# mrjoshuak/go-jpeg2000

Hardware: AMD Instinct MI355X
Metric: Mpixels/s encode+decode (4K sRGB, 5-3 lossless) (higher is better)
Workload: dtype int32

## Files before the change

go-jpeg2000_amd/csrc/ht.hip:

```cpp
#include <cstdlib>

#include "ht_tables.h"
#include "j2k_internal.h"

namespace j2k {

__device__ __constant__ uint16_t c_vlc_tbl0[1024] = J2K_HT_VLC_TBL0_INIT;
__device__ __constant__ uint16_t c_vlc_tbl1[1024] = J2K_HT_VLC_TBL1_INIT;
__device__ uint16_t g_vlc_enc[2 * 4 * 16];

__global__ void ht_build_enc_table() {
    const int t = threadIdx.x;
    if (t >= 128) return;
    const int initial = t >> 6, context = (t >> 4) & 3, rho = t & 15;
    const uint16_t *tbl = initial ? c_vlc_tbl0 : c_vlc_tbl1;
    uint16_t r = 0x0001;
    for (uint32_t cwd = 0; cwd < 128; cwd++) {
        const uint16_t e = tbl[(context << 7) | cwd];
        if (((e >> 4) & 0xF) == rho && (e & 0xF) > 0) { r = (uint16_t)((cwd << 4) | (e & 0xF)); break; }
    }
    g_vlc_enc[t] = r;
}

__device__ uint16_t g_vlc_pair1[16384];

__global__ void ht_build_pair_table() {
    const uint32_t idx = blockIdx.x * blockDim.x + threadIdx.x;
    if (idx >= 16384) return;
    const uint32_t e1 = c_vlc_tbl1[idx & 0x7F];
    const uint32_t len1 = e1 & 0xF, rho1 = (e1 >> 4) & 0xF, uo1 = (e1 >> 3) & 1;
    uint32_t r = 0x8000;
    if (len1 <= 7) {
        const uint32_t e2 = c_vlc_tbl1[((rho1 >> 2) << 7) | ((idx >> len1) & 0x7F)];
        const uint32_t len2 = e2 & 0xF, rho2 = (e2 >> 4) & 0xF, uo2 = (e2 >> 3) & 1;
        r = rho1 | rho2 << 4 | (len1 + len2) << 8 | uo2 << 13 | uo1 << 14;
    }
    g_vlc_pair1[idx] = (uint16_t)r;
}

__device__ __forceinline__ uint32_t shl32(uint32_t x, uint32_t n) { return n >= 32 ? 0u : x << n; }
__device__ __forceinline__ uint64_t shl64(uint64_t x, uint32_t n) { return n >= 64 ? 0ull : x << n; }
__device__ __forceinline__ uint64_t shr64(uint64_t x, uint32_t n) { return n >= 64 ? 0ull : x >> n; }
__device__ __forceinline__ uint32_t uabs(int v) { return v < 0 ? 0u - (uint32_t)v : (uint32_t)v; }

__device__ __forceinline__ uint32_t wave_incl_scan(uint32_t v) {
    v += (uint32_t)__builtin_amdgcn_update_dpp(0, (int)v, 0x111, 0xf, 0xf, false);
    v += (uint32_t)__builtin_amdgcn_update_dpp(0, (int)v, 0x112, 0xf, 0xf, false);
    v += (uint32_t)__builtin_amdgcn_update_dpp(0, (int)v, 0x114, 0xf, 0xf, false);
    v += (uint32_t)__builtin_amdgcn_update_dpp(0, (int)v, 0x118, 0xf, 0xf, false);
    v += (uint32_t)__builtin_amdgcn_update_dpp(0, (int)v, 0x142, 0xa, 0xf, false);
    v += (uint32_t)__builtin_amdgcn_update_dpp(0, (int)v, 0x143, 0xc, 0xf, false);
    return v;
}
__device__ __forceinline__ uint32_t wave_last(uint32_t v) { return (uint32_t)__builtin_amdgcn_readlane((int)v, 63); }

struct BitWriter {
    uint8_t *p;
    long pos, cap;
    uint64_t tmp;
    int bits;
    uint32_t last;
    int fault;
};

__device__ __forceinline__ void vlc_write(BitWriter &v, uint32_t val, uint32_t nbits) {
    v.tmp |= shl64((uint64_t)val, (uint32_t)v.bits);
    v.bits += (int)nbits;
    while (v.bits >= 8) {
        uint32_t b = (uint32_t)(v.tmp & 0xFF);
        if (v.last > 0x8F && (b & 0x7F) == 0x7F) b &= 0x7F;
        if (v.pos >= v.cap) { v.fault = 1; v.bits = 0; return; }
        v.p[v.pos++] = (uint8_t)b;
        v.last = b;
        v.tmp >>= 8;
        v.bits -= 8;
    }
}

__device__ __forceinline__ void ms_write(BitWriter &m, uint32_t val, uint32_t nbits) {
    m.tmp |= shl64((uint64_t)val, (uint32_t)m.bits);
    m.bits += (int)nbits;
    while (m.bits >= 8) {
        uint32_t b = (uint32_t)(m.tmp & 0xFF);
        if (m.pos >= m.cap) { m.fault = 1; m.bits = 0; return; }
        if (m.last == 0xFF) { b &= 0x7F; m.p[m.pos++] = (uint8_t)b; m.tmp >>= 7; m.bits -= 7; }
        else { m.p[m.pos++] = (uint8_t)b; m.tmp >>= 8; m.bits -= 8; }
        m.last = b;
    }
}

__device__ __forceinline__ void flush_bits(BitWriter &w) {
    while (w.bits > 0) {
        if (w.pos >= w.cap) { w.fault = 1; return; }
        w.p[w.pos++] = (uint8_t)(w.tmp & 0xFF);
        w.tmp >>= 8;
        w.bits -= 8;
        if (w.bits < 0) w.bits = 0;
    }
}

__device__ __forceinline__ void uvlc_one(BitWriter &v, uint32_t u) {
    if (u <= 1) vlc_write(v, 1, 1);
    else if (u <= 2) vlc_write(v, 2, 2);
    else { vlc_write(v, 0, 3); vlc_write(v, u - 3, 5); }
}

#define HT_FAST_MAX_SAMPLES 1024
#define HT_MS_WORDS (HT_FAST_MAX_SAMPLES * 31 / 32 + 4)
#define HT_VLC_WORDS (46 * (HT_FAST_MAX_SAMPLES / 8) / 32 + 8)

__device__ __forceinline__ void or_bits(uint32_t *buf, uint32_t bitpos, uint64_t val) {
    const uint32_t wd = bitpos >> 5, sh = bitpos & 31;
    const uint32_t lo = (uint32_t)(val << sh);
    const uint64_t hi = sh ? (val >> (32 - sh)) : (val >> 32);
    if (lo) atomicOr(&buf[wd], lo);
    if ((uint32_t)hi) atomicOr(&buf[wd + 1], (uint32_t)hi);
    if ((uint32_t)(hi >> 32)) atomicOr(&buf[wd + 2], (uint32_t)(hi >> 32));
}
__device__ __forceinline__ void zero_bytes(uint8_t *p, size_t n, int lane) {
    const size_t head = min(n, (size_t)((16 - ((uintptr_t)p & 15)) & 15));
    if ((size_t)lane < head) p[lane] = 0;
    uint8_t *q = p + head;
    const size_t nv = (n - head) >> 4;
    for (size_t i = lane; i < nv; i += 64) reinterpret_cast<uint4 *>(q)[i] = make_uint4(0, 0, 0, 0);
    const size_t done = head + (nv << 4);
    if (done + lane < n) p[done + lane] = 0;
}

__device__ __forceinline__ uint32_t ms_bits32(const uint32_t *buf, uint32_t bitpos) {
    const uint32_t wd = bitpos >> 5, sh = bitpos & 31;
    const uint64_t two = (uint64_t)buf[wd] | ((uint64_t)buf[wd + 1] << 32);
    return (uint32_t)(two >> sh);
}
__device__ __forceinline__ uint32_t get_bits8(const uint32_t *buf, uint32_t bitpos) {
    const uint32_t wd = bitpos >> 5, sh = bitpos & 31;
    const uint64_t two = (uint64_t)buf[wd] | ((uint64_t)buf[wd + 1] << 32);
    return (uint32_t)(two >> sh) & 0xFF;
}

template <bool LROWS>
__device__ __forceinline__ bool ht_form(const BlockJob &J, const int32_t *__restrict__ src, int lane, uint32_t *vbuf, uint32_t *mbuf,
                        uint32_t &TMout, uint32_t &TVout, const int32_t *lrows, const uint16_t *enc) {
    const int w = J.w, h = J.h, stride = LROWS ? J.w : J.stride;
    const int quadCols = (w + 3) / 4, P = (quadCols + 1) / 2, R = (h + 3) / 4, N = R * P;
    for (int i = lane; i < HT_VLC_WORDS; i += 64) vbuf[i] = 0;
    for (int i = lane; i < HT_MS_WORDS; i += 64) mbuf[i] = 0;
    __syncthreads();
    uint32_t vbase = 0, mbase = 0;
    int bad = 0;
    const bool vec_ok = ((J.stride & 3) == 0) && ((J.src_off & 3) == 0);
    for (int i0 = 0; i0 < N; i0 += 64) {
        const int it = i0 + lane;
        uint64_t vv = 0; uint32_t vl = 0, ml = 0;
        uint32_t mval[8], mlen[8];
#pragma unroll
        for (int i = 0; i < 8; i++) { mval[i] = 0; mlen[i] = 0; }
        if (it < N) {
            const int r = it / P, pi = it - r * P;
            const int initial = (r == 0);
            const int32_t *row = LROWS ? lrows + r * w : src + (size_t)(4 * r) * stride;
            const int xb = pi * 8;
            int v[8];
            if ((LROWS || vec_ok) && xb + 8 <= w) {
                const int4 a = *reinterpret_cast<const int4 *>(row + xb), b = *reinterpret_cast<const int4 *>(row + xb + 4);
                v[0] = a.x; v[1] = a.y; v[2] = a.z; v[3] = a.w; v[4] = b.x; v[5] = b.y; v[6] = b.z; v[7] = b.w;
            } else {
#pragma unroll
                for (int i = 0; i < 8; i++) {
                    const int t = row[xb + i < w ? xb + i : w - 1];
                    v[i] = (xb + i < w) ? t : 0;
                }
            }
            uint32_t rho = 0, rho2 = 0;
#pragma unroll
            for (int i = 0; i < 4; i++) {
                if (v[i] != 0) rho |= 1u << i;
                if (v[4 + i] != 0) rho2 |= 1u << i;
            }
            const uint32_t e1 = enc[(initial << 6) | rho];
            const uint32_t e2 = enc[(initial << 6) | ((rho >> 2) << 4) | rho2];
            vv = (uint64_t)(e1 >> 4);
            vl = e1 & 0xF;
            vv |= (uint64_t)(e2 >> 4) << vl;
            vl += e2 & 0xF;
            if (rho | rho2) {
                uint32_t u1 = 1, u2 = 1;
#pragma unroll
                for (int i = 0; i < 4; i++) {
                    if (xb + i < w && uabs(v[i]) >= shl32(1, u1)) u1++;
                    if (xb + 4 + i < w && uabs(v[4 + i]) >= shl32(1, u2)) u2++;
                }
#pragma unroll
                for (int q = 0; q < 2; q++) {
                    if (!(q ? rho2 : rho)) continue;
                    const uint32_t u = q ? u2 : u1;
                    if (u <= 1) { vv |= (uint64_t)1 << vl; vl += 1; }
                    else if (u <= 2) { vv |= (uint64_t)2 << vl; vl += 2; }
                    else { vv |= (uint64_t)(u - 3) << (vl + 3); vl += 8; }
                }
            }
#pragma unroll
            for (int i = 0; i < 8; i++) {
                const uint32_t rr = (i < 4) ? rho : rho2;
                if (!((rr >> (i & 3)) & 1)) continue;
                const uint32_t mag = uabs(v[i]);
                if (mag >= 0x80000000u) { bad = 1; continue; }
                const uint32_t emb = 32 - __clz(mag);
                mval[i] = (mag & (shl32(1, emb - 1) - 1)) | ((v[i] < 0 ? 1u : 0u) << (emb - 1));
                mlen[i] = emb;
                ml += emb;
            }
        }
        const uint32_t vs = wave_incl_scan(vl), ms = wave_incl_scan(ml);
        const uint32_t vtot = wave_last(vs), mtot = wave_last(ms);
        uint32_t vpos = vbase + vs - vl, mpos = mbase + ms - ml;
        if (it < N) {
            or_bits(vbuf, vpos, vv);
            if (ml <= 64) {
                uint64_t acc = 0;
                uint32_t sh = 0;
#pragma unroll
                for (int i = 0; i < 8; i++) {
                    acc |= shl64((uint64_t)mval[i], sh);
                    sh += mlen[i];
                }
                if (acc) or_bits(mbuf, mpos, acc);
            } else {
#pragma unroll
                for (int i = 0; i < 8; i++)
                    if (mlen[i]) { or_bits(mbuf, mpos, (uint64_t)mval[i]); mpos += mlen[i]; }
            }
        }
        vbase += vtot; mbase += mtot;
    }
    bad = __any(bad);
    __syncthreads();
    if (bad) return false;
    TMout = mbase; TVout = vbase;
    return true;
}

#define HT_MS_FF_CAP 2176
__device__ __forceinline__ int ht_ms_find_ff(const uint32_t *mbuf, uint32_t TM, int lane, uint16_t *flist, uint32_t &myF) {
    int nF = 0;
    uint32_t base = 0;
    myF = 0;
    const uint32_t nwords = (TM + 31) >> 5;
    for (uint32_t w0 = 0; w0 < nwords; w0 += 64) {
        const uint32_t wi = w0 + lane;
        uint64_t x = 0;
        if (wi < nwords) x = (uint64_t)mbuf[wi] | ((uint64_t)mbuf[wi + 1] << 32);
        uint64_t y = x & (x >> 1);
        y &= y >> 2;
        y &= y >> 4;
        const uint32_t m = (uint32_t)y;
        const uint32_t p0 = 32u * wi;
        for (;;) {
            const uint32_t lo = base > p0 ? base - p0 : 0u;
            const uint32_t cand = lo >= 32 ? 0u : (m & (0xFFFFFFFFu << lo) & (0x01010101u << (base & 7)));
            const unsigned long long who = __ballot(cand != 0);
            if (!who) break;
            const int L = __ffsll((long long)who) - 1;
            const uint32_t cL = (uint32_t)__builtin_amdgcn_readlane((int)cand, L);
            const uint32_t p = 32u * (w0 + (uint32_t)L) + (uint32_t)__ffs((int)cL) - 1;
            if (lane == 0) flist[nF] = (uint16_t)p;
            if (lane == nF) myF = p;
            nF++;
            base = p + 15;
        }
    }
    return nF;
}

template <bool WRITE>
__device__ bool ht_emit(const BlockJob &J, uint8_t *__restrict__ out, int lane, const uint32_t *vbuf, const uint32_t *mbuf,
                        uint32_t mbase, uint32_t vbase, long &magLenOut, long &vlcLenOut, uint16_t *flist) {
    const size_t nsamp = (size_t)J.w * J.h;
    const size_t maxSize = nsamp * 2 < 64 ? 64 : nsamp * 2;
    const long msCap = (long)(maxSize / 2), vlcCap = (long)(maxSize / 2);
    const size_t melLen = maxSize / 4;
    const uint32_t TM = mbase;
#ifdef J2K_ENC_STAMP
    const long long e0 = wall_clock64();
#endif
    uint32_t myF;
    const int nF = ht_ms_find_ff(mbuf, TM, lane, flist, myF);
    __syncthreads();
#ifdef J2K_ENC_STAMP
    const long long e05 = wall_clock64();
#endif
    auto kF = [&](int i) { return (long)(((uint32_t)flist[i] + (uint32_t)i) >> 3); };
    long K = 0;
    uint32_t posK = 0;
    if (TM >= 8) {
        K = (long)((TM - 8 + (uint32_t)nF) >> 3) + 1;
        posK = (uint32_t)(8 * K) - (uint32_t)nF;
        if (nF) {
            const uint32_t Fl = flist[nF - 1];
            const long kl = kF(nF - 1);
            if (K - 1 < kl + 2) {
                if (Fl + 16 <= TM) { K = kl + 2; posK = Fl + 15; }
                else { K = kl + 1; posK = Fl + 8; }
            }
        }
    }
    const bool tail = TM > posK;
    const long magLen = K + (tail ? 1 : 0);
    if (magLen > msCap) return false;
    if (WRITE) {
        const bool inreg = nF <= 64;
        const long myK = (lane < nF) ? (long)((myF + (uint32_t)lane) >> 3) : (long)0x7FFFFFFF;
        int fi = 0;
        for (long kb = 0; kb < K; kb += 256) {
            int fe;
            if (inreg) {
                fi = __popcll(__ballot(myK <= kb - 2));
                fe = __popcll(__ballot(myK <= kb + 254));
            } else {
                while (fi < nF && kF(fi) <= kb - 2) fi++;
                fe = fi;
                while (fe < nF && kF(fe) <= kb + 254) fe++;
            }
            const long k0 = kb + 4 * lane;
            uint32_t dw = 0;
            if (fe == fi) {
                if (k0 < K) dw = ms_bits32(mbuf, (uint32_t)(8 * k0) - (uint32_t)fi);
            } else {
                uint32_t n[4] = {(uint32_t)fi, (uint32_t)fi, (uint32_t)fi, (uint32_t)fi}, narrow = 0;
                for (int i = fi; i < fe; i++) {
                    const long kk = inreg ? (long)__builtin_amdgcn_readlane((int)myK, i) : kF(i);
#pragma unroll
                    for (int j = 0; j < 4; j++) {
                        if (kk <= k0 + j - 2) n[j]++;
                        if (kk == k0 + j - 1) narrow |= 1u << j;
                    }
                }
#pragma unroll
                for (int j = 0; j < 4; j++) {
                    if (k0 + j >= K) break;
                    const uint32_t bj = get_bits8(mbuf, (uint32_t)(8 * (k0 + j)) - n[j]) & (((narrow >> j) & 1) ? 0x7Fu : 0xFFu);
                    dw |= bj << (8 * j);
                }
            }
            if (k0 >= K) continue;
            uint8_t *q = out + k0;
            if (k0 + 4 <= K) __builtin_memcpy(q, &dw, 4);
            else {
#pragma unroll
                for (int j = 0; j < 3; j++)
                    if (k0 + j < K) q[j] = (uint8_t)(dw >> (8 * j));
            }
        }
        if (tail && lane == 0) out[K] = (uint8_t)get_bits8(mbuf, posK);
    }
#ifdef J2K_ENC_STAMP
    const long long e1 = wall_clock64();
#endif
    const uint32_t TV = vbase;
    const long nfull = TV >> 3, vlcLen = (TV + 7) >> 3;
    if (vlcLen > vlcCap) return false;
    uint8_t *vout = out + magLen + melLen;
    for (long i0 = 4 * lane; WRITE && i0 < vlcLen; i0 += 256) {
        uint32_t dw = ms_bits32(vbuf, (uint32_t)(8 * i0));
#pragma unroll
        for (int jj = 0; jj < 4; jj++) {
            const long i = i0 + jj;
            uint32_t b = (dw >> (8 * jj)) & 0xFF;
            if (i < nfull && (b & 0x7F) == 0x7F && i > 0) {
                long j = i - 1;
                while (j > 0 && (get_bits8(vbuf, (uint32_t)(8 * j)) & 0x7F) == 0x7F) j--;
                uint32_t prev = (j == 0 && (get_bits8(vbuf, 0) & 0x7F) == 0x7F) ? get_bits8(vbuf, 0)
                                                                                 : get_bits8(vbuf, (uint32_t)(8 * j));
                for (long k = j + 1; k < i; k++) {
                    uint32_t rb = get_bits8(vbuf, (uint32_t)(8 * k));
                    if (prev > 0x8F && (rb & 0x7F) == 0x7F) rb &= 0x7F;
                    prev = rb;
                }
                if (prev > 0x8F) dw &= ~(0x80u << (8 * jj));
            }
        }
        uint8_t *q = vout + i0;
        if (i0 + 4 <= vlcLen) __builtin_memcpy(q, &dw, 4);
        else {
#pragma unroll
            for (int jj = 0; jj < 3; jj++)
                if (i0 + jj < vlcLen) q[jj] = (uint8_t)(dw >> (8 * jj));
        }
    }
    magLenOut = magLen; vlcLenOut = vlcLen;
#ifdef J2K_ENC_STAMP
    if (((blockIdx.x % 200) == 7) && lane == 0) printf("   wg %d find_ff %lld (nF %d) ms emit %lld vlc emit %lld\n", (int)blockIdx.x, e05 - e0, nF, e1 - e05, wall_clock64() - e1);
#endif
    return true;
}


template <bool LROWS>
__device__ __forceinline__ bool ht_encode_fast(const BlockJob &J, const int32_t *__restrict__ src, uint8_t *__restrict__ out, int lane,
                               uint32_t *vbuf, uint32_t *mbuf, long &magLenOut, long &vlcLenOut, const int32_t *lrows, const uint16_t *enc,
                               uint16_t *flist) {
    uint32_t TM, TV;
#ifdef J2K_ENC_STAMP
    const long long f0 = wall_clock64(), c0 = clock64();
#endif
    if (!ht_form<LROWS>(J, src, lane, vbuf, mbuf, TM, TV, lrows, enc)) return false;
#ifdef J2K_ENC_STAMP
    if (0) printf("   wg %d form %lld wall ticks, %lld shader clocks\n", (int)blockIdx.x, wall_clock64() - f0, clock64() - c0);
#endif
    return ht_emit<true>(J, out, lane, vbuf, mbuf, TM, TV, magLenOut, vlcLenOut, flist);
}

__global__ __launch_bounds__(64) void ht_encode_kernel(const BlockJob *__restrict__ jobs, int njobs,
                                                       const int32_t *__restrict__ coef, uint8_t *__restrict__ slots,
                                                       uint32_t *__restrict__ lens, uint8_t *__restrict__ numbps,
                                                       int *__restrict__ fault, uint32_t *__restrict__ maglens,
                                                       const HtUJob *__restrict__ utab, const int *__restrict__ alias_ids) {
    __shared__ uint32_t s_vbuf[HT_VLC_WORDS];
    __shared__ uint32_t s_mbuf[HT_MS_WORDS];
    __shared__ __align__(16) int32_t s_rows[HT_FAST_MAX_SAMPLES];
    __shared__ uint32_t s_enc[64];
    __shared__ uint16_t s_ff[HT_MS_FF_CAP];
    if ((int)blockIdx.x >= njobs) return;
    const int lane = threadIdx.x;
#ifdef J2K_ENC_STAMP
    const long long st0 = wall_clock64();
#endif
    BlockJob J;
    int jid = (int)blockIdx.x, nalias = 1, aoff = 0;
    if (utab) {
        const HtUJob U = utab[blockIdx.x];
        J = U.J; jid = U.jid; nalias = U.nalias; aoff = U.alias_off;
    } else {
        J = jobs[jid];
    }
    int myalias = jid;
    if (utab && lane < nalias) myalias = alias_ids[aoff + lane];
    s_enc[lane] = reinterpret_cast<const uint32_t *>(g_vlc_enc)[lane];
    const int w = J.w, h = J.h, stride = J.stride;
    const int32_t *src = coef + J.src_off;
    uint8_t *out = slots + J.out_off;
    auto publish = [&](uint32_t len, uint32_t nb, bool has_mag, uint32_t mag) {
        for (int k = lane; k < nalias; k += 64) {
            const int j = k < 64 ? myalias : alias_ids[aoff + k];
            lens[j] = len;
            numbps[j] = (uint8_t)nb;
            if (maglens && has_mag) maglens[j] = mag;
        }
    };
    const bool fast = (size_t)((h + 3) / 4) * (size_t)w <= HT_FAST_MAX_SAMPLES;

    int maxMag = 0;
    const bool quads = (w & 3) == 0 && (stride & 3) == 0 && (J.src_off & 3) == 0;
    const bool lrows = quads && fast;
    if (quads) {
        const int wq = w >> 2, nq = wq * h;
        const int dy = 64 / wq, dx = 64 - dy * wq;
        int y = lane / wq, xq = lane - y * wq;
        for (int e0 = lane; e0 < nq; e0 += 64 * 16) {
            int4 qv[16];
            int ys[16];
#pragma unroll
            for (int u = 0; u < 16; u++) {
                const bool ok = e0 + 64 * u < nq;
                const int4 t = *reinterpret_cast<const int4 *>(ok ? src + (size_t)y * stride + 4 * xq : src);
                qv[u] = ok ? t : make_int4(0, 0, 0, 0);
                ys[u] = ok ? (y << 8 | xq) : -1;
                y += dy; xq += dx;
                if (xq >= wq) { xq -= wq; y++; }
            }
#pragma unroll
            for (int u = 0; u < 16; u++) {
                const int4 q = qv[u];
                if (lrows && ys[u] >= 0 && ((ys[u] >> 8) & 3) == 0)
                    *reinterpret_cast<int4 *>(&s_rows[(ys[u] >> 10) * w + 4 * (ys[u] & 0xFF)]) = q;
                const int a0 = q.x < 0 ? (int)(0u - (uint32_t)q.x) : q.x, a1 = q.y < 0 ? (int)(0u - (uint32_t)q.y) : q.y;
                const int a2 = q.z < 0 ? (int)(0u - (uint32_t)q.z) : q.z, a3 = q.w < 0 ? (int)(0u - (uint32_t)q.w) : q.w;
                maxMag = max(max(maxMag, max(a0, a1)), max(a2, a3));
            }
        }
    } else {
        for (int y = 0; y < h; y++)
            for (int x = lane; x < w; x += 64) {
                int v = src[(size_t)y * stride + x];
                if (v < 0) v = (int)(0u - (uint32_t)v);
                maxMag = max(maxMag, v);
            }
    }
    for (int o = 32; o > 0; o >>= 1) maxMag = max(maxMag, __shfl_xor(maxMag, o));
#ifdef J2K_ENC_STAMP
    const long long st1 = wall_clock64();
#endif
    if (maxMag == 0) {
        publish(0, 0, false, 0);
        return;
    }
    if (fast) {
        long mLen = 0, vLen = 0;
        const size_t nsamp_ = (size_t)w * h;
        const size_t maxSize_ = nsamp_ * 2 < 64 ? 64 : nsamp_ * 2;
        const size_t melLen_ = maxSize_ / 4;
        const uint16_t *enc = reinterpret_cast<const uint16_t *>(s_enc);
        const bool ok = lrows ? ht_encode_fast<true>(J, src, out, lane, s_vbuf, s_mbuf, mLen, vLen, s_rows, enc, s_ff)
                              : ht_encode_fast<false>(J, src, out, lane, s_vbuf, s_mbuf, mLen, vLen, nullptr, enc, s_ff);
        if (!ok) {
            if (lane == 0) atomicMax(fault, 1);
            publish(0, 0, false, 0);
            return;
        }
        if (!maglens) zero_bytes(out + mLen, melLen_, lane);
        const size_t scup = melLen_ + (size_t)vLen + 2;
        const size_t total = (size_t)mLen + scup;
        if (lane == 0) {
            out[total - 2] = (uint8_t)(scup >> 8);
            out[total - 1] = (uint8_t)(scup & 0xFF);
        }
        publish((uint32_t)total, 32 - __clz((uint32_t)maxMag), true, (uint32_t)mLen);
#ifdef J2K_ENC_STAMP
        const long long st2 = wall_clock64();
        if (((blockIdx.x % 200) == 7 || blockIdx.x >= njobs - 3) && lane == 0)
            printf("enc wg %d: start %lld end %lld scan %lld  form+emit %lld (x10 ns)  mLen %ld vLen %ld\n", (int)blockIdx.x, st0 % 100000, st2 % 100000, st1 - st0, st2 - st1, mLen, vLen);
#endif
        return;
    }
    const size_t nsamp = (size_t)w * h;
    const size_t maxSize = nsamp * 2 < 64 ? 64 : nsamp * 2;
    const size_t msCap = maxSize / 2, melLen = maxSize / 4, vlcCap = maxSize / 2;
    uint8_t *vlcScratch = out + msCap + melLen;

    long magLen = 0, vlcLen = 0;
    int bad = 0;
    if (lane == 0) {
        BitWriter vlc{vlcScratch, 0, (long)vlcCap, 0, 0, 0, 0};
        BitWriter ms{out, 0, (long)msCap, 0, 0, 0, 0};
        const int quadCols = (w + 3) / 4;
        for (int y = 0; y < h && !vlc.fault && !ms.fault; y += 4) {
            const int initial = (y == 0);
            const int32_t *row = src + (size_t)y * stride;
            for (int qx = 0; qx < quadCols && !vlc.fault && !ms.fault; qx += 2) {
                int v[8];
                uint32_t rho = 0, rho2 = 0;
#pragma unroll
                for (int i = 0; i < 8; i++) {
                    const int x = qx * 4 + i;
                    v[i] = (x < w) ? row[x] : 0;
                }
#pragma unroll
                for (int i = 0; i < 4; i++) {
                    if (qx * 4 + i < w && v[i] != 0) rho |= 1u << i;
                    if ((qx + 1) * 4 + i < w && v[4 + i] != 0) rho2 |= 1u << i;
                }
                uint16_t e1 = g_vlc_enc[(initial << 6) | rho];
                vlc_write(vlc, e1 >> 4, e1 & 0xF);
                uint16_t e2 = g_vlc_enc[(initial << 6) | ((rho >> 2) << 4) | rho2];
                vlc_write(vlc, e2 >> 4, e2 & 0xF);
                if (rho | rho2) {
                    uint32_t u1 = 1, u2 = 1;
#pragma unroll
                    for (int i = 0; i < 4; i++) {
                        if (qx * 4 + i < w && uabs(v[i]) >= shl32(1, u1)) u1++;
                        if ((qx + 1) * 4 + i < w && uabs(v[4 + i]) >= shl32(1, u2)) u2++;
                    }
                    if (rho && rho2) { uvlc_one(vlc, u1); uvlc_one(vlc, u2); }
                    else uvlc_one(vlc, rho ? u1 : u2);
                }
#pragma unroll
                for (int i = 0; i < 8; i++) {
                    const uint32_t r = (i < 4) ? rho : rho2;
                    if (!((r >> (i & 3)) & 1)) continue;
                    const uint32_t mag = uabs(v[i]);
                    if (mag >= 0x80000000u) { ms.fault = 1; break; }
                    const uint32_t emb = 32 - __clz(mag);
                    ms_write(ms, mag & (shl32(1, emb - 1) - 1), emb - 1);
                    ms_write(ms, v[i] < 0 ? 1u : 0u, 1);
                }
            }
        }
        if (!vlc.fault) flush_bits(vlc);
        if (!ms.fault) flush_bits(ms);
        magLen = ms.pos; vlcLen = vlc.pos;
        bad = vlc.fault | ms.fault;
    }
    magLen = __shfl(magLen, 0); vlcLen = __shfl(vlcLen, 0); bad = __shfl(bad, 0);
    if (bad) {
        if (lane == 0) atomicMax(fault, 1);
        publish(0, 0, false, 0);
        return;
    }
    zero_bytes(out + magLen, melLen, lane);
    __syncthreads();
    const size_t D = (size_t)magLen + melLen;
    for (long base = 0; base < vlcLen; base += 64) {
        const long i = base + lane;
        uint8_t b = 0;
        if (i < vlcLen) b = vlcScratch[i];
        __syncthreads();
        if (i < vlcLen) out[D + i] = b;
        __syncthreads();
    }
    {
        const size_t scup = melLen + (size_t)vlcLen + 2;
        const size_t total = (size_t)magLen + scup;
        if (lane == 0) {
            out[total - 2] = (uint8_t)(scup >> 8);
            out[total - 1] = (uint8_t)(scup & 0xFF);
        }
        publish((uint32_t)total, 32 - __clz((uint32_t)maxMag), true, (uint32_t)magLen);
    }
}

#define HT_ST_AGG 1ull
#define HT_ST_PREFIX 2ull
__device__ __forceinline__ unsigned long long ht_status(unsigned long long flag, uint32_t epoch, unsigned long long value) {
    return flag << 62 | (unsigned long long)(epoch & 0x3FFFFF) << 40 | (value & 0xFFFFFFFFFFull);
}

__global__ __launch_bounds__(64) void ht_encode_stream_kernel(const BlockJob *__restrict__ jobs, int njobs,
                                                              const int32_t *__restrict__ coef, uint8_t *__restrict__ stream,
                                                              unsigned long long *__restrict__ offs, uint32_t *__restrict__ lens,
                                                              uint8_t *__restrict__ numbps, unsigned long long *__restrict__ status,
                                                              uint32_t epoch, int *__restrict__ fault) {
    __shared__ uint32_t s_vbuf[HT_VLC_WORDS];
    __shared__ uint32_t s_mbuf[HT_MS_WORDS];
    __shared__ uint16_t s_ff[HT_MS_FF_CAP];
    const int jid = blockIdx.x;
    if (jid >= njobs) return;
    const int lane = threadIdx.x;
    const BlockJob J = jobs[jid];
    const int w = J.w, h = J.h, stride = J.stride;
    const int32_t *src = coef + J.src_off;
    int maxMag = 0;
    if ((w & 3) == 0 && (stride & 3) == 0 && (J.src_off & 3) == 0) {
        const int wq = w >> 2, nq = wq * h;
        const int dy = 64 / wq, dx = 64 - dy * wq;
        int y = lane / wq, xq = lane - y * wq;
        for (int e = lane; e < nq; e += 64) {
            const int4 q = *reinterpret_cast<const int4 *>(src + (size_t)y * stride + 4 * xq);
            const int a0 = q.x < 0 ? (int)(0u - (uint32_t)q.x) : q.x, a1 = q.y < 0 ? (int)(0u - (uint32_t)q.y) : q.y;
            const int a2 = q.z < 0 ? (int)(0u - (uint32_t)q.z) : q.z, a3 = q.w < 0 ? (int)(0u - (uint32_t)q.w) : q.w;
            maxMag = max(max(maxMag, max(a0, a1)), max(a2, a3));
            y += dy; xq += dx;
            if (xq >= wq) { xq -= wq; y++; }
        }
    } else {
        for (int y = 0; y < h; y++)
            for (int x = lane; x < w; x += 64) {
                int v = src[(size_t)y * stride + x];
                if (v < 0) v = (int)(0u - (uint32_t)v);
                maxMag = max(maxMag, v);
            }
    }
    for (int o = 32; o > 0; o >>= 1) maxMag = max(maxMag, __shfl_xor(maxMag, o));
    const size_t nsamp = (size_t)w * h;
    const size_t maxSize = nsamp * 2 < 64 ? 64 : nsamp * 2;
    const size_t melLen = maxSize / 4;
    uint32_t TM = 0, TV = 0;
    long mLen = 0, vLen = 0;
    unsigned long long total = 0;
    if (maxMag != 0) {
        bool ok = ht_form<false>(J, src, lane, s_vbuf, s_mbuf, TM, TV, nullptr, g_vlc_enc);
        if (ok) ok = ht_emit<false>(J, nullptr, lane, s_vbuf, s_mbuf, TM, TV, mLen, vLen, s_ff);
        if (ok) total = (unsigned long long)mLen + melLen + (unsigned long long)vLen + 2;
        else if (lane == 0) atomicMax(fault, 1);
    }
    if (lane == 0) __hip_atomic_store(&status[jid], ht_status(HT_ST_AGG, epoch, total), __ATOMIC_RELAXED, __HIP_MEMORY_SCOPE_AGENT);
    unsigned long long excl = 0;
    int base = jid - 1;
    uint32_t spins = 0;
    while (base >= 0) {
        const int idx = base - lane;
        const unsigned long long v = idx >= 0 ? __hip_atomic_load(&status[idx], __ATOMIC_RELAXED, __HIP_MEMORY_SCOPE_AGENT)
                                              : ht_status(HT_ST_PREFIX, epoch, 0);
        const unsigned long long flag = v >> 62;
        const bool valid = flag != 0 && (uint32_t)((v >> 40) & 0x3FFFFF) == (epoch & 0x3FFFFF);
        const unsigned long long inv = __ballot(!valid), pre = __ballot(valid && flag == HT_ST_PREFIX);
        const int first_inv = inv ? __ffsll((long long)inv) - 1 : 64, first_pre = pre ? __ffsll((long long)pre) - 1 : 64;
        if (first_inv < first_pre) {
            if (++spins > (1u << 22)) { if (lane == 0) atomicMax(fault, 3); break; }
            __builtin_amdgcn_s_sleep(8);
            continue;
        }
        const int upto = min(first_pre, 63);
        unsigned long long part = lane <= upto ? (v & 0xFFFFFFFFFFull) : 0ull;
        for (int o = 32; o > 0; o >>= 1) part += __shfl_xor(part, o);
        excl += part;
        if (first_pre < 64) break;
        base -= 64;
    }
    if (lane == 0) {
        __hip_atomic_store(&status[jid], ht_status(HT_ST_PREFIX, epoch, excl + total), __ATOMIC_RELAXED, __HIP_MEMORY_SCOPE_AGENT);
        offs[jid] = excl;
        if (jid == njobs - 1) offs[njobs] = excl + total;
        lens[jid] = (uint32_t)total;
        numbps[jid] = total ? (uint8_t)(32 - __clz((uint32_t)maxMag)) : 0;
    }
    if (!total) return;
    uint8_t *out = stream + excl;
    ht_emit<true>(J, out, lane, s_vbuf, s_mbuf, TM, TV, mLen, vLen, s_ff);
    zero_bytes(out + mLen, melLen, lane);
    if (lane == 0) {
        const size_t scup = melLen + (size_t)vLen + 2;
        out[total - 2] = (uint8_t)(scup >> 8);
        out[total - 1] = (uint8_t)(scup & 0xFF);
    }
}

struct RevStream { const uint8_t *data; long len, pos, size; uint64_t tmp; uint32_t bits; int unstuff; };
struct FwdStream { const uint8_t *data; long len, pos, size; uint64_t tmp; uint32_t bits; int unstuff; uint32_t x; };

__device__ void rev_read(RevStream &v) {
    if (v.bits > 32) return;
    uint32_t val = 0;
    if (v.size > 3) {
        const long p = v.pos - 3;
        if (p >= 0 && p + 3 < v.len)
            val = (uint32_t)v.data[p] | (uint32_t)v.data[p + 1] << 8 | (uint32_t)v.data[p + 2] << 16 | (uint32_t)v.data[p + 3] << 24;
        v.pos -= 4; v.size -= 4;
    } else if (v.size > 0) {
        int i = 24;
        while (v.size > 0) {
            if (v.pos >= 0 && v.pos < v.len) { val |= (uint32_t)v.data[v.pos] << i; v.pos--; }
            v.size--; i -= 8;
        }
    }
    uint32_t tmp = val >> 24, bits = 8;
    if (v.unstuff && ((val >> 24) & 0x7F) == 0x7F) bits = 7;
    int unstuff = (val >> 24) > 0x8F;
    tmp |= ((val >> 16) & 0xFF) << bits;
    bits += (unstuff && ((val >> 16) & 0x7F) == 0x7F) ? 7 : 8;
    unstuff = ((val >> 16) & 0xFF) > 0x8F;
    tmp |= ((val >> 8) & 0xFF) << bits;
    bits += (unstuff && ((val >> 8) & 0x7F) == 0x7F) ? 7 : 8;
    unstuff = ((val >> 8) & 0xFF) > 0x8F;
    tmp |= (val & 0xFF) << bits;
    bits += (unstuff && (val & 0x7F) == 0x7F) ? 7 : 8;
    v.unstuff = (val & 0xFF) > 0x8F;
    v.tmp |= shl64((uint64_t)tmp, v.bits);
    v.bits += bits;
}
__device__ __forceinline__ uint32_t rev_fetch(RevStream &v) {
    if (v.bits < 32) { rev_read(v); if (v.bits < 32) rev_read(v); }
    return (uint32_t)v.tmp;
}
__device__ __forceinline__ void rev_advance(RevStream &v, uint32_t n) { v.tmp = shr64(v.tmp, n); v.bits -= n; }

__device__ void fwd_read(FwdStream &f) {
    if (f.bits > 32) return;
    uint32_t val = 0;
    if (f.size > 3) {
        if (f.pos + 3 < f.len)
            val = (uint32_t)f.data[f.pos] | (uint32_t)f.data[f.pos + 1] << 8 | (uint32_t)f.data[f.pos + 2] << 16 | (uint32_t)f.data[f.pos + 3] << 24;
        f.pos += 4; f.size -= 4;
    } else if (f.size > 0) {
        if (f.x != 0) val = 0xFFFFFFFFu;
        int i = 0;
        while (f.size > 0) {
            if (f.pos < f.len) {
                const uint32_t b = f.data[f.pos];
                val = (val & ~((uint32_t)0xFF << i)) | (b << i);
                f.pos++;
            }
            f.size--; i += 8;
        }
    } else if (f.x != 0) {
        val = 0xFFFFFFFFu;
    }
    uint32_t bits = f.unstuff ? 7 : 8;
    uint32_t t = val & 0xFF;
    int unstuff = (val & 0xFF) == 0xFF;
    t |= ((val >> 8) & 0xFF) << bits;
    bits += unstuff ? 7 : 8;
    unstuff = ((val >> 8) & 0xFF) == 0xFF;
    t |= ((val >> 16) & 0xFF) << bits;
    bits += unstuff ? 7 : 8;
    unstuff = ((val >> 16) & 0xFF) == 0xFF;
    t |= ((val >> 24) & 0xFF) << bits;
    bits += unstuff ? 7 : 8;
    f.unstuff = ((val >> 24) & 0xFF) == 0xFF;
    f.tmp |= shl64((uint64_t)t, f.bits);
    f.bits += bits;
}
__device__ __forceinline__ uint32_t fwd_fetch(FwdStream &f) {
    if (f.bits < 32) { fwd_read(f); if (f.bits < 32) fwd_read(f); }
    return (uint32_t)f.tmp;
}
__device__ __forceinline__ void fwd_advance(FwdStream &f, uint32_t n) { f.tmp = shr64(f.tmp, n); f.bits -= n; }

__device__ __forceinline__ uint32_t uvlc_entry(uint32_t idx) {
    return (uint32_t)(0x21422167214221B7ull >> (8 * (idx & 7))) & 0xFF;
}

__device__ uint32_t decode_uvlc(uint32_t vlc, uint32_t mode, uint32_t (&u)[2], int initial) {
    uint32_t consumed = 0;
    u[0] = 1; u[1] = 1;
    if (mode == 0) return 0;
    if (mode <= 2) {
        const uint32_t t = uvlc_entry(vlc);
        const uint32_t pl = t & 3; vlc >>= pl; consumed += pl;
        const uint32_t sl = (t >> 2) & 7; consumed += sl;
        const uint32_t val = (t >> 5) + (vlc & (shl32(1, sl) - 1));
        if (mode == 1) u[0] = val + 1; else u[1] = val + 1;
    } else if (mode == 3) {
        const uint32_t t1 = uvlc_entry(vlc);
        const uint32_t pl1 = t1 & 3; vlc >>= pl1; consumed += pl1;
        if (initial && pl1 > 2) {
            u[1] = (vlc & 1) + 2; consumed++; vlc >>= 1;
            const uint32_t sl = (t1 >> 2) & 7; consumed += sl;
            u[0] = (t1 >> 5) + (vlc & (shl32(1, sl) - 1)) + 1;
        } else {
            const uint32_t t2 = uvlc_entry(vlc);
            const uint32_t pl2 = t2 & 3; vlc >>= pl2; consumed += pl2;
            const uint32_t sl1 = (t1 >> 2) & 7; consumed += sl1;
            u[0] = (t1 >> 5) + (vlc & (shl32(1, sl1) - 1)) + 1;
            vlc >>= sl1;
            const uint32_t sl2 = (t2 >> 2) & 7; consumed += sl2;
            u[1] = (t2 >> 5) + (vlc & (shl32(1, sl2) - 1)) + 1;
        }
    }
    return consumed;
}

__device__ __forceinline__ uint32_t decode_uvlc_later(uint32_t vlc, uint32_t uOff1, uint32_t uOff2, uint32_t &u0, uint32_t &u1) {
    const uint32_t t1 = uOff2 ? uvlc_entry(vlc) : 0u;
    const uint32_t pl1 = t1 & 3; vlc >>= pl1;
    const uint32_t t2 = uOff1 ? uvlc_entry(vlc) : 0u;
    const uint32_t pl2 = t2 & 3; vlc >>= pl2;
    const uint32_t sl1 = (t1 >> 2) & 7, sl2 = (t2 >> 2) & 7;
    u0 = (t1 >> 5) + (vlc & ((1u << sl1) - 1)) + 1;
    vlc >>= sl1;
    u1 = (t2 >> 5) + (vlc & ((1u << sl2) - 1)) + 1;
    return pl1 + pl2 + sl1 + sl2;
}

__device__ bool init_mel_ok(const uint8_t *data, long len, long lcup, long scup) {
    long pos = lcup - scup, size = scup - 1;
    int unstuff = 0;
    long num = 4 - (pos & 3);
    if (num > 4) num = 4;
    for (long i = 0; i < num && size > 0; i++) {
        if (unstuff && pos < len && data[pos] > 0x8F) return false;
        uint32_t b;
        if (size > 0 && pos < len) { b = data[pos]; pos++; size--; } else b = 0xFF;
        if (size == 1) b |= 0x0F;
        unstuff = (b == 0xFF);
    }
    return true;
}

#define HT_WALK_MAX_PAIRS 128
#define HT_DEC_MWORDS (33 * HT_FAST_MAX_SAMPLES / 32 + 8)
#define HT_WALK_REC 132
#define HT_PAIR_SERIAL 0xFFFFFFFFu
#define HT_PAIR_ZERO 0xFFFFFFFEu

__device__ __forceinline__ void wave_sync() {
    __builtin_amdgcn_fence(__ATOMIC_RELEASE, "wavefront");
    __builtin_amdgcn_wave_barrier();
    __builtin_amdgcn_fence(__ATOMIC_ACQUIRE, "wavefront");
}

__device__ __forceinline__ uint32_t get_bits32(const uint32_t *buf, uint32_t bitpos) {
    const uint32_t wd = bitpos >> 5, sh = bitpos & 31;
    const uint64_t two = (uint64_t)buf[wd] | ((uint64_t)buf[wd + 1] << 32);
    return (uint32_t)(two >> sh);
}

__device__ __forceinline__ uint32_t get_bits32_cut(const uint32_t *buf, uint32_t bitpos, uint32_t L) {
    if (bitpos >= L) return 0;
    const uint32_t p = bitpos < (HT_DEC_MWORDS - 2) * 32u ? bitpos : (HT_DEC_MWORDS - 2) * 32u + (bitpos & 31);
    uint32_t v = get_bits32(buf, p);
    if (L - bitpos < 32) v &= (1u << (L - bitpos)) - 1;
    return v;
}

#define HT_VBITS_WORDS 192
#define HT_VROW 193

__global__ __launch_bounds__(256) void ht_vlcprep_kernel(const BlockJob *__restrict__ jobs, int njobs,
                                                         const uint8_t *__restrict__ stream, const uint64_t *__restrict__ offs,
                                                         const uint32_t *__restrict__ lens, uint32_t *__restrict__ vbits,
                                                         uint32_t *__restrict__ pairs) {
    __shared__ uint32_t vb4[4][HT_VBITS_WORDS + 8];
    uint32_t *vb = vb4[threadIdx.x >> 6];
    const int jid = blockIdx.x * 4 + (threadIdx.x >> 6);
    if (jid >= njobs) return;
    const int lane = threadIdx.x & 63;
    const int w = jobs[jid].w, h = jobs[jid].h;
    const long len = (long)lens[jid];
    const uint8_t *data = stream + offs[jid];
    uint32_t *rec = pairs + (size_t)jid * HT_WALK_REC;
    const int quadCols = (w + 3) / 4, P = (quadCols + 1) / 2, R = (h + 3) / 4, N = R * P;
    const bool fast = (size_t)R * (size_t)w <= HT_FAST_MAX_SAMPLES && N <= HT_WALK_MAX_PAIRS;
    uint32_t tag = 0;
    long scup = 0;
    if (!fast) tag = HT_PAIR_SERIAL;
    else if (len < 2) tag = HT_PAIR_ZERO;
    else {
        scup = (long)data[len - 1] + ((long)(data[len - 2] & 0x0F) << 8);
        if (scup < 2 || scup > len) tag = HT_PAIR_ZERO;
        else if (!init_mel_ok(data, len, len, scup)) tag = HT_PAIR_ZERO;
    }
    if (tag) {
        if (lane == 0) { rec[0] = tag; rec[HT_WALK_MAX_PAIRS] = 0; }
        return;
    }
    for (int i = lane; i < HT_VBITS_WORDS + 8; i += 64) vb[i] = 0;
    wave_sync();
    const long lcup = len;
    const uint32_t b0 = data[lcup - 2];
    const uint32_t t0 = b0 >> 4;
    uint32_t off = 4 - ((t0 & 7) >> 2);
    if (lane == 0) atomicOr(&vb[0], t0);
    const long size = scup - 2;
    const long maxbytes = (long)(46 * N + 7) / 8 + 8;
    const long nb = size < maxbytes ? size : maxbytes;
    uint32_t carry = b0 | 0x0F;
    for (long k0 = 1; k0 <= nb; k0 += 256) {
        const long k = k0 + 4 * lane;
        const long e = lcup - 2 - k;
        uint32_t dw = 0;
        if (k + 3 <= nb) {
            __builtin_memcpy(&dw, data + e - 3, 4);
            dw = __builtin_bswap32(dw);
        } else {
#pragma unroll
            for (int j = 0; j < 4; j++)
                if (k + j <= nb) dw |= (uint32_t)data[e - j] << (8 * j);
        }
        uint32_t prev = __shfl_up(dw >> 24, 1);
        if (lane == 0) prev = carry;
        carry = __shfl(dw >> 24, 63);
        uint32_t wsum = 0;
        uint64_t merged = 0;
#pragma unroll
        for (int j = 0; j < 4; j++) {
            const uint32_t bj = (dw >> (8 * j)) & 0xFF;
            const uint32_t wj = (k + j <= nb) ? ((prev > 0x8F && (bj & 0x7F) == 0x7F) ? 7u : 8u) : 0u;
            merged |= (uint64_t)bj << wsum;
            wsum += wj;
            prev = bj;
        }
        const uint32_t ws = wave_incl_scan(wsum);
        if (merged) or_bits(vb, off + ws - wsum, merged);
        off += wave_last(ws);
    }
    wave_sync();
    uint32_t *dst = vbits + (size_t)jid * HT_VBITS_WORDS;
    for (int i = lane; i < HT_VBITS_WORDS; i += 64) dst[i] = vb[i];
    if (lane == 0) { rec[0] = 0; rec[HT_WALK_MAX_PAIRS] = (uint32_t)scup; }
}

#ifndef HT_WALK_BLOCKS
#define HT_WALK_BLOCKS 64
#endif
struct HtWalkShared {
    uint32_t vb[HT_WALK_BLOCKS][HT_VROW];
    uint16_t pair1[16384];
    uint16_t tbl0[512], tbl1[512];
};

__device__ __forceinline__ uint32_t uvlc_used_later(uint32_t vlc, uint32_t uOff1, uint32_t uOff2) {
    const uint32_t t1 = uOff2 ? uvlc_entry(vlc) : 0u;
    const uint32_t pl1 = t1 & 3;
    const uint32_t t2 = uOff1 ? uvlc_entry(vlc >> pl1) : 0u;
    return pl1 + (t2 & 3) + ((t1 >> 2) & 7) + ((t2 >> 2) & 7);
}

__global__ __launch_bounds__(256) void ht_walk_kernel(const BlockJob *__restrict__ jobs, int njobs,
                                                     const uint32_t *__restrict__ vbits, uint32_t *__restrict__ pairs) {
    extern __shared__ __align__(16) unsigned char walk_smem[];
    HtWalkShared &S = *reinterpret_cast<HtWalkShared *>(walk_smem);
    const int tid = threadIdx.x, lane = tid & 63;
    const int jid0 = blockIdx.x * HT_WALK_BLOCKS;
    const int jid = jid0 + lane;
    const bool have = lane < HT_WALK_BLOCKS && jid < njobs;
#ifdef J2K_WALK_STAMP
    const long long st0 = __builtin_amdgcn_s_memtime();
#endif
    const int nblk = min(HT_WALK_BLOCKS, njobs - jid0);
    uint32_t *rec = pairs + (size_t)jid * HT_WALK_REC;
    uint32_t tag = HT_PAIR_ZERO;
    int w = 0, h = 0;
    if (tid < 64 && have) { tag = rec[0]; w = jobs[jid].w; h = jobs[jid].h; }
    {
        constexpr int NV = HT_WALK_BLOCKS * 48 / 256;
        uint4 t[8], v[NV];
#pragma unroll
        for (int j = 0; j < 8; j++) t[j] = reinterpret_cast<const uint4 *>(g_vlc_pair1)[j * 256 + tid];
#pragma unroll
        for (int j = 0; j < NV; j++) {
            const int q = j * 256 + tid;
            const int bsel = min(q / 48, nblk - 1);
            v[j] = reinterpret_cast<const uint4 *>(vbits + (size_t)(jid0 + bsel) * HT_VBITS_WORDS)[q % 48];
        }
        if (tid < 64) reinterpret_cast<uint4 *>(S.tbl0)[tid] = reinterpret_cast<const uint4 *>(c_vlc_tbl0)[tid];
        else if (tid < 128) reinterpret_cast<uint4 *>(S.tbl1)[tid - 64] = reinterpret_cast<const uint4 *>(c_vlc_tbl1)[tid - 64];
#pragma unroll
        for (int j = 0; j < 8; j++) reinterpret_cast<uint4 *>(S.pair1)[j * 256 + tid] = t[j];
#pragma unroll
        for (int j = 0; j < NV; j++) {
            const int q = j * 256 + tid;
            uint32_t *d = &S.vb[q / 48][4 * (q % 48)];
            d[0] = v[j].x; d[1] = v[j].y; d[2] = v[j].z; d[3] = v[j].w;
        }
    }
    __syncthreads();
#ifdef J2K_WALK_STAMP
    const long long st1 = __builtin_amdgcn_s_memtime();
#endif
    if (tid >= 64) return;
    const int quadCols = (w + 3) / 4, P = (quadCols + 1) / 2, R = (h + 3) / 4;
    const bool walks = have && tag != HT_PAIR_SERIAL && tag != HT_PAIR_ZERO;
    int nsteps = walks ? R * P : 0;
#pragma unroll
    for (int o = 32; o > 0; o >>= 1) nsteps = max(nsteps, __shfl_xor(nsteps, o));
    nsteps = min(__builtin_amdgcn_readfirstlane(nsteps), HT_WALK_MAX_PAIRS);
    if (!walks) return;
    const uint32_t *row = &S.vb[lane][0];
    uint32_t pos = 0;
#define HT_FETCH(w0, w1)                                                          \
    uint32_t w0, w1;                                                               \
    {                                                                              \
        const uint32_t *p_ = row + (pos >> 5);                                     \
        const uint32_t d0_ = p_[0], d1_ = p_[1], d2_ = p_[2];                      \
        w0 = __builtin_amdgcn_alignbit(d1_, d0_, pos & 31);                        \
        w1 = __builtin_amdgcn_alignbit(d2_, d1_, pos & 31);                        \
    }
    for (int pi = 0; pi < P; pi++) {
        HT_FETCH(w0, w1)
        const uint32_t qinf = S.tbl0[w0 & 0x7F];
        const uint32_t rho = (qinf >> 4) & 0xF, uOff1 = (qinf >> 3) & 1, len1 = qinf & 0xF;
        const uint32_t qinf2 = S.tbl0[((rho >> 2) << 7) | ((w0 >> len1) & 0x7F)];
        const uint32_t rho2 = (qinf2 >> 4) & 0xF, uOff2 = (qinf2 >> 3) & 1, len = len1 + (qinf2 & 0xF);
        const uint32_t vw = __builtin_amdgcn_alignbit(w1, w0, len);
        const uint32_t mode = (uOff1 << 1) | uOff2;
        uint32_t u[2];
        const uint32_t used = decode_uvlc(vw, mode, u, 1);
        pos += len + used;
        rec[pi] = rho | rho2 << 4 | mode << 13 | vw << 16;
    }
    {
        for (int it = P; it < nsteps; it++) {
            HT_FETCH(w0, w1)
            uint32_t e = S.pair1[w0 & 0x3FFF];
            if (e & 0x8000) {
                const uint32_t qinf = S.tbl1[w0 & 0x7F];
                const uint32_t rho = (qinf >> 4) & 0xF, len1 = qinf & 0xF;
                const uint32_t qinf2 = S.tbl1[((rho >> 2) << 7) | ((w0 >> len1) & 0x7F)];
                e = rho | (qinf2 & 0xF0) | (len1 + (qinf2 & 0xF)) << 8 | ((qinf2 >> 3) & 1) << 13 | ((qinf >> 3) & 1) << 14;
            }
            const uint32_t len = (e >> 8) & 0x1F;
            const uint32_t vw = __builtin_amdgcn_alignbit(w1, w0, len);
            const uint32_t m1 = (uint32_t)((int32_t)(e << 18) >> 31), m2 = (uint32_t)((int32_t)(e << 17) >> 31);
            const uint32_t pl1 = (0x12131213u >> ((vw & 7) << 2)) & 3 & m1;
            const uint32_t t1 = (0x12141218u >> ((vw & 7) << 2)) & 0xF & m1;
            const uint32_t t2 = (0x12141218u >> (((vw >> pl1) & 7) << 2)) & 0xF & m2;
            pos += len + t1 + t2;
            rec[it] = (e & 0x7FFF) | vw << 16;
        }
    }
#undef HT_FETCH
#ifdef J2K_WALK_STAMP
    const long long st2 = __builtin_amdgcn_s_memtime();
    if ((blockIdx.x == 0 || blockIdx.x == 50) && lane == 0)
        printf("walk wg %d: staging %lld cyc, loop %lld cyc (%d pairs, %d bits)\n", (int)blockIdx.x, st1 - st0, st2 - st1, R * P, (int)pos);
#endif
}

#define HT_MAX_FF 64
#ifndef J2K_DECODED_NT
#define J2K_DECODED_NT 1
#endif
__device__ __forceinline__ void st_decoded(int32_t *p, int a, int b, int c, int d) {
    typedef int v4i_ __attribute__((ext_vector_type(4)));
    const v4i_ v = {a, b, c, d};
    if (J2K_DECODED_NT) __builtin_nontemporal_store(v, reinterpret_cast<v4i_ *>(p));
    else *reinterpret_cast<v4i_ *>(p) = v;
}

#ifdef J2K_DEC_STAMP
static __device__ long long g_dbg_unstuff_dummy;
#define g_dbg_unstuff S.dbg_t
#endif
struct HtDecShared {
#ifdef J2K_DEC_STAMP
    long long dbg_t;
#endif
    uint32_t mbuf[HT_DEC_MWORDS];
    uint32_t pair[HT_WALK_MAX_PAIRS];
    uint32_t ffpos[HT_MAX_FF];
    uint32_t nff;
};

__device__ uint32_t ht_loaded_bits(const HtDecShared &S, uint32_t nff, long segLen, uint32_t j) {
    const long k = 4 * (long)j;
    const long kk = k < segLen ? k : segLen;
    uint32_t f = 0, last_ff = 0;
    for (uint32_t i = 0; i < nff; i++) {
        if ((long)S.ffpos[i] + 2 <= kk) f++;
        if ((long)S.ffpos[i] == segLen - 1) last_ff = 1;
    }
    uint32_t b = (uint32_t)(8 * kk) - f;
    if (k > segLen) b += (last_ff ? 7u : 8u) + 7u * (uint32_t)(k - segLen - 1);
    return b;
}

template <bool STRIDED>
__device__ bool ht_extract_fast(HtDecShared &S, const uint8_t *__restrict__ data, long len, long scup, int w, int h,
                                int32_t *__restrict__ out, int lane, bool bigu, const uint32_t (&mpos2)[2], uint32_t total_bits,
                                const uint32_t (&raw0)[4], int os_) {
    const size_t os64 = STRIDED ? (size_t)os_ : (size_t)64, osw = STRIDED ? (size_t)os_ : (size_t)w;
    const int quadCols = (w + 3) / 4, P = (quadCols + 1) / 2, R = (h + 3) / 4, N = R * P;
    const long lcup = len;
    {
        const long segLen0 = lcup - scup;
        const long cap0 = (long)HT_DEC_MWORDS * 4 - 16;
        const uint32_t zw = bigu ? (uint32_t)HT_DEC_MWORDS
                                 : min((uint32_t)HT_DEC_MWORDS, (uint32_t)(((segLen0 < cap0 ? segLen0 : cap0) * 8) >> 5) + 3u);
        for (uint32_t i = lane; i < zw; i += 64) S.mbuf[i] = 0;
    }
    if (lane == 0) S.nff = 0;
    wave_sync();
    constexpr int PF = 4;
    {
        const long segLen = lcup - scup;
        const long maxbytes = (long)HT_DEC_MWORDS * 4 - 16;
        const long nb = segLen < maxbytes ? segLen : maxbytes;
        const long d = (long)((uintptr_t)data & 3);
        const uint32_t *wsrc = reinterpret_cast<const uint32_t *>(data - d);
        const long ndw = (d + nb + 3) >> 2;
        uint32_t off = 0, carry = 0;
        for (long j0 = 0; j0 < ndw; j0 += 64 * PF) {
            uint32_t raw[PF];
#pragma unroll
            for (int c = 0; c < PF; c++) {
                const long j = j0 + 64 * c + lane;
                if (j0 == 0) raw[c] = raw0[c];
                else raw[c] = wsrc[j < ndw ? j : ndw - 1];
            }
#pragma unroll
            for (int c = 0; c < PF; c++) {
                if (j0 + 64 * c >= ndw) break;
                const long j = j0 + 64 * c + lane;
                const uint32_t dw = raw[c];
                uint32_t prev3 = __shfl_up(dw >> 24, 1);
                if (lane == 0) prev3 = carry;
                carry = __shfl(dw >> 24, 63);
                const long k0 = 4 * j - d;
                uint32_t wd[4], tot = 0;
                bool plain = (j < ndw) && k0 >= 1 && k0 + 4 <= nb && prev3 != 0xFF;
#pragma unroll
                for (int t = 0; t < 4; t++) {
                    const long k = k0 + t;
                    const uint32_t pb = t ? ((dw >> (8 * (t - 1))) & 0xFF) : prev3;
                    const bool valid = (j < ndw) && k >= 0 && k < nb;
                    wd[t] = valid ? ((k > 0 && pb == 0xFF) ? 7u : 8u) : 0u;
                    if (t && pb == 0xFF) plain = false;
                    tot += wd[t];
                    if (bigu && valid && ((dw >> (8 * t)) & 0xFF) == 0xFF) {
                        const uint32_t idx = atomicAdd(&S.nff, 1u);
                        if (idx < HT_MAX_FF) S.ffpos[idx] = (uint32_t)k;
                    }
                }
                const uint32_t ws = wave_incl_scan(tot);
                uint32_t pos = off + ws - tot;
                if (plain) {
                    if (dw) or_bits(S.mbuf, pos, (uint64_t)dw);
                } else {
#pragma unroll
                    for (int t = 0; t < 4; t++) {
                        const uint32_t bt = (dw >> (8 * t)) & 0xFF;
                        if (wd[t] && bt) or_bits(S.mbuf, pos, (uint64_t)bt);
                        pos += wd[t];
                    }
                }
                off += wave_last(ws);
            }
        }
        wave_sync();
        if (bigu && (nb != segLen || S.nff > HT_MAX_FF)) return false;
        if (nb == segLen) {
            const uint32_t wd0 = off >> 5;
            const uint32_t wend = bigu ? (uint32_t)HT_DEC_MWORDS : min((uint32_t)HT_DEC_MWORDS, (total_bits >> 5) + 3u);
            for (uint32_t i = wd0 + lane; i < wend; i += 64)
                S.mbuf[i] = (i == wd0) ? (S.mbuf[i] | (0xFFFFFFFFu << (off & 31))) : 0xFFFFFFFFu;
        }
    }
    wave_sync();
#ifdef J2K_DEC_STAMP
    g_dbg_unstuff = wall_clock64();
#endif
#ifdef J2K_DEC_STOP_B
    if (total_bits != 0x7fffffff) return true;
#endif
    uint32_t Lcut = 0xFFFFFFFFu;
    if (bigu) {
        const long segLen = lcup - scup;
        const uint32_t nff = S.nff;
        uint32_t best_key = 0xFFFFFFFFu, best_L = 0xFFFFFFFFu, mb = 0;
        for (int i0 = 0; i0 < N; i0 += 64) {
            const int it = i0 + lane;
            uint32_t nbits = 0, rho = 0, rho2 = 0, u0 = 1, u1 = 1;
            if (it < N) {
                const uint32_t info = S.pair[it];
                const int pi = it % P, xb = pi * 8;
                rho = info & 0xF; rho2 = (info >> 4) & 0xF; u0 = (info >> 8) & 0x3F; u1 = (info >> 14) & 0x3F;
                const uint32_t m1 = (xb + 4 <= w) ? 0xFu : ((xb < w) ? ((1u << (w - xb)) - 1) : 0u);
                const uint32_t m2 = (xb + 8 <= w) ? 0xFu : ((xb + 4 < w) ? ((1u << (w - xb - 4)) - 1) : 0u);
                rho &= m1; rho2 &= m2;
                nbits = __popc(rho) * (u0 + 1) + __popc(rho2) * (u1 + 1);
            }
            const uint32_t ns = wave_incl_scan(nbits);
            uint32_t mpos = mb + ns - nbits;
            mb += wave_last(ns);
            if (it < N) {
                for (int i = 0; i < 8; i++) {
                    const uint32_t rr = (i < 4) ? rho : rho2, emb = (i < 4) ? u0 : u1;
                    if (!((rr >> (i & 3)) & 1)) continue;
                    if (emb > 32 && best_key == 0xFFFFFFFFu) {
                        uint32_t j = (mpos + 32) / 32;
                        if (j < 2) j = 2;
                        uint32_t G = ht_loaded_bits(S, nff, segLen, j);
                        while (G < mpos + 32) G = ht_loaded_bits(S, nff, segLen, ++j);
                        if (G - mpos < emb) { best_key = (uint32_t)(it * 8 + i); best_L = G; }
                    }
                    mpos += emb + 1;
                }
            }
        }
        uint32_t k = best_key;
#pragma unroll
        for (int o = 32; o > 0; o >>= 1) k = min(k, (uint32_t)__shfl_xor(k, o));
        const unsigned long long who = __ballot(best_key == k && k != 0xFFFFFFFFu);
        if (who) Lcut = __shfl(best_L, __ffsll((long long)who) - 1);
    }
#pragma unroll
    for (int t = 0; t < 2; t++) {
        if (64 * t >= N) break;
        const int it = 64 * t + lane;
        uint32_t rho = 0, rho2 = 0, u0 = 1, u1 = 1;
        int r = 0, pi = 0;
        if (it < N) {
            const uint32_t info = S.pair[it];
            r = it / P; pi = it - r * P;
            rho = info & 0xF; rho2 = (info >> 4) & 0xF; u0 = (info >> 8) & 0x3F; u1 = (info >> 14) & 0x3F;
            const int xb = pi * 8;
            const uint32_t m1 = (xb + 4 <= w) ? 0xFu : ((xb < w) ? ((1u << (w - xb)) - 1) : 0u);
            const uint32_t m2 = (xb + 8 <= w) ? 0xFu : ((xb + 4 < w) ? ((1u << (w - xb - 4)) - 1) : 0u);
            rho &= m1; rho2 &= m2;
        }
        uint32_t mpos = mpos2[t];
        int vals[8] = {0, 0, 0, 0, 0, 0, 0, 0};
        if (it < N && !bigu) {
            const uint32_t half0 = 1u << (u0 - 1), half1 = 1u << (u1 - 1);
#pragma unroll
            for (int i = 0; i < 8; i++) {
                const uint32_t rr = (i < 4) ? rho : rho2, emb = (i < 4) ? u0 : u1;
                const bool on = (rr >> (i & 3)) & 1;
                const uint32_t wd = mpos >> 5;
                const uint32_t win = __builtin_amdgcn_alignbit(S.mbuf[wd + 1], S.mbuf[wd], mpos & 31);
                const uint32_t mag = __builtin_amdgcn_ubfe(win, 0, emb) + ((i < 4) ? half0 : half1);
                const uint32_t sg = 0u - ((win >> emb) & 1);
                vals[i] = on ? (int32_t)((mag ^ sg) - sg) : 0;
                mpos += on ? emb + 1 : 0u;
            }
        } else if (it < N) {
#pragma unroll
            for (int i = 0; i < 8; i++) {
                const uint32_t rr = (i < 4) ? rho : rho2, emb = (i < 4) ? u0 : u1;
                if (!((rr >> (i & 3)) & 1)) continue;
                const uint32_t magVal = get_bits32_cut(S.mbuf, mpos, Lcut);
                const uint32_t sign = get_bits32_cut(S.mbuf, mpos + emb, Lcut) & 1;
                const uint32_t mag = (magVal & (shl32(1, emb) - 1)) + shl32(1, emb - 1);
                mpos += emb + 1;
                vals[i] = sign ? (int32_t)(0u - mag) : (int32_t)mag;
            }
        }
        if (w == 64 && (((uintptr_t)out) & 15) == 0 && (!STRIDED || (os_ & 3) == 0)) {
#pragma unroll
            for (int half = 0; half < 2; half++) {
                const int drow = half * 4 + (lane >> 4), q = lane & 15;
                const int src = drow * 8 + (q >> 1);
                int o[4];
#pragma unroll
                for (int i = 0; i < 4; i++) {
                    const int a = __shfl(vals[i], src), b = __shfl(vals[4 + i], src);
                    o[i] = (q & 1) ? b : a;
                }
                const int rg = 8 * t + drow;
#ifdef J2K_DEC_NO_CODED_STORES
                if (o[0] == 0x7fffffff)
#endif
                if (rg < R) st_decoded(out + (size_t)(4 * rg) * os64 + 4 * q, o[0], o[1], o[2], o[3]);
            }
        } else if (it < N) {
            const int xb = pi * 8;
            int32_t *orow = out + (size_t)(4 * r) * osw + xb;
            if (xb + 8 <= w && (((uintptr_t)orow) & 15) == 0) {
                st_decoded(orow, vals[0], vals[1], vals[2], vals[3]);
                st_decoded(orow + 4, vals[4], vals[5], vals[6], vals[7]);
            } else {
#pragma unroll
                for (int i = 0; i < 8; i++)
                    if (xb + i < w) orow[i] = vals[i];
            }
        }
    }
    return true;
}

template <bool STRIDED>
__global__ __launch_bounds__(256) __attribute__((amdgpu_waves_per_eu(7, 8))) void ht_decode_kernel(const BlockJob *__restrict__ jobs, int njobs,
                                                        const uint8_t *__restrict__ stream, const uint64_t *__restrict__ offs,
                                                        const uint32_t *__restrict__ lens, int32_t *__restrict__ decoded,
                                                        const uint32_t *__restrict__ pairs, int coded_rows_only_) {
    const int coded_rows_only = STRIDED ? 1 : coded_rows_only_;
    __shared__ HtDecShared S4[4];
    HtDecShared &S = S4[threadIdx.x >> 6];
    const int jid = blockIdx.x * 4 + (threadIdx.x >> 6);
    if (jid >= njobs) return;
    const int lane = threadIdx.x & 63;
#ifdef J2K_DEC_STAMP
    const long long d0 = wall_clock64();
#endif
    const BlockJob J = jobs[jid];
    const int w = J.w, h = J.h;
    const int os_ = STRIDED ? J.stride : w;
    int32_t *out = decoded + J.out_off;
    const size_t n = (size_t)w * h;
    const uint32_t *rec = pairs + (size_t)jid * HT_WALK_REC;
    const uint32_t r0 = rec[lane], r1 = rec[64 + lane];
    const uint64_t my_off = offs[jid];
    const uint32_t my_len = lens[jid], my_scup = rec[HT_WALK_MAX_PAIRS];
    const uint32_t tag = __shfl(r0, 0);
    const bool fast = (tag != HT_PAIR_ZERO) && (tag != HT_PAIR_SERIAL);
    auto zero_fill = [&](bool skip_coded) {
        if (coded_rows_only) {
            if (skip_coded) return;
            const uint32_t uw = (uint32_t)w, nrow = (uint32_t)(h + 3) >> 2;
            for (uint32_t i = lane; i < uw * nrow; i += 64) out[(size_t)(i / uw) * 4 * (STRIDED ? (uint32_t)os_ : uw) + i % uw] = 0;
            return;
        }
        if (w == 64 && (J.out_off & 3) == 0) {
            if (skip_coded && lane < 16) return;
            int32_t *q = out + 4 * (size_t)lane;
            for (int i = 0; i < h / 4; i++) st_decoded(q + 256 * (size_t)i, 0, 0, 0, 0);
            const int rem = h & 3;
            if (lane < 16 * rem) st_decoded(q + 256 * (size_t)(h / 4), 0, 0, 0, 0);
        } else if ((w & 3) == 0 && (J.out_off & 3) == 0) {
            const uint32_t wq = (uint32_t)w >> 2, nq = (uint32_t)(n >> 2);
            const uint32_t dy = 64u / wq, dx = 64u % wq;
            uint32_t y = (uint32_t)lane / wq, x = (uint32_t)lane % wq;
            for (uint32_t i = lane; i < nq; i += 64) {
                if (!skip_coded || (y & 3)) st_decoded(out + 4 * (size_t)i, 0, 0, 0, 0);
                y += dy; x += dx;
                if (x >= wq) { x -= wq; y++; }
            }
        } else {
            const uint32_t uw = (uint32_t)w;
            const uint32_t dy = 64u / uw, dx = 64u % uw;
            uint32_t y = (uint32_t)lane / uw, x = (uint32_t)lane % uw;
            for (uint32_t i = lane; i < (uint32_t)n; i += 64) {
                if (!skip_coded || (y & 3)) out[i] = 0;
                y += dy; x += dx;
                if (x >= uw) { x -= uw; y++; }
            }
        }
    };
    if (!fast) zero_fill(false);
    uint32_t raw0[4] = {0, 0, 0, 0};
#ifdef J2K_DEC_STAMP
    const long long d_a = wall_clock64();
#endif
    if (fast) {
        const uint8_t *fdata = stream + my_off;
        const long segLen = (long)my_len - (long)my_scup;
        const long maxbytes = (long)HT_DEC_MWORDS * 4 - 16;
        const long nb = segLen < maxbytes ? segLen : maxbytes;
        const long d = (long)((uintptr_t)fdata & 3);
        const uint32_t *wsrc = reinterpret_cast<const uint32_t *>(fdata - d);
        const long ndw = (d + nb + 3) >> 2;
        if (ndw > 0) {
#pragma unroll
            for (int c = 0; c < 4; c++) {
                const long j = 64 * c + lane;
                raw0[c] = wsrc[j < ndw ? j : ndw - 1];
            }
        }
        zero_fill(true);
#ifdef J2K_DEC_ONLY_ZERO
        return;
#endif
    }
#ifdef J2K_DEC_STAMP
    const long long d_b = wall_clock64();
#endif
    bool bigu = false;
    uint32_t mpos2[2] = {0, 0}, total_bits = 0;
    {
        const int quadCols = (w + 3) / 4, P = (quadCols + 1) / 2, N = ((h + 3) / 4) * P;
        uint32_t rr[2] = {r0, r1};
#pragma unroll
        for (int t = 0; t < 2; t++) {
            const int it = lane + 64 * t;
            const uint32_t r = rr[t], mode = (r >> 13) & 3, vw = r >> 16;
            uint32_t u0, u1;
            decode_uvlc_later(vw, mode >> 1, mode & 1, u0, u1);
            if (it < P) {
                uint32_t u[2];
                decode_uvlc(vw, mode, u, 1);
                u0 = u[0]; u1 = u[1];
            }
            if (it < N && (u0 > 31 || u1 > 31)) bigu = true;
            S.pair[it] = (r & 0xFF) | (u0 & 0x3F) << 8 | (u1 & 0x3F) << 14;
            uint32_t nbits = 0;
            if (it < N) {
                const int pi = it % P, xb = pi * 8;
                const uint32_t m1 = (xb + 4 <= w) ? 0xFu : ((xb < w) ? ((1u << (w - xb)) - 1) : 0u);
                const uint32_t m2 = (xb + 8 <= w) ? 0xFu : ((xb + 4 < w) ? ((1u << (w - xb - 4)) - 1) : 0u);
                nbits = __popc(r & 0xF & m1) * ((u0 & 0x3F) + 1) + __popc((r >> 4) & 0xF & m2) * ((u1 & 0x3F) + 1);
            }
            const uint32_t ns = wave_incl_scan(nbits);
            mpos2[t] = total_bits + ns - nbits;
            total_bits += wave_last(ns);
        }
        bigu = __any(bigu);
    }
    wave_sync();
#ifdef J2K_DEC_STAMP
    const long long d_c = wall_clock64();
#endif
#ifdef J2K_DEC_STOP_A
    if (total_bits != 0x7fffffff) return;
#endif
    if (tag == HT_PAIR_ZERO) return;
    if (tag != HT_PAIR_SERIAL) {
        const uint8_t *fdata = stream + my_off;
        const long flen = (long)my_len;
        const long fscup = (long)my_scup;
        if (ht_extract_fast<STRIDED>(S, fdata, flen, fscup, w, h, out, lane, bigu, mpos2, total_bits, raw0, os_)) {
#ifdef J2K_DEC_STAMP
            if ((jid % 700) == 13 && lane == 0) printf("dec job %d: start %lld | job+records %lld | prefetch+zero issue %lld | uvlc+pos %lld | unstuff %lld | extract %lld | end %lld (x10 ns)\n", jid, d0 % 100000, d_a - d0, d_b - d_a, d_c - d_b, g_dbg_unstuff - d_c, wall_clock64() - g_dbg_unstuff, wall_clock64() % 100000);
#endif
            return;
        }
        zero_fill(false);
    }
    __builtin_amdgcn_fence(__ATOMIC_SEQ_CST, "workgroup");
    __builtin_amdgcn_wave_barrier();
    if (lane != 0) return;
    const uint8_t *data = stream + offs[jid];
    const long len = (long)lens[jid];
    if (len < 2) return;
    const long scup = (long)data[len - 1] + ((long)(data[len - 2] & 0x0F) << 8);
    if (scup < 2 || scup > len) return;
    const long lcup = len;
    if (!init_mel_ok(data, len, lcup, scup)) return;

    RevStream vlc{data, len, lcup - 2, scup - 2, 0, 0, 0};
    if (vlc.pos >= 0 && vlc.pos < len) {
        const uint32_t b = data[vlc.pos];
        vlc.pos--;
        vlc.tmp = (uint64_t)(b >> 4);
        vlc.bits = 4 - (uint32_t)((vlc.tmp & 7) >> 2);
        vlc.unstuff = (b | 0x0F) > 0x8F;
    }
    {
        long num = 1 + (vlc.pos & 3);
        if (num > vlc.size) num = vlc.size;
        for (long i = 0; i < num; i++) {
            uint32_t b = 0;
            if (vlc.pos >= 0 && vlc.pos < len) { b = data[vlc.pos]; vlc.pos--; }
            const uint32_t dBits = (vlc.unstuff && (b & 0x7F) == 0x7F) ? 7 : 8;
            vlc.tmp |= shl64((uint64_t)b, vlc.bits);
            vlc.bits += dBits;
            vlc.unstuff = b > 0x8F;
        }
        vlc.size -= num;
        rev_read(vlc);
    }
    FwdStream ms{data, len, 0, lcup - scup, 0, 0, 0, 0xFF};
    for (int i = 0; i < 4; i++) {
        uint32_t b;
        if (ms.size > 0 && ms.pos < len) { b = data[ms.pos]; ms.pos++; ms.size--; } else b = 0xFF;
        const uint32_t dBits = ms.unstuff ? 7 : 8;
        ms.tmp |= shl64((uint64_t)b, ms.bits);
        ms.bits += dBits;
        ms.unstuff = (b == 0xFF);
    }
    fwd_read(ms);

    const int quadCols = (w + 3) / 4;
    for (int y = 0; y < h; y += 4) {
        const int initial = (y == 0);
        const uint16_t *tbl = initial ? c_vlc_tbl0 : c_vlc_tbl1;
        for (int qx = 0; qx < quadCols; qx += 2) {
            uint32_t vlcVal = rev_fetch(vlc);
            const uint32_t qinf = tbl[vlcVal & 0x7F];
            const uint32_t rho = (qinf >> 4) & 0xF, uOff1 = (qinf >> 3) & 1;
            rev_advance(vlc, qinf & 0xF);
            vlcVal = rev_fetch(vlc);
            const uint32_t qinf2 = tbl[((rho >> 2) << 7) | (vlcVal & 0x7F)];
            const uint32_t rho2 = (qinf2 >> 4) & 0xF, uOff2 = (qinf2 >> 3) & 1;
            rev_advance(vlc, qinf2 & 0xF);
            uint32_t u[2] = {1, 1};
            const uint32_t mode = (uOff1 << 1) | uOff2;
            if (mode > 0) {
                vlcVal = rev_fetch(vlc);
                rev_advance(vlc, decode_uvlc(vlcVal, mode, u, initial));
            }
            for (int q = 0; q < 2; q++) {
                const uint32_t r = q ? rho2 : rho, emb = u[q];
                const int base = (qx + q) * 4;
                for (int i = 0; i < 4 && base + i < w; i++) {
                    if (!((r >> i) & 1)) continue;
                    const uint32_t magVal = fwd_fetch(ms);
                    const uint32_t mag = (magVal & (shl32(1, emb) - 1)) + shl32(1, emb - 1);
                    fwd_advance(ms, emb);
                    const uint32_t sign = fwd_fetch(ms) & 1;
                    fwd_advance(ms, 1);
                    out[(size_t)y * (STRIDED ? (size_t)os_ : (size_t)w) + base + i] = sign ? (int32_t)(0u - mag) : (int32_t)mag;
                }
            }
        }
    }
}

static bool g_tables_ready[16] = {false};

static hipError_t ht_tables_ready(hipStream_t s) {
    int dev = 0;
    hipError_t e = hipGetDevice(&dev);
    if (e != hipSuccess) return e;
    if (dev < 0 || dev >= 16) return hipErrorInvalidDevice;
    if (g_tables_ready[dev]) return hipSuccess;
    hipLaunchKernelGGL(ht_build_enc_table, dim3(1), dim3(128), 0, s);
    hipLaunchKernelGGL(ht_build_pair_table, dim3(64), dim3(256), 0, s);
    if ((e = hipGetLastError()) != hipSuccess) return e;
    if ((e = hipFuncSetAttribute(reinterpret_cast<const void *>(ht_walk_kernel), hipFuncAttributeMaxDynamicSharedMemorySize,
                                 (int)sizeof(HtWalkShared))) != hipSuccess) return e;
    if ((e = hipStreamSynchronize(s)) != hipSuccess) return e;
    g_tables_ready[dev] = true;
    return hipSuccess;
}

hipError_t launch_ht_encode(hipStream_t s, const BlockJob *jobs, int njobs, const int32_t *coef, uint8_t *slots,
                            uint32_t *lens, uint8_t *numbps, int *fault, uint32_t *maglens, const HtUJob *utab, int nunique,
                            const int *alias_ids) {
    if (njobs <= 0) return hipSuccess;
    hipError_t e;
    if ((e = ht_tables_ready(s)) != hipSuccess) return e;
    const int n = utab ? nunique : njobs;
    hipLaunchKernelGGL(ht_encode_kernel, dim3(n), dim3(64), 0, s, jobs, n, coef, slots, lens, numbps, fault, maglens, utab, alias_ids);
    return hipGetLastError();
}

hipError_t launch_ht_encode_stream(hipStream_t s, const BlockJob *jobs, int njobs, const int32_t *coef, uint8_t *stream,
                                   uint64_t *offs, uint32_t *lens, uint8_t *numbps, uint64_t *status, uint32_t epoch, int *fault) {
    if (njobs <= 0) return hipSuccess;
    hipError_t e;
    if ((e = ht_tables_ready(s)) != hipSuccess) return e;
    hipLaunchKernelGGL(ht_encode_stream_kernel, dim3(njobs), dim3(64), 0, s, jobs, njobs, coef, stream,
                       reinterpret_cast<unsigned long long *>(offs), lens, numbps, reinterpret_cast<unsigned long long *>(status), epoch, fault);
    return hipGetLastError();
}
int ht_fast_max_samples() { return HT_FAST_MAX_SAMPLES; }

size_t ht_decode_scratch_words(int njobs) { return (size_t)njobs * (HT_WALK_REC + HT_VBITS_WORDS); }

hipError_t launch_ht_decode(hipStream_t s, const BlockJob *jobs, int njobs, const uint8_t *stream, const uint64_t *offs,
                            const uint32_t *lens, int32_t *decoded, uint32_t *scratch, int coded_rows_only, const BlockJob *placed_jobs) {
    if (njobs <= 0) return hipSuccess;
    hipError_t e;
    if ((e = ht_tables_ready(s)) != hipSuccess) return e;
    uint32_t *pairs = scratch, *vbits = scratch + (size_t)njobs * HT_WALK_REC;
    for (int rep_ = 0; rep_ < dev_reps(32); rep_++)
    hipLaunchKernelGGL(ht_vlcprep_kernel, dim3((njobs + 3) / 4), dim3(256), 0, s, jobs, njobs, stream, offs, lens, vbits, pairs);
    if ((e = hipGetLastError()) != hipSuccess) return e;
    for (int rep_ = 0; rep_ < dev_reps(64); rep_++)
    hipLaunchKernelGGL(ht_walk_kernel, dim3((njobs + HT_WALK_BLOCKS - 1) / HT_WALK_BLOCKS), dim3(256), sizeof(HtWalkShared), s, jobs, njobs, vbits, pairs);
    if ((e = hipGetLastError()) != hipSuccess) return e;
    for (int rep_ = 0; rep_ < dev_reps(128); rep_++)
    if (placed_jobs) hipLaunchKernelGGL(ht_decode_kernel<true>, dim3((njobs + 3) / 4), dim3(256), 0, s, placed_jobs, njobs, stream, offs, lens, decoded, pairs, 1);
    else
    hipLaunchKernelGGL(ht_decode_kernel<false>, dim3((njobs + 3) / 4), dim3(256), 0, s, jobs, njobs, stream, offs, lens, decoded, pairs, coded_rows_only);
    return hipGetLastError();
}

}
```

go-jpeg2000_amd/csrc/j2k_ctx.cpp:

```cpp
#include "j2k_host.h"

using namespace j2k;

int fail(j2k_ctx *ctx, int status, const char *msg) {
    if (ctx) ctx->last_error = msg ? msg : "";
    return status;
}
int fail_hip(j2k_ctx *ctx, hipError_t e, const char *where) {
    char buf[256];
    snprintf(buf, sizeof(buf), "%s: %s", where, hipGetErrorString(e));
    if (ctx) ctx->last_error = buf;
    return J2K_ERR_HIP;
}

extern "C" const char *j2k_ctx_last_error(j2k_ctx *ctx) { return ctx ? ctx->last_error.c_str() : ""; }

std::atomic<int> g_mq_ctxs{0};
bool mq_throughput_mode() { return g_mq_ctxs.load(std::memory_order_relaxed) >= 2; }
struct CtxOption { const char *name; bool (*set)(j2k_ctx *, long); };
static const std::vector<CtxOption> &ctx_options() {
#define OPT(name, cond, stmt) CtxOption{name, [](j2k_ctx *c, long v) -> bool { (void)c; if (!(cond)) return false; stmt; return true; }}
    static const std::vector<CtxOption> T = {
        OPT("plane_wg3", v == 0 || v == 1, c->plane_wg3 = v != 0),
        OPT("pix_fuse", v >= 0 && v <= 2, c->pix_fuse = (int)v),
        OPT("plane_wg", v == 0 || v == 4 || v == 8, c->plane_wg = (int)v),
        OPT("l0_fuse", v == 0 || v == 8 || v == 10 || v == 16, c->l0_fuse = (int)v),
        OPT("l0_wg", v == 0 || v == 4 || v == 8, c->l0_wg = (int)v),
        OPT("plane_wg97", v == 0 || v == 8, c->plane_wg97 = (int)v),
        OPT("l0_wg97_inv", v == 0 || v == 6 || v == 8 || v == 10 || v == 12, c->l0_wg97_inv = (int)v),
        OPT("l0_wg97", v == 0 || (v >= 6 && v <= 16 && v % 2 == 0), c->l0_wg97 = (int)v),
        OPT("l0_xcd", v == 0 || v == 1, c->l0_xcd = v != 0),
        OPT("l0_deal", v == 0 || v == 1, c->l0_deal = v != 0),
        OPT("ht_alias", v == 0 || v == 1, c->ht_alias = v != 0),
        OPT("l0_inv_wpe", v >= 5 && v <= 7, c->l0_inv_wpe = (int)v),
        OPT("l0_wg_inv", v == 0 || v == 1, c->l0_wg_inv = v != 0),
        OPT("l0_wg_invw", v == 0 || v == 4 || v == 8, c->l0_wg_invw = (int)v),
        OPT("l0_xcd_group", v >= 0 && v <= 4096, c->l0_xcd_group = (int)v),
        OPT("l0_store", v == 0 || v == 1 || v == 2 || v == 4, c->l0_store = (int)v),
        OPT("fuse_compact", v == 0 || v == 1, c->fuse_compact = v != 0),
        OPT("deep", v == 0 || v == 1, c->use_deep = v != 0),
        OPT("deep_min_planes", v >= 0 && v <= 1000000, c->deep_min_planes = (int)v),
        OPT("deep_mid", v == 0 || v == 1, c->deep_mid = v != 0),
        OPT("deep_mid_inv", v >= 0 && v <= 2, c->deep_mid_inv = (int)v),
        OPT("mega", v >= 0 && v <= 2, c->mega = (int)v),
        OPT("t1_split", v == 0 || v == 1, c->t1_split = v != 0),
        OPT("t1_sym_mb", v >= 0, c->t1_sym_mb = v),
        OPT("t1_dec_general", v == 0 || v == 1, c->t1_dec_general = v != 0),
        OPT("t1_dec_split", v >= -1, c->t1_dec_split = (int)v),
        OPT("t1_dec_lanes", v >= 0 && v <= 2, c->t1_dec_lanes = (int)v),
        OPT("t1_lanes", v >= 0 && v <= 64, c->t1_lanes = (int)v),
        OPT("t2_parallel", v == 0 || v == 1, c->t2_parallel = v != 0),
    };
#undef OPT
    return T;
}
extern "C" int j2k_ctx_set_option(j2k_ctx *ctx, const char *name, long value) {
    if (!ctx || !name) return J2K_ERR_INVALID_ARG;
    for (const CtxOption &o : ctx_options())
        if (!strcmp(o.name, name)) return o.set(ctx, value) ? J2K_OK : fail(ctx, J2K_ERR_INVALID_ARG, "j2k_ctx_set_option: value out of range");
    return fail(ctx, J2K_ERR_INVALID_ARG, "j2k_ctx_set_option: no such option");
}

extern "C" int j2k_ctx_create(int device, j2k_ctx **out) {
    if (!out) return J2K_ERR_INVALID_ARG;
    *out = nullptr;
    int n = 0;
    if (hipGetDeviceCount(&n) != hipSuccess || n <= 0) return J2K_ERR_NO_DEVICE;
    if (device < 0 || device >= n) return J2K_ERR_INVALID_ARG;
    if (hipSetDevice(device) != hipSuccess) return J2K_ERR_NO_DEVICE;
    j2k_ctx *ctx = new j2k_ctx();
    ctx->device = device;
    if (hipStreamCreateWithFlags(&ctx->stream, hipStreamNonBlocking) != hipSuccess) {
        delete ctx;
        return J2K_ERR_HIP;
    }
#ifdef J2K_DEV
    if (const char *e = getenv("J2K_DEV_SKIP")) j2k::g_dev_skip = (int)strtol(e, nullptr, 0);
    if (const char *e = getenv("J2K_DEV_DUP")) j2k::g_dev_dup = (int)strtol(e, nullptr, 0);
#endif
    if (j2k::tuning_env("J2K_TUNING"))
        for (const CtxOption &o : ctx_options()) {
            std::string var = "J2K_";
            for (const char *c = o.name; *c; c++) var += (char)toupper((unsigned char)*c);
            if (const char *e = getenv(var.c_str())) (void)o.set(ctx, atol(e));
        }
    *out = ctx;
    return J2K_OK;
}

extern "C" void j2k_ctx_destroy(j2k_ctx *ctx) {
    if (!ctx) return;
    if (ctx->counted_mq) g_mq_ctxs.fetch_sub(1, std::memory_order_relaxed);
    (void)hipSetDevice(ctx->device);
    (void)hipStreamSynchronize(ctx->stream);
    for (j2k_plan *p : ctx->cache) j2k_plan_destroy(p);
    for (int i = 0; i < 5; i++)
        if (ctx->stage[i]) (void)hipFree(ctx->stage[i]);
    for (hipEvent_t e : ctx->ev) (void)hipEventDestroy(e);
    (void)hipStreamDestroy(ctx->stream);
    delete ctx;
}

struct j2k_graph { j2k_ctx *ctx; hipGraph_t graph; hipGraphExec_t exec; bool arms_fault; };
extern "C" int j2k_ctx_capture_begin(j2k_ctx *ctx) {
    if (!ctx || ctx->capturing) return J2K_ERR_INVALID_ARG;
    HIPCHK(ctx, hipSetDevice(ctx->device));
    ctx->fault_armed_before_capture = ctx->fault_armed;
    HIPCHK(ctx, hipStreamBeginCapture(ctx->stream, hipStreamCaptureModeThreadLocal));
    ctx->capturing = true;
    return J2K_OK;
}
extern "C" int j2k_ctx_capture_end(j2k_ctx *ctx, j2k_graph **out) {
    if (!ctx || !out || !ctx->capturing) return J2K_ERR_INVALID_ARG;
    *out = nullptr;
    ctx->capturing = false;
    hipGraph_t g = nullptr;
    HIPCHK(ctx, hipStreamEndCapture(ctx->stream, &g));
    hipGraphExec_t ex = nullptr;
    hipError_t e = hipGraphInstantiate(&ex, g, nullptr, nullptr, 0);
    if (e != hipSuccess) { (void)hipGraphDestroy(g); return fail_hip(ctx, e, "hipGraphInstantiate"); }
    *out = new j2k_graph{ctx, g, ex, ctx->fault_armed};
    ctx->fault_armed = ctx->fault_armed_before_capture;
    return J2K_OK;
}
extern "C" int j2k_graph_launch(j2k_graph *G) {
    if (!G || !G->ctx || G->ctx->capturing) return J2K_ERR_INVALID_ARG;
    j2k_ctx *ctx = G->ctx;
    HIPCHK(ctx, hipSetDevice(ctx->device));
    HIPCHK(ctx, hipGraphLaunch(G->exec, ctx->stream));
    if (G->arms_fault) ctx->fault_armed = true;
    return J2K_OK;
}
extern "C" void j2k_graph_destroy(j2k_graph *G) {
    if (!G) return;
    if (G->ctx) { (void)hipSetDevice(G->ctx->device); (void)hipStreamSynchronize(G->ctx->stream); }
    if (G->exec) (void)hipGraphExecDestroy(G->exec);
    if (G->graph) (void)hipGraphDestroy(G->graph);
    delete G;
}

int check_fault(j2k_ctx *ctx) {
    if (ctx->capturing) return fail(ctx, J2K_ERR_INVALID_ARG, "a synchronising call while the context captures a graph");
    HIPCHK(ctx, hipStreamSynchronize(ctx->stream));
    if (!ctx->fault_armed || !ctx->stage[3]) return J2K_OK;
    int f = 0;
    HIPCHK(ctx, hipMemcpy(&f, ctx->stage[3], sizeof(int), hipMemcpyDeviceToHost));
    ctx->fault_armed = false;
    if (!f) return J2K_OK;
    HIPCHK(ctx, hipMemsetAsync(ctx->stage[3], 0, sizeof(int), ctx->stream));
    if (f == 1) return fail(ctx, J2K_ERR_GO_PANIC, "block coder: input on which the reference panics (stream buffer overrun / MinInt32)");
    if (f == 4) return fail(ctx, J2K_ERR_INVALID_ARG, "unpack_stream: the pack was not made by a plan of this geometry");
    return fail(ctx, J2K_ERR_GO_PANIC, "block coder: the block needs more bytes than the reference's own buffer holds (t1_fast5.go:47-56: index out of range)");
}

extern "C" int j2k_ctx_sync(j2k_ctx *ctx) {
    if (!ctx) return J2K_ERR_INVALID_ARG;
    return check_fault(ctx);
}
extern "C" void *j2k_ctx_stream(j2k_ctx *ctx) { return ctx ? (void *)ctx->stream : nullptr; }

extern "C" int j2k_ctx_profile_enable(j2k_ctx *ctx, int on) {
    if (!ctx) return J2K_ERR_INVALID_ARG;
    HIPCHK(ctx, hipSetDevice(ctx->device));
    HIPCHK(ctx, hipStreamSynchronize(ctx->stream));
    ctx->profile = on < 0 ? 0 : on;
    ctx->ev_used = 0;
    return J2K_OK;
}
extern "C" int j2k_ctx_profile_read(j2k_ctx *ctx, int64_t *launches, double *total_ms) {
    if (!ctx || !launches || !total_ms) return J2K_ERR_INVALID_ARG;
    HIPCHK(ctx, hipSetDevice(ctx->device));
    HIPCHK(ctx, hipStreamSynchronize(ctx->stream));
    double tot = 0;
    int64_t n = 0;
    for (size_t i = 0; i + 1 < ctx->ev_used; i += 2) {
        if (ctx->ev_tag[i / 2] != 0) continue;
        float ms = 0;
        HIPCHK(ctx, hipEventElapsedTime(&ms, ctx->ev[i], ctx->ev[i + 1]));
        tot += ms; n++;
    }
    *launches = n;
    *total_ms = tot;
    ctx->ev_used = 0;
    return J2K_OK;
}
extern "C" int j2k_ctx_profile_read_tag(j2k_ctx *ctx, int tag, int64_t *launches, double *total_ms) {
    if (!ctx || !launches || !total_ms) return J2K_ERR_INVALID_ARG;
    HIPCHK(ctx, hipSetDevice(ctx->device));
    HIPCHK(ctx, hipStreamSynchronize(ctx->stream));
    double tot = 0;
    int64_t n = 0;
    for (size_t i = 0; i + 1 < ctx->ev_used; i += 2) {
        if (ctx->ev_tag[i / 2] != tag) continue;
        float ms = 0;
        HIPCHK(ctx, hipEventElapsedTime(&ms, ctx->ev[i], ctx->ev[i + 1]));
        tot += ms; n++;
    }
    *launches = n;
    *total_ms = tot;
    return J2K_OK;
}
static hipEvent_t profile_event(j2k_ctx *ctx) {
    if (!ctx->profile || ctx->capturing || ctx->ev_used >= 8192) return nullptr;
    if (ctx->ev_used >= ctx->ev.size()) {
        hipEvent_t e;
        if (hipEventCreate(&e) != hipSuccess) return nullptr;
        ctx->ev.push_back(e);
    }
    return ctx->ev[ctx->ev_used++];
}
bool profile_pair(j2k_ctx *ctx, int tag, hipEvent_t &e0, hipEvent_t &e1) {
    e0 = e1 = nullptr;
    if (!ctx->profile || (tag != 0 && ctx->profile < 2) || ctx->capturing || ctx->ev_used + 2 > 8192) return false;
    const size_t pair = ctx->ev_used / 2;
    e0 = profile_event(ctx);
    e1 = e0 ? profile_event(ctx) : nullptr;
    if (!e1) { e0 = nullptr; ctx->ev_used = pair * 2; return false; }
    if (ctx->ev_tag.size() <= pair) ctx->ev_tag.resize(pair + 1, 0);
    ctx->ev_tag[pair] = tag;
    return true;
}

int stage_reserve(j2k_ctx *ctx, int slot, size_t bytes) {
    if (ctx->stage_bytes[slot] >= bytes) return J2K_OK;
    if (ctx->capturing) return fail(ctx, J2K_ERR_INVALID_ARG, "capture: a workspace would have to grow -- run the same calls once before j2k_ctx_capture_begin");
    if (ctx->stage[slot]) {
        HIPCHK(ctx, hipStreamSynchronize(ctx->stream));
        HIPCHK(ctx, hipFree(ctx->stage[slot]));
        ctx->stage[slot] = nullptr;
        ctx->stage_bytes[slot] = 0;
    }
    size_t cap = std::max<size_t>(bytes, 1 << 20);
    HIPCHK(ctx, hipMalloc(&ctx->stage[slot], cap));
    ctx->stage_bytes[slot] = cap;
    if (slot == 3) HIPCHK(ctx, hipMemsetAsync(ctx->stage[slot], 0, cap, ctx->stream));
    return J2K_OK;
}
```

go-jpeg2000_amd/csrc/j2k_host.h:

```cpp
#pragma once
#include <algorithm>
#include <atomic>
#include <cstdio>
#include <cstdlib>
#include <cstring>
#include <map>
#include <tuple>

#include "j2k_plan.h"

namespace j2k {
#ifdef J2K_DEV
int g_dev_skip = 0, g_dev_dup = 0;
#endif
hipError_t launch_add_const(hipStream_t s, int32_t *d, size_t n, int delta);
hipError_t launch_rct(hipStream_t s, int32_t *a, int32_t *b, int32_t *c, size_t n, int inverse);
hipError_t launch_ict(hipStream_t s, double *a, double *b, double *c, size_t n, int inverse);
hipError_t launch_dwt97_fwd(hipStream_t s, const LevelLaunch &L, const void *src, int src_is_f64, int32_t *out_i32,
                            double *out_f64, double *nxt, int dc_shift, int quant, double step, int mct);
hipError_t launch_dwt97_inv(hipStream_t s, const LevelLaunch &L, const void *coef, int coef_is_f64, const double *prev,
                            void *dst, int dc_shift, int final_level, int dst_mode, int mct, double step);
hipError_t launch_quantize97(hipStream_t s, const double *src, size_t n, double step, int32_t *dst);
hipError_t launch_dequantize97(hipStream_t s, const int32_t *src, size_t n, double step, double *dst);
hipError_t launch_ht_encode(hipStream_t s, const BlockJob *jobs, int njobs, const int32_t *coef, uint8_t *slots,
                            uint32_t *lens, uint8_t *numbps, int *fault, uint32_t *maglens = nullptr, const HtUJob *utab = nullptr, int nunique = 0,
                            const int *alias_ids = nullptr);
hipError_t launch_ht_decode(hipStream_t s, const BlockJob *jobs, int njobs, const uint8_t *stream, const uint64_t *offs,
                            const uint32_t *lens, int32_t *decoded, uint32_t *scratch, int coded_rows_only = 0, const BlockJob *placed_jobs = nullptr);
size_t ht_decode_scratch_words(int njobs);
hipError_t launch_ht_encode_stream(hipStream_t s, const BlockJob *jobs, int njobs, const int32_t *coef, uint8_t *stream,
                                   uint64_t *offs, uint32_t *lens, uint8_t *numbps, uint64_t *status, uint32_t epoch, int *fault);
int ht_fast_max_samples();
hipError_t launch_t1_encode(hipStream_t s, const BlockJob *jobs, int njobs, const int32_t *coef, uint8_t *slots,
                            uint32_t *lens, uint8_t *numbps, uint8_t *work, size_t work_per_job, int *fault, int max_dim,
                            uint8_t *sym, size_t sym_stride, uint32_t *nsyms, int lanes, uint8_t *bigsym = nullptr, const uint64_t *bigsym_off = nullptr,
                            uint32_t *bignsyms = nullptr);
size_t t1_sym_stride(int planes);
hipError_t launch_t1_decode(hipStream_t s, const BlockJob *jobs, int njobs, const uint8_t *stream, const uint64_t *offs,
                            const uint32_t *lens, const uint8_t *numbps, int32_t *decoded, uint8_t *work,
                            size_t work_per_job, int max_dim, int general_only, uint8_t *split_ws, int sig_lanes, int throughput = 0);
size_t t1_dec_split_bytes(size_t njobs);
hipError_t launch_mq_encode(hipStream_t s, const uint8_t *ctxs, const uint8_t *decs, size_t n, uint8_t *out, size_t cap, uint32_t *out_len, int *fault);
hipError_t launch_mq_decode(hipStream_t s, const uint8_t *data, size_t len, const uint8_t *ctxs, size_t n, uint8_t *decs, int *fault);
hipError_t launch_raw_encode(hipStream_t s, const uint8_t *bits, size_t n, uint8_t *out, size_t cap, uint32_t *out_len, int *fault);
hipError_t launch_raw_decode(hipStream_t s, const uint8_t *data, size_t len, size_t n, uint8_t *bits);
size_t t1_work_bytes(int w, int h);
size_t t1_flag_bytes(int w, int h);
hipError_t launch_compact(hipStream_t s, const BlockJob *jobs, int njobs, const uint8_t *slots, const uint32_t *lens,
                          uint64_t *offs, uint8_t *stream, const uint32_t *maglens, const uint32_t *mels = nullptr, uint64_t *toffs = nullptr);
hipError_t launch_mel_table(hipStream_t s, const BlockJob *jobs, int njobs, uint32_t *mels);
hipError_t launch_assemble_tiles(hipStream_t s, const uint8_t *stream, const uint64_t *offs, const int *job0, int ntiles, int tile_first,
                                 uint64_t max_tile_bytes, uint8_t *out, uint64_t *out_len);
size_t t2_chain_bytes();
hipError_t launch_t2_tile_chains(hipStream_t s, const uint8_t *cs, uint64_t len, const uint64_t *tile_offs, int ntiles, int tile_first,
                                 const int *tile_packet0, void *chains);
hipError_t launch_t2_decode_packets(hipStream_t s, void *chains, int nchains, const j2k_t2_dev_packet *packets, long npackets, j2k_t2_dev_cb *cbs, uint64_t ncbs,
                                    const uint8_t *data, int sop, int eph, int clean, uint64_t *body_base, int *frame_status);
void t2_make_chain(void *dst, uint64_t len, long npackets, const j2k_t2_dec_state &st);
void t2_read_chain(const void *src, j2k_t2_dec_state &st, int &status, long &done);
size_t t2_par_workspace(long npackets, int ntiles);
hipError_t launch_t2_decode_tiles(hipStream_t s, void *chains, int ntiles, const int *tile_packet0, const j2k_t2_dev_packet *packets, long npackets, j2k_t2_dev_cb *cbs,
                                  uint64_t ncbs, const uint8_t *data, uint64_t len, int sop, int eph, uint64_t *body_base, int *frame_status, void *ws,
                                  int ht, int mb, uint64_t *offs, uint32_t *lens, uint8_t *numbps);
hipError_t launch_t2_blocks(hipStream_t s, long n, const j2k_t2_dev_cb *cbs, int ht, int mb, uint64_t total, uint64_t *offs, uint32_t *lens, uint8_t *numbps, int *status);
hipError_t launch_place_blocks(hipStream_t s, const BlockJob *src_jobs, const BlockJob *dec_jobs, int njobs, int max_h, const int32_t *decoded, int32_t *coeff, int ystep = 1);
hipError_t launch_select_blocks(hipStream_t s, const int *ids, int m, const uint64_t *offs, const uint32_t *lens, const uint8_t *numbps, uint64_t *offs_r,
                                uint32_t *lens_r, uint8_t *numbps_r);
hipError_t launch_mallat_ll(hipStream_t s, const LLPlane *planes, int nplanes, int max_samples, const int32_t *coef, int32_t *frame, int lossy, double step,
                            int dc_shift);
hipError_t launch_scan(hipStream_t s, const uint32_t *lens, int njobs, uint64_t *offs, const uint32_t *mels, uint64_t *toffs);
size_t pack_header_bytes(size_t n);
hipError_t launch_pack(hipStream_t s, const BlockJob *jobs, int njobs, const uint8_t *stream, const uint64_t *offs, const uint64_t *toffs,
                       const uint32_t *lens, const uint8_t *numbps, const uint32_t *maglens, uint8_t *pack);
hipError_t launch_unpack(hipStream_t s, const BlockJob *jobs, int njobs, int count, const uint8_t *const *packs, const size_t *pack_bytes,
                         uint8_t *const *streams, size_t stream_cap, uint64_t *const *offs, uint32_t *const *lens, uint8_t *const *numbps, int *fault);
}

int fail(j2k_ctx *ctx, int status, const char *msg);
int fail_hip(j2k_ctx *ctx, hipError_t e, const char *where);
#define HIPCHK(ctx, call)                                      \
    do {                                                       \
        hipError_t e_ = (call);                                \
        if (e_ != hipSuccess) return fail_hip(ctx, e_, #call); \
    } while (0)
extern std::atomic<int> g_mq_ctxs;
bool mq_throughput_mode();
int check_fault(j2k_ctx *ctx);
bool profile_pair(j2k_ctx *ctx, int tag, hipEvent_t &e0, hipEvent_t &e1);
int stage_reserve(j2k_ctx *ctx, int slot, size_t bytes);

static inline int64_t align4(int64_t v) { return (v + 3) & ~int64_t(3); }
template <typename T>
static int upload(j2k_ctx *ctx, T **dptr, const std::vector<T> &v) {
    *dptr = nullptr;
    if (v.empty()) return J2K_OK;
    HIPCHK(ctx, hipMalloc((void **)dptr, v.size() * sizeof(T)));
    HIPCHK(ctx, hipMemcpy(*dptr, v.data(), v.size() * sizeof(T), hipMemcpyHostToDevice));
    return J2K_OK;
}
int build_plan(j2k_ctx *ctx, const j2k::PlanSpec &S, j2k_plan **out);
int cached_plan(j2k_ctx *ctx, const j2k::PlanSpec &S, j2k_plan **out);
void plan_t2_packets(const j2k_plan *P, int layer, std::vector<j2k_t2_dev_packet> &out, std::vector<int> *tile_packet0);
int plan_reduced(j2k_plan *P, int reduce, j2k::ReducedTab **out);

struct T1Workspace { size_t off_nsyms, off_sym, stride, total; };
T1Workspace t1_workspace(const j2k_ctx *ctx, size_t n, size_t wpj);
int ensure(j2k_ctx *ctx, void **p, size_t bytes);
struct PixIO { int stride = 0, single = 0, triple = 0; j2k::YccSrc ycc{}; };
int plan_forward_impl(j2k_plan *P, const void *d_frame, void *d_coeff, PixIO pix = PixIO());
int plan_encode_private_slots(j2k_plan *P, const int32_t *d_coeff, uint32_t *d_lens, uint8_t *d_numbps);
int plan_encode_frame_from_coeff(j2k_plan *P, const int32_t *d_coeff, uint32_t *d_lens, uint8_t *d_numbps, int sop, int eph, uint8_t *d_out, size_t cap,
                                 uint64_t *d_tile_offs);
int plan_inverse_impl(j2k_plan *P, const void *d_coeff, void *d_frame, PixIO pix = PixIO(), const int *guard = nullptr);
int plan_inverse_pixels_impl(j2k_plan *P, const int32_t *d_coeff, void *d_pix, size_t stride, const int *guard);
int plan_inverse_pixels_reduced_impl(j2k_plan *P, const int32_t *d_coeff, int reduce, void *d_pix, size_t stride, const int *guard);
int plan_decode_blocks_jobs(j2k_plan *P, const j2k::BlockJob *d_djobs, int n, const uint8_t *d_stream, const uint64_t *d_offs, const uint32_t *d_lens,
                            const uint8_t *d_numbps, int32_t *d_decoded, const j2k::BlockJob *d_placed);
bool plan_rgba8_wg_fusable(const j2k_plan *P);
int plan_forward_image_impl(j2k_plan *P, const j2k_image *d_img, int32_t *d_coeff, int *status_word);
int image_device_bytes(const j2k_image *img, uint64_t need[3]);
size_t image_layout(const j2k_image *img, const uint64_t need[3], size_t off[4]);
int image_upload(j2k_ctx *ctx, const j2k_image *img, const uint64_t need[3], uint8_t *dev, const size_t off[4], j2k_image *d_img);
```

go-jpeg2000_amd/csrc/j2k_plan.h:

```cpp
#pragma once
#include <string>
#include <vector>

#include "../../include/j2kgfx.h"
#include "j2k_internal.h"

struct j2k_ctx {
    int device = -1;
    hipStream_t stream = nullptr;
    std::string last_error;
    int fuse_compact = 0;
    int fwd_link = 1;
    int inv_link = 1;
    int pix_fuse = 1;
    bool plane_wg3 = false;
    int plane_wg = 4;
    int l0_fuse = 0;
    int l0_wg = 8;
    int l0_wg_invw = 4;
    bool l0_deal = true;
    int l0_wg97 = 8;
    int plane_wg97 = 8;
    int l0_wg97_inv = 8;
    int l0_xcd_group = 16;
    bool l0_xcd = true;
    bool ht_alias = true;
    int l0_inv_wpe = 5;
    bool l0_wg_inv = true;
    int l0_store = 1;
    int band_prows_pix = 3;
    int band_prows_97 = 8;
    int band_prows_inv = 0;
    int fwd_pf = 0;
    int band_prows = 5;
    int use_tail = 1;
    int mega = 0;
    int deep_mid_inv = 1;
    int deep_min_planes = 12;
    int deep_mid = 1;
    int use_deep = 1;
    int xcd_map = 0;
    int cpl0 = 0;
    int force_novec = 0;
    int t1_split = 1;
    long t1_sym_mb = 8192;
    int t1_dec_general = 0;
    int t1_dec_lanes = 2;
    int t1_dec_split = -1;
    bool capturing = false;
    bool fault_armed_before_capture = false;
    bool counted_mq = false;
    bool t2_parallel = true;
    int t1_lanes = 0;
    std::vector<j2k_plan *> cache;
    void *stage[5] = {nullptr, nullptr, nullptr, nullptr, nullptr};
    bool fault_armed = false;
    size_t stage_bytes[5] = {0, 0, 0, 0, 0};
    int profile = 0;
    std::vector<hipEvent_t> ev;
    std::vector<int> ev_tag;
    size_t ev_used = 0;
};

namespace j2k {

enum Wavelet { W53 = 0, W97 = 1 };
enum QuantMode {
    Q_NONE = 0,
    Q_ENCODER = 1,
    Q_TCD = 2
};

struct PlanSpec {
    int W = 0, H = 0, C = 1;
    int tile_w = 0, tile_h = 0;
    int levels = 1;
    int wavelet = W53;
    int precision = 8;
    int dc_shift = 0;
    int dc_shift_inv = 0;
    int mct = 0;
    int quant = Q_NONE;
    int quality = 100;
    int num_res_jobs = 6;
    int cb_w = 64, cb_h = 64;
    int coder = J2K_CODER_MQ;
    int frame_h = 0;
    int tile_first = 0, tile_count = 0;
    bool frame_is_f64 = false;
    bool closed_loop = false;
    bool mallat = false;
    bool operator==(const PlanSpec &o) const;
};

struct Group {
    int tile;
    int comp0, nc;
    int x0, y0, w, h;
    int64_t coef_off[3];
    int64_t scrA_off[3], scrB_off[3];
};

struct LevelTab {
    DwtPlane *d_planes = nullptr;
    DwtJob *d_jobs = nullptr;
    int njobs = 0, nplanes = 0;
    int cpl = 2, vec = 0, ncomp = 1;
    int64_t alg_bytes = 0;
    DwtJob *d_pjobs = nullptr;
    int pnjobs = 0, pwaves = 0, pmulti = 0;
    bool p_pix_only = false;
    bool mallat = false;
};

struct ReducedTab {
    bool built = false;
    int Wr = 0, Hr = 0;
    LevelTab inv[2];
    LLPlane *d_ll = nullptr;
    int nll = 0, ll_samples = 0;
    int njobs = 0, max_block_h = 0;
    int *d_ids = nullptr;
    BlockJob *d_bjobs = nullptr, *d_djobs = nullptr, *d_placed = nullptr;
    uint64_t *d_offs = nullptr; uint32_t *d_lens = nullptr; uint8_t *d_numbps = nullptr;
};

}

struct j2k_plan {
    j2k_ctx *ctx = nullptr;
    j2k::PlanSpec spec;
    int tiles_x = 1, tiles_y = 1, tile_first = 0, tile_count = 1;
    std::vector<j2k::Group> groups;
    std::vector<int64_t> plane_desc;
    int64_t coeff_elems = 0, scrA_elems = 0, scrB_elems = 0;
    std::vector<j2k::LevelTab> fwd[2], inv[2];
    void *d_scrA = nullptr, *d_scrB = nullptr;
    int tail_l0 = -1;
    j2k::TailPlane *d_tail = nullptr;
    int ntail = 0;
    size_t tail_lds_fwd = 0, tail_lds_inv = 0;
    int deep_l0 = -1;
    j2k::TailPlane *d_deep_planes = nullptr;
    j2k::DwtJob *d_deep_jobs = nullptr;
    int ndeep_jobs = 0;
    size_t deep_lds = 0, deep_lds_fwd = 0;
    std::vector<j2k::DwtJob> deep_jobs_host, deep_jobs_host_inv, flat_jobs_host, flat_jobs_host_inv;
    j2k::DwtJob *d_deep_jobs_inv = nullptr;
    int ndeep_jobs_inv = 0;
    j2k::DwtJob *d_mega_fwd_jobs = nullptr, *d_mega_inv_jobs = nullptr, *d_fwd_top_jobs = nullptr, *d_inv_top_jobs = nullptr;
    int mega_fwd_njobs = 0, mega_inv_njobs = 0, fwd_top_njobs = 0, inv_top_njobs = 0;
    int64_t fwd_top_bytes = 0, inv_top_bytes = 0;
    std::vector<j2k_block> blocks;
    std::vector<int32_t> block_tile;
    std::vector<int32_t> block_res;
    j2k_t2_dev_packet *d_t2_packets = nullptr;
    int *d_tile_packet0 = nullptr;
    int t2_npackets = 0;
    j2k_t2_dev_cb *d_t2_cbs = nullptr;
    uint64_t *d_t2_poffs = nullptr;
    int t2_body_slices = 8;
    int32_t *d_t2_ptile = nullptr;
    void *d_t2_ws = nullptr;
    void *d_t2_chains = nullptr;
    uint64_t *d_t2_body_base = nullptr;
    void *d_t2_par = nullptr;
    int *d_frame_status = nullptr;
    int32_t *d_cl_decoded = nullptr, *d_cl_coeff = nullptr;
    int32_t *d_cl_coeff_dec = nullptr;
    uint8_t *d_cl_numbps = nullptr; uint64_t *d_cl_offs = nullptr; uint32_t *d_cl_lens = nullptr;
    int max_block_h = 0;
    void *d_host_io = nullptr, *d_host_pix = nullptr;
    size_t host_io_bytes = 0, host_pix_bytes = 0;
    int *d_tile_job0 = nullptr;
    uint64_t max_tile_bytes = 0;
    std::vector<uint64_t> slot_off;
    std::vector<uint64_t> dec_off;
    j2k::BlockJob *d_bjobs = nullptr;
    j2k::BlockJob *d_djobs = nullptr;
    j2k::BlockJob *d_djobs_placed = nullptr;
    int64_t bytes_cap = 0, decoded_elems = 0, block_samples = 0;
    int64_t dwt_bytes = 0, dwt_level0_bytes = 0;
    void *d_frame = nullptr, *d_coeff = nullptr, *d_slots = nullptr, *d_stream = nullptr;
    void *d_lens = nullptr, *d_numbps = nullptr, *d_offs = nullptr;
    j2k::DwtJob *d_fwd_pix_jobs = nullptr;
    int fwd_pix_njobs = 0;
    j2k::HtUJob *d_ht_ujobs = nullptr; int *d_ht_alias_next = nullptr;
    j2k::BlockJob *d_bjobs_alias = nullptr;
    int ht_nunique = 0;
    j2k::DwtJob *d_fwd97_wg_jobs = nullptr;
    int fwd97_wg_njobs = 0, fwd97_wg_waves = 0;
    j2k::DwtJob *d_inv97_wg_jobs = nullptr;
    int inv97_wg_njobs = 0, inv97_wg_waves = 0;
    j2k::DwtJob *d_fwd_wg2_jobs = nullptr, *d_fwd_wg_rest_jobs = nullptr;
    int fwd_wg2_njobs = 0, fwd_wg2_waves = 0, fwd_wg_rest_njobs = 0;
    j2k::DwtJob *d_fwd_wg_jobs = nullptr;
    int fwd_wg_njobs = 0, fwd_wg_waves = 0;
    j2k::DwtJob *d_inv_wg_jobs = nullptr;
    int inv_wg_njobs = 0, inv_wg_waves = 0;
    uint32_t *d_maglens = nullptr;
    uint32_t *d_mels = nullptr;
    const void *last_stream = nullptr, *last_lens = nullptr;
    bool want_toffs = false, toffs_valid = false;
    uint64_t *d_toffs = nullptr;
    uint64_t *d_status = nullptr;
    uint32_t epoch = 0;
    bool all_blocks_fast = false;
    uint64_t *d_bigsym_off = nullptr;
    size_t bigsym_total = 0;
    bool dec_coded_rows_only = false;
    std::vector<j2k::ReducedTab> reduced;
    bool dequantize = false;
};
```

go-jpeg2000_amd/csrc/j2k_stages.cpp:

```cpp
#include "j2k_host.h"

using namespace j2k;

static LevelLaunch mk(const LevelTab &T, int pf = 0) {
    LevelLaunch L{T.d_jobs, T.njobs, T.d_planes, T.cpl, T.vec, T.ncomp, pf};
    L.pjobs = T.d_pjobs; L.pnjobs = T.p_pix_only ? 0 : T.pnjobs; L.pwaves = T.pwaves; L.pmulti = T.pmulti;
    L.mallat = T.mallat ? 1 : 0;
    return L;
}

static void pix_launch(LevelLaunch &L, const LevelTab &T, const PixIO &pix, int cls, const PlanSpec &S) {
    L.pix_stride = pix.stride;
    L.pix_src = cls ? (pix.triple == 4 ? 4 : 0) : pix.single;
    L.comp_elems = (long long)S.W * S.H;
    if (cls == 1 && pix.triple == 4) L.pnjobs = T.pnjobs;
}

int plan_forward_impl(j2k_plan *P, const void *d_frame, void *d_coeff, PixIO pix) {
    const int pix_stride = pix.stride;
    j2k_ctx *ctx = P->ctx;
    const PlanSpec &S = P->spec;
    if (((uintptr_t)d_frame & 15) || ((uintptr_t)d_coeff & 15)) return fail(ctx, J2K_ERR_INVALID_ARG, "device pointers must be 16-byte aligned");
    HIPCHK(ctx, hipSetDevice(ctx->device));
    const double step = 1.0 / (double)S.quality;
    const int nlevel_launches = (P->deep_l0 >= 0) ? P->deep_l0 : ((P->tail_l0 >= 0) ? P->tail_l0 : S.levels);
    bool fused_l1 = false;
    bool mega = false;
    for (int l = 0; l < nlevel_launches; l++)
    for (int rep_ = 0; rep_ < dev_reps(l == 0 ? 1 : (l == 1 ? 2 : 4)); rep_++) {
        if (l == 1 && fused_l1) continue;
        void *in = (l == 0) ? const_cast<void *>(d_frame) : ((l & 1) ? P->d_scrA : P->d_scrB);
        void *nx = (l & 1) ? P->d_scrB : P->d_scrA;
        const int prof_cls = P->fwd[1][0].njobs ? 1 : 0;
        for (int cls = 0; cls < 2; cls++) {
            const LevelTab &T = P->fwd[cls][l];
            if (!T.njobs) continue;
            hipEvent_t ev0 = nullptr, ev1 = nullptr;
            if (l == 0 ? cls == prof_cls : S.wavelet == W53) profile_pair(ctx, l == 0 ? 0 : 1, ev0, ev1);
            if (S.wavelet == W53) {
                LevelLaunch L = mk(T, ctx->fwd_pf);
                if (l == 0 && pix_stride > 0) {
                    pix_launch(L, T, pix, cls, S);
                    const bool rgba8 = cls == 1 && pix.triple == 8;
                    if (rgba8 && P->d_fwd_pix_jobs) { L.jobs = P->d_fwd_pix_jobs; L.njobs = P->fwd_pix_njobs; }
                    if (rgba8 && P->d_fwd_wg_jobs) {
                        L.jobs = P->d_fwd_wg_jobs; L.njobs = P->fwd_wg_njobs; L.wg_waves = P->fwd_wg_waves; L.wg_store = ctx->l0_store;
                        L.ycc = pix.ycc;
                        if (P->d_mega_fwd_jobs && !P->d_fwd_wg2_jobs) {
                            L.jobs = P->d_fwd_top_jobs; L.njobs = P->fwd_top_njobs;
                            mega = true;
                        }
                        if (P->d_fwd_wg2_jobs) {
                            L.jobs2 = P->d_fwd_wg2_jobs; L.njobs2 = P->fwd_wg2_njobs; L.wg2_waves = P->fwd_wg2_waves;
                            L.jobs = P->d_fwd_wg_rest_jobs; L.njobs = P->fwd_wg_rest_njobs;
                            L.planes1 = P->fwd[0][1].d_planes; L.nxt1 = (int32_t *)P->d_scrB;
                            fused_l1 = true;
                        }
                    }
                }
                if (ev1) { L.ev_start = ev0; L.ev_stop = ev1; }
                HIPCHK(ctx, launch_dwt53_fwd(ctx->stream, L, (const int32_t *)in, (int32_t *)d_coeff, (int32_t *)nx, l == 0 ? S.dc_shift : 0));
            } else {
                const int src_f64 = (l > 0) || S.frame_is_f64;
                LevelLaunch L97 = mk(T);
                if (l == 0 && cls == 0 && pix.single == 97) L97.pix_stride = pix.stride;
                if (l == 0 && cls == prof_cls && ev1) { L97.ev_start = ev0; L97.ev_stop = ev1; }
                if (l == 0 && cls == 1 && !src_f64 && P->d_fwd97_wg_jobs) {
                    L97.jobs = P->d_fwd97_wg_jobs; L97.njobs = P->fwd97_wg_njobs; L97.wg_waves = P->fwd97_wg_waves;
                    if (pix.triple == 97) L97.pix_stride = pix.stride;
                }
                HIPCHK(ctx, launch_dwt97_fwd(ctx->stream, L97, in, src_f64, (int32_t *)d_coeff, (double *)d_coeff, (double *)nx,
                                             l == 0 ? S.dc_shift : 0, S.quant, step, (cls == 1) ? 1 : 0));
            }
        }
    }
    for (int rep_ = 0; mega && rep_ < dev_reps(4); rep_++) {
        hipEvent_t e0, e1;
        profile_pair(ctx, 1, e0, e1);
        HIPCHK(ctx, launch_dwt53_mega_fwd(ctx->stream, P->d_mega_fwd_jobs, P->mega_fwd_njobs, P->d_deep_planes, P->fwd[1][0].d_planes, P->deep_lds_fwd,
                                          (const int32_t *)P->d_scrA, (int32_t *)d_coeff, (const uint32_t *)d_frame, (int32_t *)P->d_scrA,
                                          S.dc_shift, pix_stride, e0, e1));
    }
    for (int rep_ = 0; !mega && P->deep_l0 >= 0 && rep_ < dev_reps(4); rep_++) {
        hipEvent_t e0, e1;
        profile_pair(ctx, 1, e0, e1);
        HIPCHK(ctx, launch_dwt53_deep_fwd(ctx->stream, P->d_deep_jobs, P->ndeep_jobs, P->d_deep_planes, P->deep_lds_fwd,
                                          (const int32_t *)((P->deep_l0 & 1) ? P->d_scrA : P->d_scrB), (int32_t *)d_coeff, e0, e1));
    }
    for (int rep_ = 0; P->deep_l0 < 0 && P->tail_l0 >= 0 && rep_ < dev_reps(4); rep_++) {
        hipEvent_t e0, e1;
        profile_pair(ctx, 1, e0, e1);
        HIPCHK(ctx, launch_dwt53_tail_fwd(ctx->stream, P->d_tail, P->ntail, P->tail_lds_fwd,
                                          (const int32_t *)((P->tail_l0 & 1) ? P->d_scrA : P->d_scrB), (int32_t *)d_coeff, e0, e1));
    }
    return J2K_OK;
}

int plan_inverse_impl(j2k_plan *P, const void *d_coeff, void *d_frame, PixIO pix, const int *guard) {
    const int pix_stride = pix.stride;
    j2k_ctx *ctx = P->ctx;
    const PlanSpec &S = P->spec;
    if (((uintptr_t)d_frame & 15) || ((uintptr_t)d_coeff & 15)) return fail(ctx, J2K_ERR_INVALID_ARG, "device pointers must be 16-byte aligned");
    HIPCHK(ctx, hipSetDevice(ctx->device));
    const double dq_step = (P->dequantize && S.quant == Q_ENCODER) ? 1.0 / (double)S.quality : 1.0;
    const bool mega = P->d_mega_inv_jobs && pix.triple == 8 && pix_stride > 0 && ctx->l0_wg_inv && S.wavelet == W53 && !guard;
    for (int rep_ = 0; mega && rep_ < dev_reps(0x100); rep_++) {
        hipEvent_t e0, e1;
        profile_pair(ctx, 3, e0, e1);
        HIPCHK(ctx, launch_dwt53_mega_inv(ctx->stream, P->d_mega_inv_jobs, P->mega_inv_njobs, P->d_deep_planes, P->inv[1][0].d_planes, P->deep_lds,
                                          (const int32_t *)d_coeff, (int32_t *)P->d_scrA, (const int32_t *)P->d_scrA, (uint32_t *)d_frame,
                                          S.dc_shift_inv, pix_stride, e0, e1));
    }
    for (int rep_ = 0; !mega && P->deep_l0 >= 0 && rep_ < dev_reps(0x100); rep_++) {
        hipEvent_t e0, e1;
        profile_pair(ctx, 3, e0, e1);
        HIPCHK(ctx, launch_dwt53_deep_inv(ctx->stream, P->d_deep_jobs_inv, P->ndeep_jobs_inv, P->d_deep_planes, P->deep_lds, (const int32_t *)d_coeff,
                                          (int32_t *)((P->deep_l0 & 1) ? P->d_scrA : P->d_scrB), e0, e1));
    }
    for (int rep_ = 0; P->deep_l0 < 0 && P->tail_l0 >= 0 && rep_ < dev_reps(0x100); rep_++) {
        hipEvent_t e0, e1;
        profile_pair(ctx, 3, e0, e1);
        HIPCHK(ctx, launch_dwt53_tail_inv(ctx->stream, P->d_tail, P->ntail, P->tail_lds_inv, (const int32_t *)d_coeff,
                                          (int32_t *)((P->tail_l0 & 1) ? P->d_scrA : P->d_scrB), e0, e1));
    }
    for (int l = ((P->deep_l0 >= 0) ? P->deep_l0 : ((P->tail_l0 >= 0) ? P->tail_l0 : S.levels)) - 1; l >= 0; l--)
    for (int rep_ = 0; rep_ < dev_reps(l == 0 ? 0x400 : (l == 1 ? 0x200 : 0x100)); rep_++) {
        void *prev = (l & 1) ? P->d_scrB : P->d_scrA;
        void *dst = (l == 0) ? d_frame : ((l & 1) ? P->d_scrA : P->d_scrB);
        for (int ci = 0; ci < 2; ci++) {
            const int cls = (l == 0 && pix_stride > 0) ? 1 - ci : ci;
            const LevelTab &T = P->inv[cls][l];
            if (!T.njobs) continue;
            if (S.wavelet == W53) {
                LevelLaunch L = mk(T);
                if (l == 0) L.guard = guard;
                if (l == 0 && pix_stride > 0) pix_launch(L, T, pix, cls, S);
                if (l == 0 && cls == 1 && pix.triple == 8 && pix_stride > 0 && P->d_inv_wg_jobs && ctx->l0_wg_inv) {
                    L.jobs = P->d_inv_wg_jobs; L.njobs = P->inv_wg_njobs; L.wg_waves = P->inv_wg_waves; L.wg_store = ctx->l0_inv_wpe;
                    if (mega) { L.jobs = P->d_inv_top_jobs; L.njobs = P->inv_top_njobs; }
                }
                profile_pair(ctx, l == 0 ? 2 : 3, L.ev_start, L.ev_stop);
                HIPCHK(ctx, launch_dwt53_inv(ctx->stream, L, (const int32_t *)d_coeff, (const int32_t *)prev, (int32_t *)dst,
                                             l == 0 ? S.dc_shift_inv : 0, l == 0));
            } else {
                const int dst_mode = (l > 0) ? 0 : (S.frame_is_f64 ? 1 : 2);
                LevelLaunch L97 = mk(T);
                if (l == 0 && pix_stride > 0) L97.guard = guard;
                if (l == 0 && cls == 0 && pix.single == 97) L97.pix_stride = pix.stride;
                if (l == 0 && cls == 1 && dst_mode == 2 && P->d_inv97_wg_jobs) {
                    L97.jobs = P->d_inv97_wg_jobs; L97.njobs = P->inv97_wg_njobs; L97.wg_waves = P->inv97_wg_waves;
                    if (pix.triple == 97) L97.pix_stride = pix.stride;
                }
                HIPCHK(ctx, launch_dwt97_inv(ctx->stream, L97, d_coeff, S.quant == Q_NONE ? 1 : 0, (const double *)prev, dst,
                                             l == 0 ? S.dc_shift_inv : 0, l == 0, dst_mode, (cls == 1) ? 1 : 0, dq_step));
            }
        }
    }
    return J2K_OK;
}

static int plan_inverse_reduced_impl(j2k_plan *P, const void *d_coeff, int reduce, int32_t *d_frame) {
    j2k_ctx *ctx = P->ctx;
    const PlanSpec &S = P->spec;
    if (((uintptr_t)d_frame & 15) || ((uintptr_t)d_coeff & 15)) return fail(ctx, J2K_ERR_INVALID_ARG, "device pointers must be 16-byte aligned");
    ReducedTab *R = nullptr;
    int r = plan_reduced(P, reduce, &R);
    if (r != J2K_OK) return r;
    HIPCHK(ctx, hipSetDevice(ctx->device));
    const double dq_step = (P->dequantize && S.quant == Q_ENCODER) ? 1.0 / (double)S.quality : 1.0;
    if (reduce == S.levels) {
        HIPCHK(ctx, launch_mallat_ll(ctx->stream, R->d_ll, R->nll, R->ll_samples, (const int32_t *)d_coeff, d_frame, S.wavelet == W97 ? 1 : 0, dq_step, S.dc_shift_inv));
        return J2K_OK;
    }
    for (int l = S.levels - 1; l >= reduce; l--) {
        const bool fin = l == reduce;
        void *prev = (l & 1) ? P->d_scrB : P->d_scrA;
        void *dst = fin ? (void *)d_frame : ((l & 1) ? P->d_scrA : P->d_scrB);
        for (int cls = 0; cls < 2; cls++) {
            const LevelTab &T = fin ? R->inv[cls] : P->inv[cls][l];
            if (!T.njobs) continue;
            LevelLaunch L = mk(T);
            if (S.wavelet == W53) {
                profile_pair(ctx, 3, L.ev_start, L.ev_stop);
                HIPCHK(ctx, launch_dwt53_inv(ctx->stream, L, (const int32_t *)d_coeff, (const int32_t *)prev, (int32_t *)dst, fin ? S.dc_shift_inv : 0, fin));
            } else {
                HIPCHK(ctx, launch_dwt97_inv(ctx->stream, L, d_coeff, S.quant == Q_NONE ? 1 : 0, (const double *)prev, dst, fin ? S.dc_shift_inv : 0, fin,
                                             fin ? 2 : 0, (cls == 1) ? 1 : 0, dq_step));
            }
        }
    }
    return J2K_OK;
}

extern "C" int j2k_plan_inverse_reduced(j2k_plan *P, const int32_t *d_coeff, int reduce, int32_t *d_frame) {
    if (!P || !d_frame || !d_coeff) return J2K_ERR_INVALID_ARG;
    ReducedTab *R = nullptr;
    int r = plan_reduced(P, reduce, &R);
    if (r != J2K_OK) return r;
    if (reduce == 0) return plan_inverse_impl(P, d_coeff, d_frame);
    return plan_inverse_reduced_impl(P, d_coeff, reduce, d_frame);
}

extern "C" int j2k_plan_forward(j2k_plan *P, const int32_t *d_frame, int32_t *d_coeff) {
    if (!P || !d_frame || !d_coeff) return J2K_ERR_INVALID_ARG;
    return plan_forward_impl(P, d_frame, d_coeff);
}
extern "C" int j2k_plan_inverse(j2k_plan *P, const int32_t *d_coeff, int32_t *d_frame) {
    if (!P || !d_frame || !d_coeff) return J2K_ERR_INVALID_ARG;
    return plan_inverse_impl(P, d_coeff, d_frame);
}

int ensure(j2k_ctx *ctx, void **p, size_t bytes) {
    if (*p) return J2K_OK;
    HIPCHK(ctx, hipMalloc(p, std::max<size_t>(bytes, 16)));
    return J2K_OK;
}

static int coder_call(j2k_ctx *ctx, int which, const uint8_t *a, size_t na, const uint8_t *b, size_t nb, size_t n, uint8_t *out, size_t cap,
                      size_t *out_len) {
    HIPCHK(ctx, hipSetDevice(ctx->device));
    const size_t na16 = (na + 15) & ~size_t(15);
    int r = stage_reserve(ctx, 0, na16 + nb + 64);
    if (r == J2K_OK) r = stage_reserve(ctx, 1, cap + 64);
    if (r == J2K_OK) r = stage_reserve(ctx, 3, 256);
    if (r != J2K_OK) return r;
    uint8_t *d_a = (uint8_t *)ctx->stage[0], *d_b = d_a + na16, *d_out = (uint8_t *)ctx->stage[1];
    int *d_fault = (int *)ctx->stage[3] + 16;
    uint32_t *d_len = (uint32_t *)ctx->stage[3] + 20;
    HIPCHK(ctx, hipMemsetAsync(d_fault, 0, 32, ctx->stream));
    if (na) HIPCHK(ctx, hipMemcpyAsync(d_a, a, na, hipMemcpyHostToDevice, ctx->stream));
    if (nb) HIPCHK(ctx, hipMemcpyAsync(d_b, b, nb, hipMemcpyHostToDevice, ctx->stream));
    switch (which) {
    case 0: HIPCHK(ctx, launch_mq_encode(ctx->stream, d_a, d_b, n, d_out, cap, d_len, d_fault)); break;
    case 1: HIPCHK(ctx, launch_mq_decode(ctx->stream, d_a, na, d_b, n, d_out, d_fault)); break;
    case 2: HIPCHK(ctx, launch_raw_encode(ctx->stream, d_a, n, d_out, cap, d_len, d_fault)); break;
    default: HIPCHK(ctx, launch_raw_decode(ctx->stream, d_a, na, n, d_out)); break;
    }
    int h[8] = {0};
    HIPCHK(ctx, hipMemcpyAsync(h, d_fault, 32, hipMemcpyDeviceToHost, ctx->stream));
    HIPCHK(ctx, hipStreamSynchronize(ctx->stream));
    if (h[0] == 3) return fail(ctx, J2K_ERR_GO_PANIC, "context index out of range (the Go coder panics)");
    if (h[0] == 2) return fail(ctx, J2K_ERR_CAPACITY, "output buffer too small");
    const size_t produced = (which == 0 || which == 2) ? (size_t)(uint32_t)h[4] : n;
    if (out_len) *out_len = produced;
    if (produced) HIPCHK(ctx, hipMemcpy(out, d_out, std::min(produced, cap), hipMemcpyDeviceToHost));
    return J2K_OK;
}

extern "C" int j2k_mq_encode(j2k_ctx *ctx, const uint8_t *ctxs, const uint8_t *decisions, size_t n, uint8_t *out, size_t cap, size_t *out_len) {
    if (!ctx || !out_len || (n && (!ctxs || !decisions)) || (cap && !out)) return J2K_ERR_INVALID_ARG;
    return coder_call(ctx, 0, ctxs, n, decisions, n, n, out, cap, out_len);
}
extern "C" int j2k_mq_decode(j2k_ctx *ctx, const uint8_t *data, size_t len, const uint8_t *ctxs, size_t n, uint8_t *decisions) {
    if (!ctx || (len && !data) || (n && (!ctxs || !decisions))) return J2K_ERR_INVALID_ARG;
    return coder_call(ctx, 1, data, len, ctxs, n, n, decisions, n, nullptr);
}
extern "C" int j2k_raw_encode(j2k_ctx *ctx, const uint8_t *bits, size_t n, uint8_t *out, size_t cap, size_t *out_len) {
    if (!ctx || !out_len || (n && !bits) || (cap && !out)) return J2K_ERR_INVALID_ARG;
    return coder_call(ctx, 2, bits, n, nullptr, 0, n, out, cap, out_len);
}
extern "C" int j2k_raw_decode(j2k_ctx *ctx, const uint8_t *data, size_t len, size_t n, uint8_t *bits) {
    if (!ctx || (len && !data) || (n && !bits)) return J2K_ERR_INVALID_ARG;
    return coder_call(ctx, 3, data, len, nullptr, 0, n, bits, n, nullptr);
}

static const int kPixComp[6] = {1, 1, 3, 3, 4, 4}, kPixPrec[6] = {8, 16, 8, 16, 8, 16}, kPixBytes[6] = {1, 2, 4, 8, 4, 8};
extern "C" int j2k_pixels_components(int format) { return (format >= 0 && format < 6) ? kPixComp[format] : 0; }
extern "C" int j2k_pixels_precision(int format) { return (format >= 0 && format < 6) ? kPixPrec[format] : 0; }

static int pix_args_ok(j2k_ctx *ctx, int format, const void *pix, size_t stride, int w, int h, int target_precision) {
    if (!ctx || !pix || format < 0 || format >= 6 || w < 0 || h < 0 || target_precision < 0 || target_precision > 16)
        return J2K_ERR_INVALID_ARG;
    if (stride < (size_t)w * kPixBytes[format]) return J2K_ERR_INVALID_ARG;
    return J2K_OK;
}

extern "C" int j2k_unpack_pixels(j2k_ctx *ctx, int format, const void *d_pix, size_t stride, int w, int h, int target_precision,
                                 int32_t *d_planes) {
    int r = pix_args_ok(ctx, format, d_pix, stride, w, h, target_precision);
    if (r != J2K_OK || !d_planes) return ctx ? fail(ctx, J2K_ERR_INVALID_ARG, "j2k_unpack_pixels: bad argument") : J2K_ERR_INVALID_ARG;
    if ((format == J2K_PIX_RGBA8 || format == J2K_PIX_NRGBA8) && (((uintptr_t)d_pix | stride) & 3))
        return fail(ctx, J2K_ERR_INVALID_ARG, "RGBA rows must be 4-byte aligned");
    HIPCHK(ctx, hipSetDevice(ctx->device));
    const int src_max = (1 << kPixPrec[format]) - 1;
    const int dst_max = (target_precision > 0 && target_precision != kPixPrec[format]) ? (1 << target_precision) - 1 : src_max;
    HIPCHK(ctx, launch_unpack_pixels(ctx->stream, (const uint8_t *)d_pix, stride, format, w, h, src_max, dst_max, d_planes));
    return J2K_OK;
}

extern "C" int j2k_pack_pixels(j2k_ctx *ctx, const int32_t *d_planes, int ncomp, int precision, int w, int h, void *d_pix, size_t stride) {
    if (!ctx || !d_planes || !d_pix || w < 0 || h < 0 || precision < 1 || precision > 16) return J2K_ERR_INVALID_ARG;
    if (ncomp != 1 && ncomp != 3 && ncomp != 4) return fail(ctx, J2K_ERR_UNSUPPORTED, "unsupported number of components");
    const size_t bpp = (ncomp == 1 ? 1 : 4) * (precision > 8 ? 2 : 1);
    if (stride < (size_t)w * bpp) return fail(ctx, J2K_ERR_INVALID_ARG, "stride smaller than a row");
    if (ncomp != 1 && precision <= 8 && (((uintptr_t)d_pix | stride) & 3)) return fail(ctx, J2K_ERR_INVALID_ARG, "RGBA rows must be 4-byte aligned");
    HIPCHK(ctx, hipSetDevice(ctx->device));
    HIPCHK(ctx, launch_pack_pixels(ctx->stream, d_planes, ncomp, precision, w, h, (uint8_t *)d_pix, stride));
    return J2K_OK;
}

extern "C" int j2k_extract_image_data(j2k_ctx *ctx, int format, const void *pix, size_t stride, int w, int h, int target_precision,
                                      int32_t *const *planes) {
    int r = pix_args_ok(ctx, format, pix, stride, w, h, target_precision);
    if (r != J2K_OK || !planes) return ctx ? fail(ctx, J2K_ERR_INVALID_ARG, "j2k_extract_image_data: bad argument") : J2K_ERR_INVALID_ARG;
    const size_t n = (size_t)w * h;
    if (!n) return J2K_OK;
    const int nc = kPixComp[format];
    const size_t pbytes = (((size_t)h * stride) + 15) & ~size_t(15);
    HIPCHK(ctx, hipSetDevice(ctx->device));
    r = stage_reserve(ctx, 0, pbytes + 64);
    if (r == J2K_OK) r = stage_reserve(ctx, 1, n * 4 * nc + 64);
    if (r != J2K_OK) return r;
    HIPCHK(ctx, hipMemcpyAsync(ctx->stage[0], pix, (size_t)(h - 1) * stride + (size_t)w * kPixBytes[format], hipMemcpyHostToDevice, ctx->stream));
    r = j2k_unpack_pixels(ctx, format, ctx->stage[0], stride, w, h, target_precision, (int32_t *)ctx->stage[1]);
    if (r != J2K_OK) return r;
    for (int c = 0; c < nc; c++)
        HIPCHK(ctx, hipMemcpyAsync(planes[c], (int32_t *)ctx->stage[1] + (size_t)c * n, n * 4, hipMemcpyDeviceToHost, ctx->stream));
    HIPCHK(ctx, hipStreamSynchronize(ctx->stream));
    return J2K_OK;
}

extern "C" int j2k_create_image(j2k_ctx *ctx, const int32_t *const *planes, int ncomp, int precision, int w, int h, void *pix, size_t stride) {
    if (!ctx || !planes || !pix || w < 0 || h < 0 || precision < 1 || precision > 16) return J2K_ERR_INVALID_ARG;
    if (ncomp != 1 && ncomp != 3 && ncomp != 4) return fail(ctx, J2K_ERR_UNSUPPORTED, "unsupported number of components");
    const size_t n = (size_t)w * h;
    if (!n) return J2K_OK;
    const size_t bpp = (ncomp == 1 ? 1 : 4) * (precision > 8 ? 2 : 1);
    if (stride < (size_t)w * bpp) return fail(ctx, J2K_ERR_INVALID_ARG, "stride smaller than a row");
    HIPCHK(ctx, hipSetDevice(ctx->device));
    int r = stage_reserve(ctx, 0, (size_t)h * stride + 64);
    if (r == J2K_OK) r = stage_reserve(ctx, 1, n * 4 * ncomp + 64);
    if (r != J2K_OK) return r;
    for (int c = 0; c < ncomp; c++)
        HIPCHK(ctx, hipMemcpyAsync((int32_t *)ctx->stage[1] + (size_t)c * n, planes[c], n * 4, hipMemcpyHostToDevice, ctx->stream));
    r = j2k_pack_pixels(ctx, (const int32_t *)ctx->stage[1], ncomp, precision, w, h, ctx->stage[0], stride);
    if (r != J2K_OK) return r;
    HIPCHK(ctx, hipMemcpy2DAsync(pix, stride, ctx->stage[0], stride, (size_t)w * bpp, (size_t)h, hipMemcpyDeviceToHost, ctx->stream));
    HIPCHK(ctx, hipStreamSynchronize(ctx->stream));
    return J2K_OK;
}

static bool cs_applies(int cs, int ncomp) {
    switch (cs) {
    case J2K_CS_CMYK: case J2K_CS_YCCK: return ncomp >= 4;
    case J2K_CS_SYCC: case J2K_CS_EYCC: case J2K_CS_YCBCR2: case J2K_CS_YCBCR3: case J2K_CS_PHOTOYCC: case J2K_CS_CMY:
    case J2K_CS_CIELAB: case J2K_CS_CIEJAB: case J2K_CS_ESRGB: case J2K_CS_ROMMRGB: case J2K_CS_YPBPR60: case J2K_CS_YPBPR50:
        return ncomp >= 3;
    default: return false;
    }
}

extern "C" int j2k_convert_colorspace_device(j2k_ctx *ctx, int cs, int32_t *d_planes, int ncomp, size_t n, int precision) {
    if (!ctx || (n && !d_planes) || ncomp < 0 || precision < 1 || precision > 31) return J2K_ERR_INVALID_ARG;
    if (!cs_applies(cs, ncomp) || !n) return J2K_OK;
    HIPCHK(ctx, hipSetDevice(ctx->device));
    HIPCHK(ctx, launch_colorspace(ctx->stream, cs, d_planes, ncomp, n, precision));
    return J2K_OK;
}

extern "C" int j2k_convert_colorspace(j2k_ctx *ctx, int cs, int32_t *const *planes, int ncomp, size_t n, int precision) {
    if (!ctx || (n && ncomp > 0 && !planes) || ncomp < 0 || precision < 1 || precision > 31) return J2K_ERR_INVALID_ARG;
    if (!cs_applies(cs, ncomp) || !n) return J2K_OK;
    const int nc = (cs == J2K_CS_CMYK || cs == J2K_CS_YCCK) ? 4 : 3;
    HIPCHK(ctx, hipSetDevice(ctx->device));
    int r = stage_reserve(ctx, 0, n * 4 * nc + 64);
    if (r != J2K_OK) return r;
    int32_t *d = (int32_t *)ctx->stage[0];
    for (int c = 0; c < nc; c++) HIPCHK(ctx, hipMemcpyAsync(d + (size_t)c * n, planes[c], n * 4, hipMemcpyHostToDevice, ctx->stream));
    HIPCHK(ctx, launch_colorspace(ctx->stream, cs, d, nc, n, precision));
    for (int c = 0; c < 3; c++) HIPCHK(ctx, hipMemcpyAsync(planes[c], d + (size_t)c * n, n * 4, hipMemcpyDeviceToHost, ctx->stream));
    HIPCHK(ctx, hipStreamSynchronize(ctx->stream));
    return J2K_OK;
}

static bool pix_fusable(const j2k_plan *P, int bps, int channels, const void *d_pix, size_t stride, bool inverse, PixIO &io) {
    const PlanSpec &S = P->spec;
    const int prec = 8 * bps, pb = bps * channels;
    if (S.wavelet == W97) {
        if (P->ctx->pix_fuse != 1 || bps != 1 || S.frame_is_f64 || S.precision != 8 || S.quant != Q_ENCODER) return false;
        if ((inverse ? S.dc_shift_inv : S.dc_shift) != 128 || S.levels < 1 || (S.W % 8)) return false;
        if ((((uintptr_t)d_pix | stride) & 15) || stride < (size_t)S.W * (size_t)channels) return false;
        const LevelTab &T0 = (inverse ? P->inv : P->fwd)[0][0], &T1 = (inverse ? P->inv : P->fwd)[1][0];
        if (channels == 1 && S.C == 1) {
            if (!T0.njobs || T1.njobs || !(T0.pnjobs > 0 && T0.pwaves == 8)) return false;
            io = PixIO();
            io.stride = (int)stride;
            io.single = 97;
            return true;
        }
        if (channels != 4 || S.C != 3 || !S.mct) return false;
        if (inverse ? !(P->d_inv97_wg_jobs && P->inv97_wg_waves == 8) : !(P->d_fwd97_wg_jobs && P->fwd97_wg_waves == 8)) return false;
        if (T0.njobs) return false;
        io = PixIO();
        io.stride = (int)(stride / 4);
        io.triple = 97;
        return true;
    }
    if (S.wavelet != W53 || S.levels < 1 || S.precision != prec || (inverse ? S.dc_shift_inv : S.dc_shift) != (1 << (prec - 1))) return false;
    if (P->tail_l0 == 0 || (S.W % 8)) return false;
    if (P->ctx->pix_fuse == 0 || (P->ctx->pix_fuse == 2 && !(bps == 1 && channels == 4 && S.C == 3) && !(bps == 2 && channels == 1))) return false;
    if ((((uintptr_t)d_pix | stride) & 15) || stride < (size_t)S.W * pb) return false;
    const LevelTab &T0 = (inverse ? P->inv : P->fwd)[0][0], &T1 = (inverse ? P->inv : P->fwd)[1][0];
    if (!T0.njobs && !T1.njobs) return false;
    io = PixIO();
    io.stride = (int)(stride / pb);
    if (T0.njobs) {
        io.single = channels == 1 ? (bps == 2 ? 1 : 2) : (bps == 2 ? 4 : 3);
        const bool wg = T0.pnjobs > 0 && !T0.p_pix_only;
        if (io.single == 1 ? !(wg || (T0.vec && T0.cpl == 8 && !S.mallat)) : !(wg && T0.pwaves == 4)) return false;
        if (io.single == 1 && T1.njobs) return false;
    }
    if (T1.njobs) {
        if (channels != 4 || !S.mct) return false;
        if (bps == 1) {
            if (!T1.vec || T1.cpl != 8) return false;
            if (S.mallat && (inverse ? !(P->d_inv_wg_jobs && P->ctx->l0_wg_inv && P->ctx->l0_inv_wpe == 5) : !(P->d_fwd_wg_jobs && P->ctx->l0_store == 1))) return false;
            io.triple = 8;
        }
        else { if (!T1.pnjobs || T1.pwaves != 4) return false; io.triple = 4; }
    }
    if (inverse && channels == 4 && !T1.njobs && S.C != 4) return false;
    if (inverse && channels == 4 && T0.njobs && !(T1.njobs && S.C - 3 <= 1)) return false;
    return true;
}

bool plan_rgba8_wg_fusable(const j2k_plan *P) {
    const PlanSpec &S = P->spec;
    PixIO io;
    const void *aligned = reinterpret_cast<const void *>(uintptr_t(256));
    if (S.mallat) return false;
    if (S.C != 3 || !S.mct || !pix_fusable(P, 1, 4, aligned, (size_t)S.W * 4, false, io) || io.triple != 8) return false;
    return P->d_fwd_wg_jobs && !P->d_fwd_wg2_jobs && !P->d_mega_fwd_jobs && P->ctx->l0_store == 1 && !P->fwd[0][0].njobs;
}

static int plan_pack_pixels(j2k_plan *P, const int32_t *d_planes, int ncomp, int precision, void *d_pix, size_t stride, const int *guard = nullptr) {
    j2k_ctx *ctx = P->ctx;
    const PlanSpec &S = P->spec;
    if (P->tile_count == P->tiles_x * P->tiles_y && !guard) return j2k_pack_pixels(ctx, d_planes, ncomp, precision, S.W, S.H, d_pix, stride);
    int r = j2k_pack_pixels(ctx, d_planes, ncomp, precision, S.W, 0, d_pix, stride);
    if (r != J2K_OK) return r;
    if (P->tile_count == P->tiles_x * P->tiles_y) {
        HIPCHK(ctx, launch_pack_pixels_rect(ctx->stream, d_planes, ncomp, precision, S.W, S.H, 0, 0, S.W, S.H, (uint8_t *)d_pix, stride, guard));
        return J2K_OK;
    }
    size_t i = 0;
    while (i < P->groups.size()) {
        const Group &a = P->groups[i];
        int x1 = a.x0 + a.w;
        size_t k = i + 1;
        for (; k < P->groups.size() && (P->groups[k].tile == a.tile || (P->groups[k].y0 == a.y0 && P->groups[k].x0 >= x1)); k++) x1 = std::max(x1, P->groups[k].x0 + P->groups[k].w);
        HIPCHK(ctx, launch_pack_pixels_rect(ctx->stream, d_planes, ncomp, precision, S.W, S.H, a.x0, a.y0, x1 - a.x0, a.h, (uint8_t *)d_pix, stride, guard));
        i = k;
    }
    return J2K_OK;
}

static int plan_pack_pixels_reduced(j2k_plan *P, const ReducedTab &R, int reduce, const int32_t *d_planes, void *d_pix, size_t stride, const int *guard) {
    j2k_ctx *ctx = P->ctx;
    const PlanSpec &S = P->spec;
    const bool whole = P->tile_count == P->tiles_x * P->tiles_y;
    if (whole && !guard) return j2k_pack_pixels(ctx, d_planes, S.C, S.precision, R.Wr, R.Hr, d_pix, stride);
    int r = j2k_pack_pixels(ctx, d_planes, S.C, S.precision, R.Wr, 0, d_pix, stride);
    if (r != J2K_OK) return r;
    if (whole) {
        HIPCHK(ctx, launch_pack_pixels_rect(ctx->stream, d_planes, S.C, S.precision, R.Wr, R.Hr, 0, 0, R.Wr, R.Hr, (uint8_t *)d_pix, stride, guard));
        return J2K_OK;
    }
    const int m = (1 << reduce) - 1;
    int last_tile = -1;
    for (const Group &g : P->groups) {
        if (g.tile == last_tile) continue;
        last_tile = g.tile;
        HIPCHK(ctx, launch_pack_pixels_rect(ctx->stream, d_planes, S.C, S.precision, R.Wr, R.Hr, g.x0 >> reduce, g.y0 >> reduce, (g.w + m) >> reduce, (g.h + m) >> reduce,
                                            (uint8_t *)d_pix, stride, guard));
    }
    return J2K_OK;
}

int plan_inverse_pixels_reduced_impl(j2k_plan *P, const int32_t *d_coeff, int reduce, void *d_pix, size_t stride, const int *guard) {
    if (!P || !d_pix || !d_coeff) return J2K_ERR_INVALID_ARG;
    j2k_ctx *ctx = P->ctx;
    const PlanSpec &S = P->spec;
    ReducedTab *R = nullptr;
    int r = plan_reduced(P, reduce, &R);
    if (r != J2K_OK) return r;
    if (reduce == 0) return plan_inverse_pixels_impl(P, d_coeff, d_pix, stride, guard);
    r = stage_reserve(ctx, 0, (size_t)R->Wr * R->Hr * S.C * 4 + 64);
    if (r != J2K_OK) return r;
    r = plan_inverse_reduced_impl(P, d_coeff, reduce, (int32_t *)ctx->stage[0]);
    if (r != J2K_OK) return r;
    return plan_pack_pixels_reduced(P, *R, reduce, (const int32_t *)ctx->stage[0], d_pix, stride, guard);
}
extern "C" int j2k_plan_inverse_pixels_reduced(j2k_plan *P, const int32_t *d_coeff, int reduce, void *d_pix, size_t stride) {
    return plan_inverse_pixels_reduced_impl(P, d_coeff, reduce, d_pix, stride, nullptr);
}

extern "C" int j2k_plan_forward_rgba8(j2k_plan *P, const void *d_pix, size_t stride, int32_t *d_coeff) {
    if (!P || !d_pix || !d_coeff) return J2K_ERR_INVALID_ARG;
    j2k_ctx *ctx = P->ctx;
    const PlanSpec &S = P->spec;
    if (S.C != 3) return fail(ctx, J2K_ERR_INVALID_ARG, "j2k_plan_forward_rgba8 needs a 3-component plan");
    if (stride < (size_t)S.W * 4 || (((uintptr_t)d_pix | stride) & 3)) return fail(ctx, J2K_ERR_INVALID_ARG, "bad RGBA8 stride / alignment");
    PixIO io;
    if (S.mct && pix_fusable(P, 1, 4, d_pix, stride, false, io)) return plan_forward_impl(P, d_pix, d_coeff, io);
    int r = stage_reserve(ctx, 0, (size_t)S.W * S.H * 3 * 4 + 64);
    if (r != J2K_OK) return r;
    r = j2k_unpack_pixels(ctx, J2K_PIX_RGBA8, d_pix, stride, S.W, S.H, 0, (int32_t *)ctx->stage[0]);
    if (r != J2K_OK) return r;
    return plan_forward_impl(P, ctx->stage[0], d_coeff);
}

extern "C" int j2k_plan_inverse_rgba8(j2k_plan *P, const int32_t *d_coeff, void *d_pix, size_t stride) {
    if (!P || !d_pix || !d_coeff) return J2K_ERR_INVALID_ARG;
    j2k_ctx *ctx = P->ctx;
    const PlanSpec &S = P->spec;
    if (S.C != 3) return fail(ctx, J2K_ERR_INVALID_ARG, "j2k_plan_inverse_rgba8 needs a 3-component plan");
    if (S.dc_shift_inv != 128) return fail(ctx, J2K_ERR_UNSUPPORTED, "j2k_plan_inverse_rgba8 needs an unsigned 8-bit plan");
    if (stride < (size_t)S.W * 4 || (((uintptr_t)d_pix | stride) & 3)) return fail(ctx, J2K_ERR_INVALID_ARG, "bad RGBA8 stride / alignment");
    PixIO io;
    if (S.mct && pix_fusable(P, 1, 4, d_pix, stride, true, io)) return plan_inverse_impl(P, d_coeff, d_pix, io);
    int r = stage_reserve(ctx, 0, (size_t)S.W * S.H * 3 * 4 + 64);
    if (r != J2K_OK) return r;
    r = plan_inverse_impl(P, d_coeff, ctx->stage[0]);
    if (r != J2K_OK) return r;
    return plan_pack_pixels(P, (const int32_t *)ctx->stage[0], 3, 8, d_pix, stride);
}

extern "C" int j2k_plan_forward_pixels(j2k_plan *P, int format, const void *d_pix, size_t stride, int32_t *d_coeff) {
    if (!P || !d_pix || !d_coeff) return J2K_ERR_INVALID_ARG;
    j2k_ctx *ctx = P->ctx;
    const PlanSpec &S = P->spec;
    if (format < 0 || format >= 6) return fail(ctx, J2K_ERR_INVALID_ARG, "unknown pixel format");
    if (kPixComp[format] != S.C) return fail(ctx, J2K_ERR_INVALID_ARG, "pixel format and plan disagree on the component count");
    if (stride < (size_t)S.W * kPixBytes[format]) return fail(ctx, J2K_ERR_INVALID_ARG, "pixel stride shorter than a row");
    PixIO io;
    if (pix_fusable(P, kPixPrec[format] / 8, S.C == 1 ? 1 : 4, d_pix, stride, false, io)) return plan_forward_impl(P, d_pix, d_coeff, io);
    int r = stage_reserve(ctx, 0, (size_t)S.W * S.H * S.C * 4 + 64);
    if (r != J2K_OK) return r;
    r = j2k_unpack_pixels(ctx, format, d_pix, stride, S.W, S.H, S.precision, (int32_t *)ctx->stage[0]);
    if (r != J2K_OK) return r;
    return plan_forward_impl(P, ctx->stage[0], d_coeff);
}

extern "C" int j2k_plan_pixels_fused(const j2k_plan *P, int format, const void *d_pix, size_t stride, int inverse) {
    if (!P || !d_pix) return J2K_ERR_INVALID_ARG;
    const PlanSpec &S = P->spec;
    PixIO io;
    if (inverse) return ((S.precision == 8 || S.precision == 16) && pix_fusable(P, S.precision / 8, S.C == 1 ? 1 : 4, d_pix, stride, true, io)) ? 1 : 0;
    if (format < 0 || format >= 6 || kPixComp[format] != S.C) return J2K_ERR_INVALID_ARG;
    return pix_fusable(P, kPixPrec[format] / 8, S.C == 1 ? 1 : 4, d_pix, stride, false, io) ? 1 : 0;
}

extern "C" int j2k_plan_inverse_pixels(j2k_plan *P, const int32_t *d_coeff, void *d_pix, size_t stride) {
    return plan_inverse_pixels_impl(P, d_coeff, d_pix, stride, nullptr);
}
int plan_inverse_pixels_impl(j2k_plan *P, const int32_t *d_coeff, void *d_pix, size_t stride, const int *guard) {
    if (!P || !d_pix || !d_coeff) return J2K_ERR_INVALID_ARG;
    j2k_ctx *ctx = P->ctx;
    const PlanSpec &S = P->spec;
    PixIO io;
    if ((S.precision == 8 || S.precision == 16) && pix_fusable(P, S.precision / 8, S.C == 1 ? 1 : 4, d_pix, stride, true, io))
        return plan_inverse_impl(P, d_coeff, d_pix, io, guard);
    int r = stage_reserve(ctx, 0, (size_t)S.W * S.H * S.C * 4 + 64);
    if (r != J2K_OK) return r;
    r = plan_inverse_impl(P, d_coeff, ctx->stage[0]);
    if (r != J2K_OK) return r;
    return plan_pack_pixels(P, (const int32_t *)ctx->stage[0], S.C, S.precision, d_pix, stride, guard);
}

T1Workspace t1_workspace(const j2k_ctx *ctx, size_t n, size_t wpj) {
    const long limit_mb = ctx->t1_sym_mb;
    const int split = ctx->t1_split;
    T1Workspace W{};
    W.off_nsyms = (wpj * n + 255) & ~size_t(255);
    W.off_sym = (W.off_nsyms + (2 * n + 64) * 4 + 255) & ~size_t(255);
    W.stride = 0;
    if (split && n) {
        int planes = 31;
        const size_t limit = (size_t)limit_mb << 20;
        while (planes >= 8 && j2k::t1_sym_stride(planes) * n > limit) planes--;
        if (planes >= 8) W.stride = j2k::t1_sym_stride(planes);
    }
    W.total = W.off_sym + W.stride * n + 256;
    return W;
}

static size_t t1_work_per_job(const j2k_plan *P) {
    size_t m = 0;
    for (const j2k_block &b : P->blocks) m = std::max(m, t1_work_bytes(b.w, b.h));
    return (m + 255) & ~size_t(255);
}

extern "C" int j2k_plan_encode_blocks(j2k_plan *P, const int32_t *d_coeff, uint8_t *d_slots, uint32_t *d_lens, uint8_t *d_numbps) {
    if (!P || !d_coeff || !d_slots || !d_lens || !d_numbps) return J2K_ERR_INVALID_ARG;
    j2k_ctx *ctx = P->ctx;
    HIPCHK(ctx, hipSetDevice(ctx->device));
    const int n = (int)P->blocks.size();
    if (!n) return J2K_OK;
    int r = stage_reserve(ctx, 3, 256);
    if (r != J2K_OK) return r;
    int *d_fault = (int *)ctx->stage[3];
    ctx->fault_armed = true;
    if (P->spec.coder == J2K_CODER_HT) {
        HIPCHK(ctx, launch_ht_encode(ctx->stream, P->d_bjobs, n, d_coeff, d_slots, d_lens, d_numbps, d_fault));
    } else {
        int max_dim = 0;
        for (const j2k_block &b : P->blocks) max_dim = std::max(max_dim, std::max(b.w, b.h));
        const size_t wpj = max_dim > 64 ? t1_work_per_job(P) : 0;
        const T1Workspace W = t1_workspace(ctx, (size_t)n, wpj);
        r = stage_reserve(ctx, 2, W.total);
        if (r != J2K_OK) return r;
        uint8_t *ws = (uint8_t *)ctx->stage[2];
        uint8_t *bigsym = nullptr;
        uint32_t *bignsyms = nullptr;
        if (max_dim > 64 && (mq_throughput_mode() || j2k::tuning_env("J2K_T1_BIG_SPLIT")) && !(ctx->capturing && !P->d_bigsym_off)) {
            if (!P->d_bigsym_off) {
                std::vector<uint64_t> off((size_t)n + 1, 0);
                uint64_t room = 16;
                if (const char *en = j2k::tuning_env("J2K_T1_BIG_SYM_ROOM")) { const long v = atol(en); if (v >= 1 && v <= 64) room = (uint64_t)v; }
                for (int j = 0; j < n; j++) {
                    const j2k_block &b = P->blocks[(size_t)j];
                    const bool big = (b.w > 64 || b.h > 64) && b.w <= 256 && b.h <= 256;
                    off[(size_t)j + 1] = off[(size_t)j] + (big ? ((room * b.w * b.h + 255) & ~uint64_t(255)) : 0);
                }
                r = upload(ctx, &P->d_bigsym_off, off);
                if (r != J2K_OK) return r;
                P->bigsym_total = (size_t)off[(size_t)n];
            }
            const size_t head = ((size_t)n * 4 + 255) & ~size_t(255);
            if (P->bigsym_total && stage_reserve(ctx, 4, head + P->bigsym_total + 256) == J2K_OK) {
                bignsyms = (uint32_t *)ctx->stage[4];
                bigsym = (uint8_t *)ctx->stage[4] + head;
            }
        }
        HIPCHK(ctx, launch_t1_encode(ctx->stream, P->d_bjobs, n, d_coeff, d_slots, d_lens, d_numbps, ws, wpj, d_fault, max_dim,
                                     W.stride ? ws + W.off_sym : nullptr, W.stride, (uint32_t *)(ws + W.off_nsyms),
                                     ctx->t1_lanes > 0 ? ctx->t1_lanes : (mq_throughput_mode() ? -1 : 0), bigsym, P->d_bigsym_off, bignsyms));
    }
    return J2K_OK;
}

int plan_encode_private_slots(j2k_plan *P, const int32_t *d_coeff, uint32_t *d_lens, uint8_t *d_numbps) {
    j2k_ctx *ctx = P->ctx;
    const int n = (int)P->blocks.size();
    if (!P->d_slots) {
        if (ctx->capturing) return fail(ctx, J2K_ERR_INVALID_ARG, "capture: run the same calls once before j2k_ctx_capture_begin");
        HIPCHK(ctx, hipMalloc(&P->d_slots, (size_t)P->bytes_cap + 64));
    }
    if (P->spec.coder != J2K_CODER_HT) return j2k_plan_encode_blocks(P, d_coeff, (uint8_t *)P->d_slots, d_lens, d_numbps);
    if (!P->d_maglens) {
        if (ctx->capturing) return fail(ctx, J2K_ERR_INVALID_ARG, "capture: run the same calls once before j2k_ctx_capture_begin");
        HIPCHK(ctx, hipMalloc((void **)&P->d_maglens, (size_t)n * 4));
        HIPCHK(ctx, hipMalloc((void **)&P->d_mels, (size_t)n * 4));
        HIPCHK(ctx, hipMalloc((void **)&P->d_toffs, ((size_t)n + 1) * 8));
        HIPCHK(ctx, launch_mel_table(ctx->stream, P->d_bjobs, n, P->d_mels));
    }
    int r = stage_reserve(ctx, 3, 256);
    if (r != J2K_OK) return r;
    ctx->fault_armed = true;
    for (int rep_ = 0; rep_ < dev_reps(8); rep_++)
    HIPCHK(ctx, launch_ht_encode(ctx->stream, P->d_bjobs, n, d_coeff, (uint8_t *)P->d_slots, d_lens, d_numbps, (int *)ctx->stage[3],
                                 P->d_maglens, P->d_ht_ujobs, P->ht_nunique, P->d_ht_alias_next));
    return J2K_OK;
}

extern "C" int j2k_plan_encode_stream(j2k_plan *P, const int32_t *d_coeff, uint8_t *d_stream, uint64_t *d_offs, uint32_t *d_lens,
                                      uint8_t *d_numbps) {
    if (!P || !d_coeff || !d_stream || !d_offs || !d_lens || !d_numbps) return J2K_ERR_INVALID_ARG;
    j2k_ctx *ctx = P->ctx;
    HIPCHK(ctx, hipSetDevice(ctx->device));
    const int n = (int)P->blocks.size();
    if (!n) { HIPCHK(ctx, hipMemsetAsync(d_offs, 0, 8, ctx->stream)); return J2K_OK; }
    bool fused = P->spec.coder == J2K_CODER_HT && ctx->fuse_compact;
    if (fused && ctx->capturing)
        return fail(ctx, J2K_ERR_UNSUPPORTED, "capture: the one-kernel HT path (J2K_FUSE_COMPACT=1) cannot be replayed from a graph -- unset it");
    if (fused && !P->d_status) {
        P->all_blocks_fast = true;
        for (const j2k_block &b : P->blocks)
            if ((int64_t)((b.h + 3) / 4) * b.w > ht_fast_max_samples()) P->all_blocks_fast = false;
        if (P->all_blocks_fast) {
            if (ctx->capturing) return fail(ctx, J2K_ERR_INVALID_ARG, "capture: run the same calls once before j2k_ctx_capture_begin");
            HIPCHK(ctx, hipMalloc((void **)&P->d_status, (size_t)n * 8));
            HIPCHK(ctx, hipMemsetAsync(P->d_status, 0, (size_t)n * 8, ctx->stream));
        }
    }
    if (fused && P->all_blocks_fast && P->d_status) {
        int r = stage_reserve(ctx, 3, 256);
        if (r != J2K_OK) return r;
        if ((++P->epoch & 0x3FFFFF) == 0) {
            HIPCHK(ctx, hipMemsetAsync(P->d_status, 0, (size_t)n * 8, ctx->stream));
            P->epoch = 1;
        }
        ctx->fault_armed = true;
        HIPCHK(ctx, launch_ht_encode_stream(ctx->stream, P->d_bjobs, n, d_coeff, d_stream, d_offs, d_lens, d_numbps, P->d_status,
                                            P->epoch, (int *)ctx->stage[3]));
        return J2K_OK;
    }
    int r = plan_encode_private_slots(P, d_coeff, d_lens, d_numbps);
    if (r != J2K_OK) return r;
    if (P->spec.coder == J2K_CODER_HT) {
        for (int rep_ = 0; rep_ < dev_reps(16); rep_++)
        HIPCHK(ctx, launch_compact(ctx->stream, P->d_bjobs_alias ? P->d_bjobs_alias : P->d_bjobs, n, (const uint8_t *)P->d_slots, d_lens, d_offs, d_stream, P->d_maglens,
                                   P->want_toffs ? P->d_mels : nullptr, P->want_toffs ? P->d_toffs : nullptr));
        P->toffs_valid = P->want_toffs;
        P->last_stream = d_stream; P->last_lens = d_lens;
        return J2K_OK;
    }
    return j2k_plan_compact(P, (const uint8_t *)P->d_slots, d_lens, d_offs, d_stream);
}

extern "C" size_t j2k_plan_pack_bound(const j2k_plan *P) {
    if (!P) return 0;
    return pack_header_bytes(P->blocks.size()) + (size_t)P->bytes_cap + 64;
}

extern "C" size_t j2k_plan_tile_parts_bound(const j2k_plan *P) {
    return P ? (size_t)P->bytes_cap + 14 * (size_t)P->tile_count : 0;
}
extern "C" int j2k_plan_assemble_tiles_device(j2k_plan *P, const uint8_t *d_stream, const uint64_t *d_offs, uint8_t *d_out,
                                              uint64_t *d_out_len) {
    if (!P) return J2K_ERR_INVALID_ARG;
    j2k_ctx *ctx = P->ctx;
    if (!d_stream || !d_offs || !d_out || !d_out_len) return fail(ctx, J2K_ERR_INVALID_ARG, "null device pointer");
    HIPCHK(ctx, hipSetDevice(ctx->device));
    HIPCHK(ctx, launch_assemble_tiles(ctx->stream, d_stream, d_offs, P->d_tile_job0, P->tile_count, P->tile_first,
                                      P->max_tile_bytes, d_out, d_out_len));
    return J2K_OK;
}

extern "C" int j2k_plan_pack_stream(j2k_plan *P, const uint8_t *d_stream, const uint64_t *d_offs, const uint32_t *d_lens,
                                    const uint8_t *d_numbps, uint8_t *d_pack) {
    if (!P || !d_stream || !d_offs || !d_lens || !d_numbps || !d_pack) return J2K_ERR_INVALID_ARG;
    j2k_ctx *ctx = P->ctx;
    HIPCHK(ctx, hipSetDevice(ctx->device));
    const int n = (int)P->blocks.size();
    const bool ht = P->spec.coder == J2K_CODER_HT;
    if (ht && !P->d_maglens) return fail(ctx, J2K_ERR_UNSUPPORTED, "pack_stream: no j2k_plan_encode_stream (three-kernel path) ran on this plan");
    if (ht && (P->last_stream != d_stream || P->last_lens != d_lens))
        return fail(ctx, J2K_ERR_INVALID_ARG, "pack_stream: d_stream / d_lens are not the outputs of the last j2k_plan_encode_stream on this plan");
    if (ht && !P->toffs_valid) {
        int r = stage_reserve(ctx, 1, ((size_t)n + 1) * 8 + 4096);
        if (r != J2K_OK) return r;
        HIPCHK(ctx, launch_scan(ctx->stream, d_lens, n, (uint64_t *)ctx->stage[1], P->d_mels, P->d_toffs));
        P->want_toffs = true;
        P->toffs_valid = true;
    }
    HIPCHK(ctx, launch_pack(ctx->stream, P->d_bjobs, n, d_stream, d_offs, ht ? P->d_toffs : d_offs, d_lens, d_numbps,
                            ht ? P->d_maglens : nullptr, d_pack));
    return J2K_OK;
}

extern "C" int j2k_plan_unpack_streams(j2k_plan *P, int count, const uint8_t *const *d_packs, const size_t *pack_bytes,
                                       uint8_t *const *d_streams, uint64_t *const *d_offs, uint32_t *const *d_lens, uint8_t *const *d_numbps) {
    if (!P || count < 0 || (count && (!d_packs || !pack_bytes || !d_streams || !d_offs || !d_lens || !d_numbps))) return J2K_ERR_INVALID_ARG;
    for (int i = 0; i < count; i++)
        if (!d_packs[i] || !d_streams[i] || !d_offs[i] || !d_lens[i] || !d_numbps[i]) return J2K_ERR_INVALID_ARG;
    j2k_ctx *ctx = P->ctx;
    HIPCHK(ctx, hipSetDevice(ctx->device));
    if (!count) return J2K_OK;
    const int n = (int)P->blocks.size();
    for (int i = 0; i < count; i++)
        if (pack_bytes[i] < pack_header_bytes((size_t)n)) return fail(ctx, J2K_ERR_INVALID_ARG, "unpack_stream: the pack is shorter than its own header");
    int r = stage_reserve(ctx, 3, 256);
    if (r != J2K_OK) return r;
    ctx->fault_armed = true;
    HIPCHK(ctx, launch_unpack(ctx->stream, P->d_bjobs, n, count, d_packs, pack_bytes, d_streams, (size_t)P->bytes_cap, d_offs, d_lens, d_numbps,
                              (int *)ctx->stage[3]));
    return J2K_OK;
}

extern "C" int j2k_plan_unpack_stream(j2k_plan *P, const uint8_t *d_pack, size_t pack_bytes, uint8_t *d_stream, uint64_t *d_offs,
                                      uint32_t *d_lens, uint8_t *d_numbps) {
    return j2k_plan_unpack_streams(P, 1, &d_pack, &pack_bytes, &d_stream, &d_offs, &d_lens, &d_numbps);
}

extern "C" int j2k_plan_compact(j2k_plan *P, const uint8_t *d_slots, const uint32_t *d_lens, uint64_t *d_offs, uint8_t *d_stream) {
    if (!P || !d_slots || !d_lens || !d_offs || !d_stream) return J2K_ERR_INVALID_ARG;
    j2k_ctx *ctx = P->ctx;
    HIPCHK(ctx, hipSetDevice(ctx->device));
    const int n = (int)P->blocks.size();
    int r = stage_reserve(ctx, 1, 4096);
    if (r != J2K_OK) return r;
    HIPCHK(ctx, launch_compact(ctx->stream, P->d_bjobs, n, d_slots, d_lens, d_offs, d_stream, nullptr));
    return J2K_OK;
}

extern "C" int j2k_plan_set_decode_coded_rows_only(j2k_plan *P, int on) {
    if (!P) return J2K_ERR_INVALID_ARG;
    P->dec_coded_rows_only = on != 0;
    return J2K_OK;
}

extern "C" int j2k_plan_set_dequantize(j2k_plan *P, int on) {
    if (!P) return J2K_ERR_INVALID_ARG;
    if (P->spec.wavelet != W97 || P->spec.quant != Q_ENCODER) return fail(P->ctx, J2K_ERR_UNSUPPORTED, "j2k_plan_set_dequantize: a lossy plan only");
    P->dequantize = on != 0;
    return J2K_OK;
}

extern "C" int j2k_plan_decode_blocks(j2k_plan *P, const uint8_t *d_stream, const uint64_t *d_offs, const uint32_t *d_lens,
                                      const uint8_t *d_numbps, int32_t *d_decoded) {
    if (!P || !d_stream || !d_offs || !d_lens || !d_numbps || !d_decoded) return J2K_ERR_INVALID_ARG;
    return plan_decode_blocks_jobs(P, P->d_djobs, (int)P->blocks.size(), d_stream, d_offs, d_lens, d_numbps, d_decoded, nullptr);
}

int plan_decode_blocks_jobs(j2k_plan *P, const BlockJob *d_djobs, int n, const uint8_t *d_stream, const uint64_t *d_offs, const uint32_t *d_lens,
                            const uint8_t *d_numbps, int32_t *d_decoded, const BlockJob *d_placed) {
    j2k_ctx *ctx = P->ctx;
    HIPCHK(ctx, hipSetDevice(ctx->device));
    if (!n) return J2K_OK;
    if (P->spec.coder == J2K_CODER_HT) {
        int r = stage_reserve(ctx, 2, ht_decode_scratch_words(n) * 4 + 256);
        if (r != J2K_OK) return r;
        HIPCHK(ctx, launch_ht_decode(ctx->stream, d_djobs, n, d_stream, d_offs, d_lens, d_decoded, (uint32_t *)ctx->stage[2],
                                     (d_placed || P->dec_coded_rows_only) ? 1 : 0, d_placed));
    } else {
        size_t wpj = 0;
        int max_dim = 0;
        for (const j2k_block &b : P->blocks) { wpj = std::max(wpj, t1_flag_bytes(b.w, b.h)); max_dim = std::max(max_dim, std::max(b.w, b.h)); }
        wpj = (wpj + 255) & ~size_t(255);
        const int split_min = ctx->t1_dec_split >= 0 ? ctx->t1_dec_split : (mq_throughput_mode() ? 512 : 12000);
        bool split = split_min > 0 && n >= split_min && !ctx->t1_dec_general && !((uintptr_t)d_stream & 15);
        const size_t gen_bytes = (wpj * (size_t)n + 255) & ~size_t(255);
        int r = stage_reserve(ctx, 2, gen_bytes + 256 + (split ? j2k::t1_dec_split_bytes((size_t)n) : 0));
        if (r != J2K_OK && split) { (void)hipGetLastError(); split = false; r = stage_reserve(ctx, 2, gen_bytes + 256); }
        if (r != J2K_OK) return r;
        HIPCHK(ctx, launch_t1_decode(ctx->stream, d_djobs, n, d_stream, d_offs, d_lens, d_numbps, d_decoded,
                                     (uint8_t *)ctx->stage[2], wpj, max_dim, ctx->t1_dec_general,
                                     split ? (uint8_t *)ctx->stage[2] + gen_bytes : nullptr, ctx->t1_dec_lanes, mq_throughput_mode() ? 1 : 0));
    }
    return J2K_OK;
}
```

Baseline: 78080.

## Encode each HT code block with a four-wave workgroup instead of one wave

Adds a 256-thread workgroup kernel for HT block encoding that splits one code block across four wavefronts. The max-magnitude scan, formation of VLC/magsign items, and emission of byte streams are strided across waves, with per-wave sync via waitcnt where only one wave is involved. It is enabled by default through a new ht_enc_waves option set to 4. This targets the latency of single-wave per-block encoding. In exchange it adds cross-wave synchronization, shared buffer coordination, and fewer blocks resident per CU.

```diff
diff --git a/go-jpeg2000_amd/csrc/ht.hip b/go-jpeg2000_amd/csrc/ht.hip
--- a/go-jpeg2000_amd/csrc/ht.hip
+++ b/go-jpeg2000_amd/csrc/ht.hip
@@ -138,10 +138,95 @@
     return (uint32_t)(two >> sh) & 0xFF;
 }
 
+struct HtItem {
+    uint64_t vv;
+    uint32_t vl, ml;
+    uint32_t mval[8], mlen[8];
+};
+
+template <bool LROWS>
+__device__ __forceinline__ void ht_form_item(const BlockJob &J, const int32_t *__restrict__ src, int it, int P, bool vec_ok,
+                                             const int32_t *lrows, const uint16_t *enc, HtItem &I, int &bad) {
+    const int w = J.w, stride = LROWS ? J.w : J.stride;
+    const int r = it / P, pi = it - r * P;
+    const int initial = (r == 0);
+    const int32_t *row = LROWS ? lrows + r * w : src + (size_t)(4 * r) * stride;
+    const int xb = pi * 8;
+    int v[8];
+    if ((LROWS || vec_ok) && xb + 8 <= w) {
+        const int4 a = *reinterpret_cast<const int4 *>(row + xb), b = *reinterpret_cast<const int4 *>(row + xb + 4);
+        v[0] = a.x; v[1] = a.y; v[2] = a.z; v[3] = a.w; v[4] = b.x; v[5] = b.y; v[6] = b.z; v[7] = b.w;
+    } else {
+#pragma unroll
+        for (int i = 0; i < 8; i++) {
+            const int t = row[xb + i < w ? xb + i : w - 1];
+            v[i] = (xb + i < w) ? t : 0;
+        }
+    }
+    uint32_t rho = 0, rho2 = 0;
+#pragma unroll
+    for (int i = 0; i < 4; i++) {
+        if (v[i] != 0) rho |= 1u << i;
+        if (v[4 + i] != 0) rho2 |= 1u << i;
+    }
+    const uint32_t e1 = enc[(initial << 6) | rho];
+    const uint32_t e2 = enc[(initial << 6) | ((rho >> 2) << 4) | rho2];
+    uint64_t vv = (uint64_t)(e1 >> 4);
+    uint32_t vl = e1 & 0xF, ml = 0;
+    vv |= (uint64_t)(e2 >> 4) << vl;
+    vl += e2 & 0xF;
+    if (rho | rho2) {
+        uint32_t u1 = 1, u2 = 1;
+#pragma unroll
+        for (int i = 0; i < 4; i++) {
+            if (xb + i < w && uabs(v[i]) >= shl32(1, u1)) u1++;
+            if (xb + 4 + i < w && uabs(v[4 + i]) >= shl32(1, u2)) u2++;
+        }
+#pragma unroll
+        for (int q = 0; q < 2; q++) {
+            if (!(q ? rho2 : rho)) continue;
+            const uint32_t u = q ? u2 : u1;
+            if (u <= 1) { vv |= (uint64_t)1 << vl; vl += 1; }
+            else if (u <= 2) { vv |= (uint64_t)2 << vl; vl += 2; }
+            else { vv |= (uint64_t)(u - 3) << (vl + 3); vl += 8; }
+        }
+    }
+#pragma unroll
+    for (int i = 0; i < 8; i++) {
+        const uint32_t rr = (i < 4) ? rho : rho2;
+        if (!((rr >> (i & 3)) & 1)) continue;
+        const uint32_t mag = uabs(v[i]);
+        if (mag >= 0x80000000u) { bad = 1; continue; }
+        const uint32_t emb = 32 - __clz(mag);
+        I.mval[i] = (mag & (shl32(1, emb - 1) - 1)) | ((v[i] < 0 ? 1u : 0u) << (emb - 1));
+        I.mlen[i] = emb;
+        ml += emb;
+    }
+    I.vv = vv; I.vl = vl; I.ml = ml;
+}
+
+__device__ __forceinline__ void ht_deposit_item(uint32_t *vbuf, uint32_t *mbuf, uint32_t vpos, uint32_t mpos, const HtItem &I) {
+    or_bits(vbuf, vpos, I.vv);
+    if (I.ml <= 64) {
+        uint64_t acc = 0;
+        uint32_t sh = 0;
+#pragma unroll
+        for (int i = 0; i < 8; i++) {
+            acc |= shl64((uint64_t)I.mval[i], sh);
+            sh += I.mlen[i];
+        }
+        if (acc) or_bits(mbuf, mpos, acc);
+    } else {
+#pragma unroll
+        for (int i = 0; i < 8; i++)
+            if (I.mlen[i]) { or_bits(mbuf, mpos, (uint64_t)I.mval[i]); mpos += I.mlen[i]; }
+    }
+}
+
 template <bool LROWS>
 __device__ __forceinline__ bool ht_form(const BlockJob &J, const int32_t *__restrict__ src, int lane, uint32_t *vbuf, uint32_t *mbuf,
                         uint32_t &TMout, uint32_t &TVout, const int32_t *lrows, const uint16_t *enc) {
-    const int w = J.w, h = J.h, stride = LROWS ? J.w : J.stride;
+    const int w = J.w, h = J.h;
     const int quadCols = (w + 3) / 4, P = (quadCols + 1) / 2, R = (h + 3) / 4, N = R * P;
     for (int i = lane; i < HT_VLC_WORDS; i += 64) vbuf[i] = 0;
     for (int i = lane; i < HT_MS_WORDS; i += 64) mbuf[i] = 0;
@@ -151,86 +236,11 @@
     const bool vec_ok = ((J.stride & 3) == 0) && ((J.src_off & 3) == 0);
     for (int i0 = 0; i0 < N; i0 += 64) {
         const int it = i0 + lane;
-        uint64_t vv = 0; uint32_t vl = 0, ml = 0;
-        uint32_t mval[8], mlen[8];
-#pragma unroll
-        for (int i = 0; i < 8; i++) { mval[i] = 0; mlen[i] = 0; }
-        if (it < N) {
-            const int r = it / P, pi = it - r * P;
-            const int initial = (r == 0);
-            const int32_t *row = LROWS ? lrows + r * w : src + (size_t)(4 * r) * stride;
-            const int xb = pi * 8;
-            int v[8];
-            if ((LROWS || vec_ok) && xb + 8 <= w) {
-                const int4 a = *reinterpret_cast<const int4 *>(row + xb), b = *reinterpret_cast<const int4 *>(row + xb + 4);
-                v[0] = a.x; v[1] = a.y; v[2] = a.z; v[3] = a.w; v[4] = b.x; v[5] = b.y; v[6] = b.z; v[7] = b.w;
-            } else {
-#pragma unroll
-                for (int i = 0; i < 8; i++) {
-                    const int t = row[xb + i < w ? xb + i : w - 1];
-                    v[i] = (xb + i < w) ? t : 0;
-                }
-            }
-            uint32_t rho = 0, rho2 = 0;
-#pragma unroll
-            for (int i = 0; i < 4; i++) {
-                if (v[i] != 0) rho |= 1u << i;
-                if (v[4 + i] != 0) rho2 |= 1u << i;
-            }
-            const uint32_t e1 = enc[(initial << 6) | rho];
-            const uint32_t e2 = enc[(initial << 6) | ((rho >> 2) << 4) | rho2];
-            vv = (uint64_t)(e1 >> 4);
-            vl = e1 & 0xF;
-            vv |= (uint64_t)(e2 >> 4) << vl;
-            vl += e2 & 0xF;
-            if (rho | rho2) {
-                uint32_t u1 = 1, u2 = 1;
-#pragma unroll
-                for (int i = 0; i < 4; i++) {
-                    if (xb + i < w && uabs(v[i]) >= shl32(1, u1)) u1++;
-                    if (xb + 4 + i < w && uabs(v[4 + i]) >= shl32(1, u2)) u2++;
-                }
-#pragma unroll
-                for (int q = 0; q < 2; q++) {
-                    if (!(q ? rho2 : rho)) continue;
-                    const uint32_t u = q ? u2 : u1;
-                    if (u <= 1) { vv |= (uint64_t)1 << vl; vl += 1; }
-                    else if (u <= 2) { vv |= (uint64_t)2 << vl; vl += 2; }
-                    else { vv |= (uint64_t)(u - 3) << (vl + 3); vl += 8; }
-                }
-            }
-#pragma unroll
-            for (int i = 0; i < 8; i++) {
-                const uint32_t rr = (i < 4) ? rho : rho2;
-                if (!((rr >> (i & 3)) & 1)) continue;
-                const uint32_t mag = uabs(v[i]);
-                if (mag >= 0x80000000u) { bad = 1; continue; }
-                const uint32_t emb = 32 - __clz(mag);
-                mval[i] = (mag & (shl32(1, emb - 1) - 1)) | ((v[i] < 0 ? 1u : 0u) << (emb - 1));
-                mlen[i] = emb;
-                ml += emb;
-            }
-        }
-        const uint32_t vs = wave_incl_scan(vl), ms = wave_incl_scan(ml);
+        HtItem I = {};
+        if (it < N) ht_form_item<LROWS>(J, src, it, P, vec_ok, lrows, enc, I, bad);
+        const uint32_t vs = wave_incl_scan(I.vl), ms = wave_incl_scan(I.ml);
         const uint32_t vtot = wave_last(vs), mtot = wave_last(ms);
-        uint32_t vpos = vbase + vs - vl, mpos = mbase + ms - ml;
-        if (it < N) {
-            or_bits(vbuf, vpos, vv);
-            if (ml <= 64) {
-                uint64_t acc = 0;
-                uint32_t sh = 0;
-#pragma unroll
-                for (int i = 0; i < 8; i++) {
-                    acc |= shl64((uint64_t)mval[i], sh);
-                    sh += mlen[i];
-                }
-                if (acc) or_bits(mbuf, mpos, acc);
-            } else {
-#pragma unroll
-                for (int i = 0; i < 8; i++)
-                    if (mlen[i]) { or_bits(mbuf, mpos, (uint64_t)mval[i]); mpos += mlen[i]; }
-            }
-        }
+        if (it < N) ht_deposit_item(vbuf, mbuf, vbase + vs - I.vl, mbase + ms - I.ml, I);
         vbase += vtot; mbase += mtot;
     }
     bad = __any(bad);
@@ -272,9 +282,9 @@
     return nF;
 }
 
-template <bool WRITE>
+template <bool WRITE, int NW = 1>
 __device__ bool ht_emit(const BlockJob &J, uint8_t *__restrict__ out, int lane, const uint32_t *vbuf, const uint32_t *mbuf,
-                        uint32_t mbase, uint32_t vbase, long &magLenOut, long &vlcLenOut, uint16_t *flist) {
+                        uint32_t mbase, uint32_t vbase, long &magLenOut, long &vlcLenOut, uint16_t *flist, int wv = 0) {
     const size_t nsamp = (size_t)J.w * J.h;
     const size_t maxSize = nsamp * 2 < 64 ? 64 : nsamp * 2;
     const long msCap = (long)(maxSize / 2), vlcCap = (long)(maxSize / 2);
@@ -285,7 +295,8 @@
 #endif
     uint32_t myF;
     const int nF = ht_ms_find_ff(mbuf, TM, lane, flist, myF);
-    __syncthreads();
+    if (NW == 1) __syncthreads();
+    else asm volatile("s_waitcnt lgkmcnt(0)" ::: "memory");
 #ifdef J2K_ENC_STAMP
     const long long e05 = wall_clock64();
 #endif
@@ -311,7 +322,7 @@
         const bool inreg = nF <= 64;
         const long myK = (lane < nF) ? (long)((myF + (uint32_t)lane) >> 3) : (long)0x7FFFFFFF;
         int fi = 0;
-        for (long kb = 0; kb < K; kb += 256) {
+        for (long kb = 256 * wv; kb < K; kb += 256 * NW) {
             int fe;
             if (inreg) {
                 fi = __popcll(__ballot(myK <= kb - 2));
@@ -351,7 +362,7 @@
                     if (k0 + j < K) q[j] = (uint8_t)(dw >> (8 * j));
             }
         }
-        if (tail && lane == 0) out[K] = (uint8_t)get_bits8(mbuf, posK);
+        if (tail && lane == 0 && wv == 0) out[K] = (uint8_t)get_bits8(mbuf, posK);
     }
 #ifdef J2K_ENC_STAMP
     const long long e1 = wall_clock64();
@@ -360,7 +371,7 @@
     const long nfull = TV >> 3, vlcLen = (TV + 7) >> 3;
     if (vlcLen > vlcCap) return false;
     uint8_t *vout = out + magLen + melLen;
-    for (long i0 = 4 * lane; WRITE && i0 < vlcLen; i0 += 256) {
+    for (long i0 = 256 * wv + 4 * lane; WRITE && i0 < vlcLen; i0 += 256 * NW) {
         uint32_t dw = ms_bits32(vbuf, (uint32_t)(8 * i0));
 #pragma unroll
         for (int jj = 0; jj < 4; jj++) {
@@ -410,6 +421,189 @@
     return ht_emit<true>(J, out, lane, vbuf, mbuf, TM, TV, magLenOut, vlcLenOut, flist);
 }
 
+template <int SCAN>
+__device__ __forceinline__ void ht_encode_block_wave(const BlockJob &J, int nalias, int aoff, int myalias, int lane, int njobs,
+                                                     const int32_t *__restrict__ coef, uint8_t *__restrict__ slots,
+                                                     uint32_t *__restrict__ lens, uint8_t *__restrict__ numbps,
+                                                     int *__restrict__ fault, uint32_t *__restrict__ maglens,
+                                                     const int *__restrict__ alias_ids, uint32_t *s_vbuf, uint32_t *s_mbuf,
+                                                     int32_t *s_rows, uint32_t *s_enc, uint16_t *s_ff) {
+#ifdef J2K_ENC_STAMP
+    const long long st0 = wall_clock64();
+#endif
+    s_enc[lane] = reinterpret_cast<const uint32_t *>(g_vlc_enc)[lane];
+    const int w = J.w, h = J.h, stride = J.stride;
+    const int32_t *src = coef + J.src_off;
+    uint8_t *out = slots + J.out_off;
+    auto publish = [&](uint32_t len, uint32_t nb, bool has_mag, uint32_t mag) {
+        for (int k = lane; k < nalias; k += 64) {
+            const int j = k < 64 ? myalias : alias_ids[aoff + k];
+            lens[j] = len;
+            numbps[j] = (uint8_t)nb;
+            if (maglens && has_mag) maglens[j] = mag;
+        }
+    };
+    const bool fast = (size_t)((h + 3) / 4) * (size_t)w <= HT_FAST_MAX_SAMPLES;
+
+    int maxMag = 0;
+    const bool quads = (w & 3) == 0 && (stride & 3) == 0 && (J.src_off & 3) == 0;
+    const bool lrows = quads && fast;
+    if (quads) {
+        const int wq = w >> 2, nq = wq * h;
+        const int dy = 64 / wq, dx = 64 - dy * wq;
+        int y = lane / wq, xq = lane - y * wq;
+        for (int e0 = lane; e0 < nq; e0 += 64 * SCAN) {
+            int4 qv[SCAN];
+            int ys[SCAN];
+#pragma unroll
+            for (int u = 0; u < SCAN; u++) {
+                const bool ok = e0 + 64 * u < nq;
+                const int4 t = *reinterpret_cast<const int4 *>(ok ? src + (size_t)y * stride + 4 * xq : src);
+                qv[u] = ok ? t : make_int4(0, 0, 0, 0);
+                ys[u] = ok ? (y << 8 | xq) : -1;
+                y += dy; xq += dx;
+                if (xq >= wq) { xq -= wq; y++; }
+            }
+#pragma unroll
+            for (int u = 0; u < SCAN; u++) {
+                const int4 q = qv[u];
+                if (lrows && ys[u] >= 0 && ((ys[u] >> 8) & 3) == 0)
+                    *reinterpret_cast<int4 *>(&s_rows[(ys[u] >> 10) * w + 4 * (ys[u] & 0xFF)]) = q;
+                const int a0 = q.x < 0 ? (int)(0u - (uint32_t)q.x) : q.x, a1 = q.y < 0 ? (int)(0u - (uint32_t)q.y) : q.y;
+                const int a2 = q.z < 0 ? (int)(0u - (uint32_t)q.z) : q.z, a3 = q.w < 0 ? (int)(0u - (uint32_t)q.w) : q.w;
+                maxMag = max(max(maxMag, max(a0, a1)), max(a2, a3));
+            }
+        }
+    } else {
+        for (int y = 0; y < h; y++)
+            for (int x = lane; x < w; x += 64) {
+                int v = src[(size_t)y * stride + x];
+                if (v < 0) v = (int)(0u - (uint32_t)v);
+                maxMag = max(maxMag, v);
+            }
+    }
+    for (int o = 32; o > 0; o >>= 1) maxMag = max(maxMag, __shfl_xor(maxMag, o));
+#ifdef J2K_ENC_STAMP
+    const long long st1 = wall_clock64();
+#endif
+    if (maxMag == 0) {
+        publish(0, 0, false, 0);
+        return;
+    }
+    if (fast) {
+        long mLen = 0, vLen = 0;
+        const size_t nsamp_ = (size_t)w * h;
+        const size_t maxSize_ = nsamp_ * 2 < 64 ? 64 : nsamp_ * 2;
+        const size_t melLen_ = maxSize_ / 4;
+        const uint16_t *enc = reinterpret_cast<const uint16_t *>(s_enc);
+        const bool ok = lrows ? ht_encode_fast<true>(J, src, out, lane, s_vbuf, s_mbuf, mLen, vLen, s_rows, enc, s_ff)
+                              : ht_encode_fast<false>(J, src, out, lane, s_vbuf, s_mbuf, mLen, vLen, nullptr, enc, s_ff);
+        if (!ok) {
+            if (lane == 0) atomicMax(fault, 1);
+            publish(0, 0, false, 0);
+            return;
+        }
+        if (!maglens) zero_bytes(out + mLen, melLen_, lane);
+        const size_t scup = melLen_ + (size_t)vLen + 2;
+        const size_t total = (size_t)mLen + scup;
+        if (lane == 0) {
+            out[total - 2] = (uint8_t)(scup >> 8);
+            out[total - 1] = (uint8_t)(scup & 0xFF);
+        }
+        publish((uint32_t)total, 32 - __clz((uint32_t)maxMag), true, (uint32_t)mLen);
+#ifdef J2K_ENC_STAMP
+        const long long st2 = wall_clock64();
+        if (((blockIdx.x % 200) == 7 || blockIdx.x >= njobs - 3) && lane == 0)
+            printf("enc wg %d: start %lld end %lld scan %lld  form+emit %lld (x10 ns)  mLen %ld vLen %ld\n", (int)blockIdx.x, st0 % 100000, st2 % 100000, st1 - st0, st2 - st1, mLen, vLen);
+#endif
+        return;
+    }
+    const size_t nsamp = (size_t)w * h;
+    const size_t maxSize = nsamp * 2 < 64 ? 64 : nsamp * 2;
+    const size_t msCap = maxSize / 2, melLen = maxSize / 4, vlcCap = maxSize / 2;
+    uint8_t *vlcScratch = out + msCap + melLen;
+
+    long magLen = 0, vlcLen = 0;
+    int bad = 0;
+    if (lane == 0) {
+        BitWriter vlc{vlcScratch, 0, (long)vlcCap, 0, 0, 0, 0};
+        BitWriter ms{out, 0, (long)msCap, 0, 0, 0, 0};
+        const int quadCols = (w + 3) / 4;
+        for (int y = 0; y < h && !vlc.fault && !ms.fault; y += 4) {
+            const int initial = (y == 0);
+            const int32_t *row = src + (size_t)y * stride;
+            for (int qx = 0; qx < quadCols && !vlc.fault && !ms.fault; qx += 2) {
+                int v[8];
+                uint32_t rho = 0, rho2 = 0;
+#pragma unroll
+                for (int i = 0; i < 8; i++) {
+                    const int x = qx * 4 + i;
+                    v[i] = (x < w) ? row[x] : 0;
+                }
+#pragma unroll
+                for (int i = 0; i < 4; i++) {
+                    if (qx * 4 + i < w && v[i] != 0) rho |= 1u << i;
+                    if ((qx + 1) * 4 + i < w && v[4 + i] != 0) rho2 |= 1u << i;
+                }
+                uint16_t e1 = g_vlc_enc[(initial << 6) | rho];
+                vlc_write(vlc, e1 >> 4, e1 & 0xF);
+                uint16_t e2 = g_vlc_enc[(initial << 6) | ((rho >> 2) << 4) | rho2];
+                vlc_write(vlc, e2 >> 4, e2 & 0xF);
+                if (rho | rho2) {
+                    uint32_t u1 = 1, u2 = 1;
+#pragma unroll
+                    for (int i = 0; i < 4; i++) {
+                        if (qx * 4 + i < w && uabs(v[i]) >= shl32(1, u1)) u1++;
+                        if ((qx + 1) * 4 + i < w && uabs(v[4 + i]) >= shl32(1, u2)) u2++;
+                    }
+                    if (rho && rho2) { uvlc_one(vlc, u1); uvlc_one(vlc, u2); }
+                    else uvlc_one(vlc, rho ? u1 : u2);
+                }
+#pragma unroll
+                for (int i = 0; i < 8; i++) {
+                    const uint32_t r = (i < 4) ? rho : rho2;
+                    if (!((r >> (i & 3)) & 1)) continue;
+                    const uint32_t mag = uabs(v[i]);
+                    if (mag >= 0x80000000u) { ms.fault = 1; break; }
+                    const uint32_t emb = 32 - __clz(mag);
+                    ms_write(ms, mag & (shl32(1, emb - 1) - 1), emb - 1);
+                    ms_write(ms, v[i] < 0 ? 1u : 0u, 1);
+                }
+            }
+        }
+        if (!vlc.fault) flush_bits(vlc);
+        if (!ms.fault) flush_bits(ms);
+        magLen = ms.pos; vlcLen = vlc.pos;
+        bad = vlc.fault | ms.fault;
+    }
+    magLen = __shfl(magLen, 0); vlcLen = __shfl(vlcLen, 0); bad = __shfl(bad, 0);
+    if (bad) {
+        if (lane == 0) atomicMax(fault, 1);
+        publish(0, 0, false, 0);
+        return;
+    }
+    zero_bytes(out + magLen, melLen, lane);
+    __syncthreads();
+    const size_t D = (size_t)magLen + melLen;
+    for (long base = 0; base < vlcLen; base += 64) {
+        const long i = base + lane;
+        uint8_t b = 0;
+        if (i < vlcLen) b = vlcScratch[i];
+        __syncthreads();
+        if (i < vlcLen) out[D + i] = b;
+        __syncthreads();
+    }
+    {
+        const size_t scup = melLen + (size_t)vlcLen + 2;
+        const size_t total = (size_t)magLen + scup;
+        if (lane == 0) {
+            out[total - 2] = (uint8_t)(scup >> 8);
+            out[total - 1] = (uint8_t)(scup & 0xFF);
+        }
+        publish((uint32_t)total, 32 - __clz((uint32_t)maxMag), true, (uint32_t)magLen);
+    }
+}
+
 __global__ __launch_bounds__(64) void ht_encode_kernel(const BlockJob *__restrict__ jobs, int njobs,
                                                        const int32_t *__restrict__ coef, uint8_t *__restrict__ slots,
                                                        uint32_t *__restrict__ lens, uint8_t *__restrict__ numbps,
@@ -422,9 +616,6 @@
     __shared__ uint16_t s_ff[HT_MS_FF_CAP];
     if ((int)blockIdx.x >= njobs) return;
     const int lane = threadIdx.x;
-#ifdef J2K_ENC_STAMP
-    const long long st0 = wall_clock64();
-#endif
     BlockJob J;
     int jid = (int)blockIdx.x, nalias = 1, aoff = 0;
     if (utab) {
@@ -435,8 +626,43 @@
     }
     int myalias = jid;
     if (utab && lane < nalias) myalias = alias_ids[aoff + lane];
-    s_enc[lane] = reinterpret_cast<const uint32_t *>(g_vlc_enc)[lane];
+    ht_encode_block_wave<16>(J, nalias, aoff, myalias, lane, njobs, coef, slots, lens, numbps, fault, maglens, alias_ids, s_vbuf, s_mbuf,
+                         s_rows, s_enc, s_ff);
+}
+
+__device__ __forceinline__ void ht_lds_barrier() { asm volatile("s_waitcnt lgkmcnt(0)\n\ts_barrier" ::: "memory"); }
+
+__global__ __launch_bounds__(256) void ht_encode_wg_kernel(int nunique, const int32_t *__restrict__ coef, uint8_t *__restrict__ slots,
+                                                           uint32_t *__restrict__ lens, uint8_t *__restrict__ numbps,
+                                                           int *__restrict__ fault, uint32_t *__restrict__ maglens,
+                                                           const HtUJob *__restrict__ utab, const int *__restrict__ alias_ids) {
+    __shared__ uint32_t s_vbuf[HT_VLC_WORDS];
+    __shared__ uint32_t s_mbuf[HT_MS_WORDS];
+    __shared__ __align__(16) int32_t s_rows[HT_FAST_MAX_SAMPLES];
+    __shared__ uint32_t s_enc[64];
+    __shared__ uint16_t s_ff[HT_MS_FF_CAP];
+    __shared__ int s_max[4], s_bad[4];
+    __shared__ uint32_t s_tot[4][2];
+    if ((int)blockIdx.x >= nunique) return;
+    const int tid = threadIdx.x, lane = tid & 63;
+    const int wave = __builtin_amdgcn_readfirstlane(tid >> 6);
+#ifdef J2K_ENC_STAMP
+    const long long st0 = wall_clock64();
+#endif
+    const HtUJob U = utab[blockIdx.x];
+    const BlockJob J = U.J;
+    const int nalias = U.nalias, aoff = U.alias_off;
+    int myalias = U.jid;
+    if (wave == 0 && lane < nalias) myalias = alias_ids[aoff + lane];
     const int w = J.w, h = J.h, stride = J.stride;
+    const bool fast = (size_t)((h + 3) / 4) * (size_t)w <= HT_FAST_MAX_SAMPLES;
+    const bool quads = (w & 3) == 0 && (stride & 3) == 0 && (J.src_off & 3) == 0;
+    if (!(quads && fast)) {
+        if (wave != 0) return;
+        ht_encode_block_wave<4>(J, nalias, aoff, myalias, lane, nunique, coef, slots, lens, numbps, fault, maglens, alias_ids, s_vbuf,
+                             s_mbuf, s_rows, s_enc, s_ff);
+        return;
+    }
     const int32_t *src = coef + J.src_off;
     uint8_t *out = slots + J.out_off;
     auto publish = [&](uint32_t len, uint32_t nb, bool has_mag, uint32_t mag) {
@@ -447,165 +673,97 @@
             if (maglens && has_mag) maglens[j] = mag;
         }
     };
-    const bool fast = (size_t)((h + 3) / 4) * (size_t)w <= HT_FAST_MAX_SAMPLES;
 
     int maxMag = 0;
-    const bool quads = (w & 3) == 0 && (stride & 3) == 0 && (J.src_off & 3) == 0;
-    const bool lrows = quads && fast;
-    if (quads) {
+    {
         const int wq = w >> 2, nq = wq * h;
-        const int dy = 64 / wq, dx = 64 - dy * wq;
-        int y = lane / wq, xq = lane - y * wq;
-        for (int e0 = lane; e0 < nq; e0 += 64 * 16) {
-            int4 qv[16];
-            int ys[16];
-#pragma unroll
-            for (int u = 0; u < 16; u++) {
-                const bool ok = e0 + 64 * u < nq;
-                const int4 t = *reinterpret_cast<const int4 *>(ok ? src + (size_t)y * stride + 4 * xq : src);
-                qv[u] = ok ? t : make_int4(0, 0, 0, 0);
-                ys[u] = ok ? (y << 8 | xq) : -1;
-                y += dy; xq += dx;
-                if (xq >= wq) { xq -= wq; y++; }
-            }
-#pragma unroll
-            for (int u = 0; u < 16; u++) {
-                const int4 q = qv[u];
-                if (lrows && ys[u] >= 0 && ((ys[u] >> 8) & 3) == 0)
-                    *reinterpret_cast<int4 *>(&s_rows[(ys[u] >> 10) * w + 4 * (ys[u] & 0xFF)]) = q;
-                const int a0 = q.x < 0 ? (int)(0u - (uint32_t)q.x) : q.x, a1 = q.y < 0 ? (int)(0u - (uint32_t)q.y) : q.y;
-                const int a2 = q.z < 0 ? (int)(0u - (uint32_t)q.z) : q.z, a3 = q.w < 0 ? (int)(0u - (uint32_t)q.w) : q.w;
-                maxMag = max(max(maxMag, max(a0, a1)), max(a2, a3));
-            }
-        }
-    } else {
-        for (int y = 0; y < h; y++)
-            for (int x = lane; x < w; x += 64) {
-                int v = src[(size_t)y * stride + x];
-                if (v < 0) v = (int)(0u - (uint32_t)v);
-                maxMag = max(maxMag, v);
-            }
+        const int dy = 256 / wq, dx = 256 - dy * wq;
+        int y = tid / wq, xq = tid - y * wq;
+        int4 qv[4];
+        int ys[4];
+#pragma unroll
+        for (int u = 0; u < 4; u++) {
+            const bool ok = tid + 256 * u < nq;
+            const int4 t = *reinterpret_cast<const int4 *>(ok ? src + (size_t)y * stride + 4 * xq : src);
+            qv[u] = ok ? t : make_int4(0, 0, 0, 0);
+            ys[u] = ok ? (y << 8 | xq) : -1;
+            y += dy; xq += dx;
+            if (xq >= wq) { xq -= wq; y++; }
+        }
+        if (tid < 64) s_enc[tid] = reinterpret_cast<const uint32_t *>(g_vlc_enc)[tid];
+        for (int i = tid; i < HT_VLC_WORDS; i += 256) s_vbuf[i] = 0;
+        for (int i = tid; i < HT_MS_WORDS; i += 256) s_mbuf[i] = 0;
+#pragma unroll
+        for (int u = 0; u < 4; u++) {
+            const int4 q = qv[u];
+            if (ys[u] >= 0 && ((ys[u] >> 8) & 3) == 0)
+                *reinterpret_cast<int4 *>(&s_rows[(ys[u] >> 10) * w + 4 * (ys[u] & 0xFF)]) = q;
+            const int a0 = q.x < 0 ? (int)(0u - (uint32_t)q.x) : q.x, a1 = q.y < 0 ? (int)(0u - (uint32_t)q.y) : q.y;
+            const int a2 = q.z < 0 ? (int)(0u - (uint32_t)q.z) : q.z, a3 = q.w < 0 ? (int)(0u - (uint32_t)q.w) : q.w;
+            maxMag = max(max(maxMag, max(a0, a1)), max(a2, a3));
+        }
     }
     for (int o = 32; o > 0; o >>= 1) maxMag = max(maxMag, __shfl_xor(maxMag, o));
+    if (lane == 0) s_max[wave] = maxMag;
+    ht_lds_barrier();
+    maxMag = max(max(s_max[0], s_max[1]), max(s_max[2], s_max[3]));
 #ifdef J2K_ENC_STAMP
     const long long st1 = wall_clock64();
 #endif
     if (maxMag == 0) {
-        publish(0, 0, false, 0);
+        if (wave == 0) publish(0, 0, false, 0);
         return;
     }
-    if (fast) {
-        long mLen = 0, vLen = 0;
-        const size_t nsamp_ = (size_t)w * h;
-        const size_t maxSize_ = nsamp_ * 2 < 64 ? 64 : nsamp_ * 2;
-        const size_t melLen_ = maxSize_ / 4;
-        const uint16_t *enc = reinterpret_cast<const uint16_t *>(s_enc);
-        const bool ok = lrows ? ht_encode_fast<true>(J, src, out, lane, s_vbuf, s_mbuf, mLen, vLen, s_rows, enc, s_ff)
-                              : ht_encode_fast<false>(J, src, out, lane, s_vbuf, s_mbuf, mLen, vLen, nullptr, enc, s_ff);
-        if (!ok) {
+
+    const int quadCols = w >> 2, P = (quadCols + 1) / 2, R = (h + 3) / 4, N = R * P;
+    const uint16_t *enc = reinterpret_cast<const uint16_t *>(s_enc);
+    HtItem I = {};
+    int bad = 0;
+    if (tid < N) ht_form_item<true>(J, src, tid, P, true, s_rows, enc, I, bad);
+    const uint32_t vs = wave_incl_scan(I.vl), ms = wave_incl_scan(I.ml);
+    bad = __any(bad);
+    if (lane == 63) { s_tot[wave][0] = vs; s_tot[wave][1] = ms; s_bad[wave] = bad; }
+    ht_lds_barrier();
+    uint32_t vbase = 0, mbase = 0, TV = 0, TM = 0;
+    bad = 0;
+#pragma unroll
+    for (int k = 0; k < 4; k++) {
+        const uint32_t a = s_tot[k][0], b = s_tot[k][1];
+        if (k < wave) { vbase += a; mbase += b; }
+        TV += a; TM += b;
+        bad |= s_bad[k];
+    }
+    if (tid < N) ht_deposit_item(s_vbuf, s_mbuf, vbase + vs - I.vl, mbase + ms - I.ml, I);
+    ht_lds_barrier();
+#ifdef J2K_ENC_STAMP
+    const long long st2 = wall_clock64();
+#endif
+    long mLen = 0, vLen = 0;
+    if (bad || !ht_emit<true, 4>(J, out, lane, s_vbuf, s_mbuf, TM, TV, mLen, vLen, s_ff, wave)) {
+        if (wave == 0) {
             if (lane == 0) atomicMax(fault, 1);
             publish(0, 0, false, 0);
-            return;
-        }
-        if (!maglens) zero_bytes(out + mLen, melLen_, lane);
-        const size_t scup = melLen_ + (size_t)vLen + 2;
+        }
+        return;
+    }
+    if (wave == 0) {
+        const size_t nsamp = (size_t)w * h;
+        const size_t maxSize = nsamp * 2 < 64 ? 64 : nsamp * 2;
+        const size_t melLen = maxSize / 4;
+        if (!maglens) zero_bytes(out + mLen, melLen, lane);
+        const size_t scup = melLen + (size_t)vLen + 2;
         const size_t total = (size_t)mLen + scup;
         if (lane == 0) {
             out[total - 2] = (uint8_t)(scup >> 8);
             out[total - 1] = (uint8_t)(scup & 0xFF);
         }
         publish((uint32_t)total, 32 - __clz((uint32_t)maxMag), true, (uint32_t)mLen);
+    }
 #ifdef J2K_ENC_STAMP
-        const long long st2 = wall_clock64();
-        if (((blockIdx.x % 200) == 7 || blockIdx.x >= njobs - 3) && lane == 0)
-            printf("enc wg %d: start %lld end %lld scan %lld  form+emit %lld (x10 ns)  mLen %ld vLen %ld\n", (int)blockIdx.x, st0 % 100000, st2 % 100000, st1 - st0, st2 - st1, mLen, vLen);
-#endif
-        return;
-    }
-    const size_t nsamp = (size_t)w * h;
-    const size_t maxSize = nsamp * 2 < 64 ? 64 : nsamp * 2;
-    const size_t msCap = maxSize / 2, melLen = maxSize / 4, vlcCap = maxSize / 2;
-    uint8_t *vlcScratch = out + msCap + melLen;
-
-    long magLen = 0, vlcLen = 0;
-    int bad = 0;
-    if (lane == 0) {
-        BitWriter vlc{vlcScratch, 0, (long)vlcCap, 0, 0, 0, 0};
-        BitWriter ms{out, 0, (long)msCap, 0, 0, 0, 0};
-        const int quadCols = (w + 3) / 4;
-        for (int y = 0; y < h && !vlc.fault && !ms.fault; y += 4) {
-            const int initial = (y == 0);
-            const int32_t *row = src + (size_t)y * stride;
-            for (int qx = 0; qx < quadCols && !vlc.fault && !ms.fault; qx += 2) {
-                int v[8];
-                uint32_t rho = 0, rho2 = 0;
-#pragma unroll
-                for (int i = 0; i < 8; i++) {
-                    const int x = qx * 4 + i;
-                    v[i] = (x < w) ? row[x] : 0;
-                }
-#pragma unroll
-                for (int i = 0; i < 4; i++) {
-                    if (qx * 4 + i < w && v[i] != 0) rho |= 1u << i;
-                    if ((qx + 1) * 4 + i < w && v[4 + i] != 0) rho2 |= 1u << i;
-                }
-                uint16_t e1 = g_vlc_enc[(initial << 6) | rho];
-                vlc_write(vlc, e1 >> 4, e1 & 0xF);
-                uint16_t e2 = g_vlc_enc[(initial << 6) | ((rho >> 2) << 4) | rho2];
-                vlc_write(vlc, e2 >> 4, e2 & 0xF);
-                if (rho | rho2) {
-                    uint32_t u1 = 1, u2 = 1;
-#pragma unroll
-                    for (int i = 0; i < 4; i++) {
-                        if (qx * 4 + i < w && uabs(v[i]) >= shl32(1, u1)) u1++;
-                        if ((qx + 1) * 4 + i < w && uabs(v[4 + i]) >= shl32(1, u2)) u2++;
-                    }
-                    if (rho && rho2) { uvlc_one(vlc, u1); uvlc_one(vlc, u2); }
-                    else uvlc_one(vlc, rho ? u1 : u2);
-                }
-#pragma unroll
-                for (int i = 0; i < 8; i++) {
-                    const uint32_t r = (i < 4) ? rho : rho2;
-                    if (!((r >> (i & 3)) & 1)) continue;
-                    const uint32_t mag = uabs(v[i]);
-                    if (mag >= 0x80000000u) { ms.fault = 1; break; }
-                    const uint32_t emb = 32 - __clz(mag);
-                    ms_write(ms, mag & (shl32(1, emb - 1) - 1), emb - 1);
-                    ms_write(ms, v[i] < 0 ? 1u : 0u, 1);
-                }
-            }
-        }
-        if (!vlc.fault) flush_bits(vlc);
-        if (!ms.fault) flush_bits(ms);
-        magLen = ms.pos; vlcLen = vlc.pos;
-        bad = vlc.fault | ms.fault;
-    }
-    magLen = __shfl(magLen, 0); vlcLen = __shfl(vlcLen, 0); bad = __shfl(bad, 0);
-    if (bad) {
-        if (lane == 0) atomicMax(fault, 1);
-        publish(0, 0, false, 0);
-        return;
-    }
-    zero_bytes(out + magLen, melLen, lane);
-    __syncthreads();
-    const size_t D = (size_t)magLen + melLen;
-    for (long base = 0; base < vlcLen; base += 64) {
-        const long i = base + lane;
-        uint8_t b = 0;
-        if (i < vlcLen) b = vlcScratch[i];
-        __syncthreads();
-        if (i < vlcLen) out[D + i] = b;
-        __syncthreads();
-    }
-    {
-        const size_t scup = melLen + (size_t)vlcLen + 2;
-        const size_t total = (size_t)magLen + scup;
-        if (lane == 0) {
-            out[total - 2] = (uint8_t)(scup >> 8);
-            out[total - 1] = (uint8_t)(scup & 0xFF);
-        }
-        publish((uint32_t)total, 32 - __clz((uint32_t)maxMag), true, (uint32_t)magLen);
-    }
+    if (((blockIdx.x % 200) == 7 || (int)blockIdx.x >= nunique - 3) && lane == 0)
+        printf("enc4 wg %d wave %d: start %lld scan %lld form %lld emit %lld (x10 ns)  mLen %ld vLen %ld\n", (int)blockIdx.x, wave,
+               st0 % 100000, st1 - st0, st2 - st1, wall_clock64() - st2, mLen, vLen);
+#endif
 }
 
 #define HT_ST_AGG 1ull
@@ -1545,12 +1703,15 @@
 
 hipError_t launch_ht_encode(hipStream_t s, const BlockJob *jobs, int njobs, const int32_t *coef, uint8_t *slots,
                             uint32_t *lens, uint8_t *numbps, int *fault, uint32_t *maglens, const HtUJob *utab, int nunique,
-                            const int *alias_ids) {
+                            const int *alias_ids, int waves) {
     if (njobs <= 0) return hipSuccess;
     hipError_t e;
     if ((e = ht_tables_ready(s)) != hipSuccess) return e;
     const int n = utab ? nunique : njobs;
-    hipLaunchKernelGGL(ht_encode_kernel, dim3(n), dim3(64), 0, s, jobs, n, coef, slots, lens, numbps, fault, maglens, utab, alias_ids);
+    if (waves == 4 && utab && alias_ids)
+        hipLaunchKernelGGL(ht_encode_wg_kernel, dim3(n), dim3(256), 0, s, n, coef, slots, lens, numbps, fault, maglens, utab, alias_ids);
+    else
+        hipLaunchKernelGGL(ht_encode_kernel, dim3(n), dim3(64), 0, s, jobs, n, coef, slots, lens, numbps, fault, maglens, utab, alias_ids);
     return hipGetLastError();
 }
 
diff --git a/go-jpeg2000_amd/csrc/j2k_ctx.cpp b/go-jpeg2000_amd/csrc/j2k_ctx.cpp
--- a/go-jpeg2000_amd/csrc/j2k_ctx.cpp
+++ b/go-jpeg2000_amd/csrc/j2k_ctx.cpp
@@ -32,6 +32,7 @@
         OPT("l0_xcd", v == 0 || v == 1, c->l0_xcd = v != 0),
         OPT("l0_deal", v == 0 || v == 1, c->l0_deal = v != 0),
         OPT("ht_alias", v == 0 || v == 1, c->ht_alias = v != 0),
+        OPT("ht_enc_waves", v == 1 || v == 4, c->ht_enc_waves = (int)v),
         OPT("l0_inv_wpe", v >= 5 && v <= 7, c->l0_inv_wpe = (int)v),
         OPT("l0_wg_inv", v == 0 || v == 1, c->l0_wg_inv = v != 0),
         OPT("l0_wg_invw", v == 0 || v == 4 || v == 8, c->l0_wg_invw = (int)v),
diff --git a/go-jpeg2000_amd/csrc/j2k_host.h b/go-jpeg2000_amd/csrc/j2k_host.h
--- a/go-jpeg2000_amd/csrc/j2k_host.h
+++ b/go-jpeg2000_amd/csrc/j2k_host.h
@@ -24,7 +24,7 @@
 hipError_t launch_dequantize97(hipStream_t s, const int32_t *src, size_t n, double step, double *dst);
 hipError_t launch_ht_encode(hipStream_t s, const BlockJob *jobs, int njobs, const int32_t *coef, uint8_t *slots,
                             uint32_t *lens, uint8_t *numbps, int *fault, uint32_t *maglens = nullptr, const HtUJob *utab = nullptr, int nunique = 0,
-                            const int *alias_ids = nullptr);
+                            const int *alias_ids = nullptr, int waves = 1);
 hipError_t launch_ht_decode(hipStream_t s, const BlockJob *jobs, int njobs, const uint8_t *stream, const uint64_t *offs,
                             const uint32_t *lens, int32_t *decoded, uint32_t *scratch, int coded_rows_only = 0, const BlockJob *placed_jobs = nullptr);
 size_t ht_decode_scratch_words(int njobs);
diff --git a/go-jpeg2000_amd/csrc/j2k_plan.h b/go-jpeg2000_amd/csrc/j2k_plan.h
--- a/go-jpeg2000_amd/csrc/j2k_plan.h
+++ b/go-jpeg2000_amd/csrc/j2k_plan.h
@@ -25,6 +25,7 @@
     int l0_xcd_group = 16;
     bool l0_xcd = true;
     bool ht_alias = true;
+    int ht_enc_waves = 4;
     int l0_inv_wpe = 5;
     bool l0_wg_inv = true;
     int l0_store = 1;
diff --git a/go-jpeg2000_amd/csrc/j2k_stages.cpp b/go-jpeg2000_amd/csrc/j2k_stages.cpp
--- a/go-jpeg2000_amd/csrc/j2k_stages.cpp
+++ b/go-jpeg2000_amd/csrc/j2k_stages.cpp
@@ -660,7 +660,7 @@
     ctx->fault_armed = true;
     for (int rep_ = 0; rep_ < dev_reps(8); rep_++)
     HIPCHK(ctx, launch_ht_encode(ctx->stream, P->d_bjobs, n, d_coeff, (uint8_t *)P->d_slots, d_lens, d_numbps, (int *)ctx->stage[3],
-                                 P->d_maglens, P->d_ht_ujobs, P->ht_nunique, P->d_ht_alias_next));
+                                 P->d_maglens, P->d_ht_ujobs, P->ht_nunique, P->d_ht_alias_next, ctx->ht_enc_waves));
     return J2K_OK;
 }
 
```

After: 79210, median of 6. 1.01x the previous value.
